# feiyeha/BS-YOLO

Hardware: AMD Instinct MI355X
Metric: images/sec YOLO11s 640x640 bs=64 (forward + NMS) (higher is better)
Workload: dtype f16

## Files before the change

bs_yolo_amd/csrc/c3k2_fused.hip:

```cpp
#include "common.h"

#define CK_TH 4
#define CK_TW 16
#define CK_XR (CK_TH + 4)
#define CK_XC (CK_TW + 4)
#define CK_NX (CK_XR * CK_XC)
#define CK_MR (CK_TH + 2)
#define CK_MC (CK_TW + 2)
#define CK_NM (CK_MR * CK_MC)
#define CK_NPX (CK_TH * CK_TW)

struct C3k2K {
    const half_t* src;
    half_t* dst;
    const half_t *w1, *wa, *wb, *w4;
    const float *b1, *ba, *bb, *b4;
    int B, H, W, lds, ldd, K1, Ka, Kb, K4;
    TileGrid grid;
};

template <int CIN, int C, int C2>
__global__ __launch_bounds__(256, 3) void c3k2_fused_kernel(const C3k2K p) {
    constexpr int CH = C / 2;
    constexpr int YS = C + 8, MS = CH + 8, OS = C2 + 8;
    constexpr int WAS = 9 * C + 8, WBS = 9 * CH + 8;
    constexpr int KS1 = CIN / 16, KSA = 9 * C / 16, KSB = 9 * CH / 16, KSEG = C / 16;
    static_assert(C == 32 && CH == 16 && CIN % 16 == 0 && C2 == 128 && CK_NX == 160 && CK_NPX == 64, "instantiated for the c = 32 C3k2 block");
    constexpr int SY1 = CK_NX * YS, SY0 = CK_NPX * YS, SM = CK_NM * MS, SY2 = CK_NPX * YS;
    constexpr int SOUT = CK_NPX * OS;
    static_assert(SOUT <= SY1 + SY0, "output tile must fit the y1 + y0 tiles it aliases");
    constexpr int SWA = CH * WAS, SWB = C * WBS;
    constexpr int W0S = CIN + 8, SW0 = C * W0S;
    __shared__ __attribute__((aligned(16))) half_t lds[SY1 + SY0 + SM + SY2 + SWA + SWB + SW0 + 2 * (2 * C + CH + C + C2)];
    half_t* sy1 = lds;
    half_t* sy0 = sy1 + SY1;
    half_t* sout = lds;
    half_t* smid = sy0 + SY0;
    half_t* sy2 = smid + SM;
    half_t* swa = sy2 + SY2;
    half_t* swb = swa + SWA;
    half_t* sw0 = swb + SWB;
    float* sb1 = reinterpret_cast<float*>(sw0 + SW0);
    float* sba = sb1 + 2 * C;
    float* sbb = sba + CH;
    float* sb4 = sbb + C;

    const int tid = threadIdx.x, lane = tid & 63;
    const int wave = __builtin_amdgcn_readfirstlane(tid >> 6);
    const int lrow = lane & 31, lh = lane >> 5;

    for (int i = tid; i < 2 * C; i += 256) sb1[i] = p.b1[i];
    if (tid < CH) sba[tid] = p.ba[tid];
    if (tid < C) sbb[tid] = p.bb[tid];
    for (int i = tid; i < C2; i += 256) sb4[i] = p.b4[i];
    half8 w1y1[KS1], a4[3 * KSEG];
#pragma unroll
    for (int ks = 0; ks < KS1; ++ks) w1y1[ks] = *reinterpret_cast<const half8*>(p.w1 + (size_t)(C + lrow) * p.K1 + 16 * ks + 8 * lh);
    for (int i = tid; i < C * (CIN / 8); i += 256) {
        const int row = i / (CIN / 8), ch = i - row * (CIN / 8);
        *reinterpret_cast<half8*>(sw0 + row * W0S + ch * 8) = *reinterpret_cast<const half8*>(p.w1 + (size_t)row * p.K1 + ch * 8);
    }
#pragma unroll
    for (int ks = 0; ks < 3 * KSEG; ++ks) a4[ks] = *reinterpret_cast<const half8*>(p.w4 + (size_t)(32 * wave + lrow) * p.K4 + 16 * ks + 8 * lh);
    for (int i = tid; i < CH * (9 * C / 8); i += 256) {
        const int row = i / (9 * C / 8), ch = i - row * (9 * C / 8);
        *reinterpret_cast<half8*>(swa + row * WAS + ch * 8) = *reinterpret_cast<const half8*>(p.wa + (size_t)row * p.Ka + ch * 8);
    }
    for (int i = tid; i < C * (9 * CH / 8); i += 256) {
        const int row = i / (9 * CH / 8), ch = i - row * (9 * CH / 8);
        *reinterpret_cast<half8*>(swb + row * WBS + ch * 8) = *reinterpret_cast<const half8*>(p.wb + (size_t)row * p.Kb + ch * 8);
    }

    auto tile_origin = [&](int tile, int& n, int& oy0, int& ox0) {
        const TileIdx t = tile_index(p.grid, tile);
        n = t.n; oy0 = t.ty * CK_TH; ox0 = t.tx * CK_TW;
    };
    const int lty = lrow >> 4, ltx = lrow & 15;
    const int eA = 32 * wave + lrow, rA = eA / CK_XC, cA = eA - rA * CK_XC;
    const bool b_y0 = wave == 1 || wave == 2;
    const int eB = b_y0 ? (2 * (wave - 1) + lty + 2) * CK_XC + ltx + 2 : 128 + lrow, rB = eB / CK_XC, cB = eB - rB * CK_XC;
    const unsigned relA = (unsigned)((rA * p.W + cA) * p.lds + 8 * lh), relB = (unsigned)((rB * p.W + cB) * p.lds + 8 * lh);
    half8 xa[KS1], xb[KS1];
    int nn = 0, noy0 = 0, nox0 = 0;
    auto fetch = [&](int tile) {
        tile_origin(tile, nn, noy0, nox0);
        const half_t* tb = p.src + ((long long)(nn * p.H + noy0 - 2) * p.W + (nox0 - 2)) * p.lds;
        const bool inA = (unsigned)(noy0 - 2 + rA) < (unsigned)p.H && (unsigned)(nox0 - 2 + cA) < (unsigned)p.W;
        const bool inB = wave < 3 && (unsigned)(noy0 - 2 + rB) < (unsigned)p.H && (unsigned)(nox0 - 2 + cB) < (unsigned)p.W;
#pragma unroll
        for (int ks = 0; ks < KS1; ++ks) {
            xa[ks] = half8{0, 0, 0, 0, 0, 0, 0, 0};
            xb[ks] = half8{0, 0, 0, 0, 0, 0, 0, 0};
            if (inA) xa[ks] = *reinterpret_cast<const half8*>(tb + relA + 16 * ks);
            if (inB) xb[ks] = *reinterpret_cast<const half8*>(tb + relB + 16 * ks);
        }
    };
    constexpr int CPRW = C2 / 8, NST = CK_NPX * CPRW / 256;
    const int mm2 = wave * 32 + lrow, mc2 = mm2 < CK_NM ? mm2 : CK_NM - 1, r2 = mc2 / CK_MC, c2 = mc2 - r2 * CK_MC;

    const half_t* a2base = swb + lrow * WBS + 8 * lh;
    const int a1off = (lrow & (CH - 1)) * WAS + 8 * lh;

    __builtin_amdgcn_s_waitcnt(0x0F70);
    const TileWalk tw = xcd_tile_walk(blockIdx.x, gridDim.x, p.grid.ntiles);
    int tile = tw.tile;
    if (tile < tw.end) fetch(tile);
    __syncthreads();
    for (; tile < tw.end; tile += tw.step) {
        const int n = nn, oy0 = noy0, ox0 = nox0;
        half_t* ob = p.dst + ((long long)(n * p.H + oy0) * p.W + ox0) * p.ldd;
        auto s1_job = [&](const bool is_y0, const half8 (&wf)[KS1], const half8 (&xf)[KS1], const int e, const int r, const int c, const int opix) {
            f32x16 acc;
            acc_bias(acc, sb1 + (is_y0 ? 0 : C), lh);
#pragma unroll
            for (int ks = 0; ks < KS1; ++ks)
                acc = __builtin_amdgcn_mfma_f32_32x32x16_f16(wf[ks], xf[ks], acc, 0, 0, 0);
            const unsigned keep = (is_y0 || ((unsigned)(oy0 - 2 + r) < (unsigned)p.H && (unsigned)(ox0 - 2 + c) < (unsigned)p.W)) ? 0xffffffffu : 0u;
            half_t* d = is_y0 ? sy0 + opix * YS : sy1 + e * YS;
#pragma unroll
            for (int g = 0; g < C / 8; ++g) {
                union { half4 h; unsigned u[2]; } o;
                const f32x4 tv = silu4_f(f32x4{acc[4 * g], acc[4 * g + 1], acc[4 * g + 2], acc[4 * g + 3]});
#pragma unroll
                for (int q = 0; q < 4; ++q) o.h[q] = (half_t)tv[q];
                o.u[0] &= keep;
                o.u[1] &= keep;
                *reinterpret_cast<half4*>(d + 8 * g + 4 * lh) = o.h;
            }
        };
        s1_job(false, w1y1, xa, eA, rA, cA, 0);
        if (wave == 0) s1_job(false, w1y1, xb, eB, rB, cB, 0);
        else if (wave < 3) {
            int wo = lrow * W0S + 8 * lh;
            asm volatile("" : "+v"(wo));
            half8 w1y0[KS1];
#pragma unroll
            for (int ks = 0; ks < KS1; ++ks) w1y0[ks] = *reinterpret_cast<const half8*>(sw0 + wo + 16 * ks);
            s1_job(true, w1y0, xb, eB, rB, cB, 32 * (wave - 1) + lrow);
        }
        if (tile + tw.step < tw.end) fetch(tile + tw.step);
        lds_barrier();

        {
            const int mm = mm2, r = r2, c = c2;
            const half_t* yb = sy1 + (r * CK_XC + c) * YS + 8 * lh;
            int ao = a1off;
            asm volatile("" : "+v"(ao));
            const half_t* a1base = swa + ao;
            f32x16 acc;
            acc_bias(acc, sba, lh);
#pragma unroll
            for (int ks = 0; ks < KSA; ++ks) {
                const int k0 = 16 * ks, tap = k0 / C, ch0 = (k0 % C) / 8;
                const half8 bf = *reinterpret_cast<const half8*>(yb + ((tap / 3) * CK_XC + tap % 3) * YS + ch0 * 8);
                acc = __builtin_amdgcn_mfma_f32_32x32x16_f16(*reinterpret_cast<const half8*>(a1base + 16 * ks), bf, acc, 0, 0, 0);
            }
            const unsigned keep = ((unsigned)(oy0 - 1 + r) < (unsigned)p.H && (unsigned)(ox0 - 1 + c) < (unsigned)p.W) ? 0xffffffffu : 0u;
            if (mm < CK_NM) {
#pragma unroll
                for (int g = 0; g < CH / 8; ++g) {
                    union { half4 h; unsigned u[2]; } o;
                    const f32x4 tv = silu4_f(f32x4{acc[4 * g], acc[4 * g + 1], acc[4 * g + 2], acc[4 * g + 3]});
#pragma unroll
                    for (int q = 0; q < 4; ++q) o.h[q] = (half_t)tv[q];
                    o.u[0] &= keep;
                    o.u[1] &= keep;
                    *reinterpret_cast<half4*>(smid + mm * MS + 8 * g + 4 * lh) = o.h;
                }
            }
        }
        lds_barrier();

        if (wave < 2) {
            const int ty2 = 2 * wave + lty;
            const half_t* b2base = smid + (ty2 * CK_MC + ltx) * MS + 8 * lh;
            const half_t* y1own = sy1 + ((ty2 + 2) * CK_XC + ltx + 2) * YS;
            f32x16 acc;
            acc_bias(acc, sbb, lh);
#pragma unroll
            for (int ks = 0; ks < KSB; ++ks) {
                const int k0 = 16 * ks, tap = k0 / CH, ch0 = (k0 % CH) / 8;
                const half8 bf = *reinterpret_cast<const half8*>(b2base + ((tap / 3) * CK_MC + tap % 3) * MS + ch0 * 8);
                acc = __builtin_amdgcn_mfma_f32_32x32x16_f16(*reinterpret_cast<const half8*>(a2base + 16 * ks), bf, acc, 0, 0, 0);
            }
#pragma unroll
            for (int g = 0; g < C / 8; ++g) {
                const half4 rv = *reinterpret_cast<const half4*>(y1own + 8 * g + 4 * lh);
                half4 o;
                const f32x4 tv = silu4_f(f32x4{acc[4 * g], acc[4 * g + 1], acc[4 * g + 2], acc[4 * g + 3]});
#pragma unroll
                for (int q = 0; q < 4; ++q) o[q] = (half_t)((float)(half_t)tv[q] + (float)rv[q]);
                *reinterpret_cast<half4*>(sy2 + (32 * wave + lrow) * YS + 8 * g + 4 * lh) = o;
            }
        }
        lds_barrier();

        {
            f32x16 acc[2];
#pragma unroll
            for (int q2 = 0; q2 < 2; ++q2) acc_bias(acc[q2], sb4 + 32 * wave, lh);
#pragma unroll
            for (int ks = 0; ks < 3 * KSEG; ++ks) {
                const int seg = ks / KSEG, kk = ks - seg * KSEG;
#pragma unroll
                for (int q2 = 0; q2 < 2; ++q2) {
                    const int prow = 32 * q2 + lrow;
                    const half_t* sp = seg == 0 ? sy0 + prow * YS : (seg == 1 ? sy1 + ((2 * q2 + lty + 2) * CK_XC + ltx + 2) * YS : sy2 + prow * YS);
                    acc[q2] = __builtin_amdgcn_mfma_f32_32x32x16_f16(a4[ks], *reinterpret_cast<const half8*>(sp + 16 * kk + 8 * lh), acc[q2], 0, 0, 0);
                }
            }
            lds_barrier();
#pragma unroll
            for (int q2 = 0; q2 < 2; ++q2)
#pragma unroll
                for (int g = 0; g < 4; ++g) {
                    const int cc = 32 * wave + 8 * g + 4 * lh;
                    half4 o;
                    const f32x4 tv = silu4_f(f32x4{acc[q2][4 * g], acc[q2][4 * g + 1], acc[q2][4 * g + 2], acc[q2][4 * g + 3]});
#pragma unroll
                    for (int q = 0; q < 4; ++q) o[q] = (half_t)tv[q];
                    *reinterpret_cast<half4*>(sout + (32 * q2 + lrow) * OS + cc) = o;
                }
        }
        lds_barrier();

#pragma unroll
        for (int j = 0; j < NST; ++j) {
            const int id = tid + 256 * j, pr = id / CPRW, cc = (id % CPRW) * 8, sy = pr / CK_TW, sx_ = pr % CK_TW;
            if (oy0 + sy < p.H && ox0 + sx_ < p.W)
                *reinterpret_cast<half8*>(ob + (size_t)(sy * p.W + sx_) * p.ldd + cc) = *reinterpret_cast<const half8*>(sout + pr * OS + cc);
        }
        lds_barrier();
    }
}

bool c3k2_fused_supported(int Cin, int C, int C2) { return Cin == 64 && C == 32 && C2 == 128; }

int launch_c3k2_fused(const C3k2Args& a, hipStream_t s) {
    if (!c3k2_fused_supported(a.Cin, a.C, a.C2)) BSY_FAIL(BSY_ERR_ARG, "c3k2: unsupported widths (Cin %d, c %d, C2 %d): need (64, 32, 128)", a.Cin, a.C, a.C2);
    if (a.B <= 0 || a.H <= 0 || a.W <= 0) BSY_FAIL(BSY_ERR_ARG, "c3k2: bad extent");
    const void* ptrs[10] = {a.src, a.dst, a.w1, a.wa, a.wb, a.w4, a.b1, a.ba, a.bb, a.b4};
    for (const void* q : ptrs)
        if (!q || ((uintptr_t)q & 15)) BSY_FAIL(BSY_ERR_ARG, "c3k2: null or misaligned pointer");
    if ((a.lds & 7) || (a.ldd & 7) || a.lds < a.Cin || a.ldd < a.C2) BSY_FAIL(BSY_ERR_ARG, "c3k2: bad leading dimension");
    C3k2K k;
    k.src = a.src; k.dst = a.dst; k.w1 = (const half_t*)a.w1; k.wa = (const half_t*)a.wa; k.wb = (const half_t*)a.wb; k.w4 = (const half_t*)a.w4;
    k.b1 = a.b1; k.ba = a.ba; k.bb = a.bb; k.b4 = a.b4;
    k.B = a.B; k.H = a.H; k.W = a.W; k.lds = a.lds; k.ldd = a.ldd;
    int cp = 0;
    bsy_conv_packed_dims(2 * a.C, a.Cin, 1, &cp, &k.K1);
    bsy_conv_packed_dims(a.C / 2, a.C, 3, &cp, &k.Ka);
    bsy_conv_packed_dims(a.C, a.C / 2, 3, &cp, &k.Kb);
    bsy_conv_packed_dims(a.C2, 3 * a.C, 1, &cp, &k.K4);
    const int rc = make_tile_grid(k.grid, a.B, a.H, a.W, CK_TH, CK_TW, "c3k2");
    if (rc != BSY_OK) return rc;
    const int grid = k.grid.ntiles < 768 ? k.grid.ntiles : 768;
    hipLaunchKernelGGL((c3k2_fused_kernel<64, 32, 128>), dim3(grid), dim3(256), 0, s, k);
    HIP_TRY(hipGetLastError());
    return BSY_OK;
}
```

bs_yolo_amd/csrc/common.h:

```cpp
#pragma once
#include <hip/hip_runtime.h>
#include <stdint.h>
#include <stdio.h>
#include <string>

#include "../../include/bsyolo.h"

typedef _Float16 half_t;
typedef _Float16 half8 __attribute__((ext_vector_type(8)));
typedef _Float16 half4 __attribute__((ext_vector_type(4)));
typedef _Float16 half2v __attribute__((ext_vector_type(2)));
typedef float f32x16 __attribute__((ext_vector_type(16)));
typedef float f32x4 __attribute__((ext_vector_type(4)));

void bsy_set_error(const char* fmt, ...);
#define BSY_FAIL(code, ...)        \
    do {                           \
        bsy_set_error(__VA_ARGS__); \
        return (code);             \
    } while (0)
#define HIP_TRY(expr)                                                                                     \
    do {                                                                                                  \
        hipError_t _e = (expr);                                                                           \
        if (_e != hipSuccess) BSY_FAIL(BSY_ERR_HIP, "%s failed: %s (%s:%d)", #expr, hipGetErrorString(_e), \
                                       __FILE__, __LINE__);                                               \
    } while (0)

static inline int ceil_div(int a, int b) { return (a + b - 1) / b; }
static inline int round_up(int a, int b) { return ceil_div(a, b) * b; }

struct ConvArgs {
    const half_t* src0;
    const half_t* src1;
    int ld0, ld1;
    int C0, C1;
    int up0, up1;
    int B, H, W, OH, OW;
    int ksize, stride, pad;
    const half_t* wgt;
    const float* bias;
    void* dst;
    int ldd, Cout, out_f32;
    const half_t* res;
    int ldr;
    int act;
    int dst_scale, dst_dy, dst_dx;
    int cfg;
    int epi;
    void* y;
    int y_f32, A, a0, nrows;
    float lvl_stride;
    void* raw;
    int raw_f32, rawC;
    const half_t* tail_wgt;
    const float* tail_bias;
    int nsl_c = 0, nsl_t = 0;
    float* split_ws = nullptr;
};
int launch_conv(const ConvArgs& a, hipStream_t s);
#define BSY_CONV_MAX_CFG 64
int conv_candidates(const ConvArgs& a, int* out, int max_out);
bool conv_cfg_valid(const ConvArgs& a, int cfg);
int conv_korder(const ConvArgs& a);

struct ConvFirstArgs {
    const void* img;
    int img_dtype;
    int B, H, W, OH, OW, ksize, stride, pad;
    const void* w;
    const float* b;
    half_t* dst;
    int ldd, Cout, act;
};
int launch_conv_first(const ConvFirstArgs& a, hipStream_t s);

struct StemArgs {
    const void* img;
    int img_dtype;
    int B, H, W, OH, OW;
    const void* w0;
    const float* b0;
    const void* w1;
    const float* b1;
    int C0, C1, Kpad1;
    half_t* dst;
    int ldd, act;
};
bool stem_fused_supported(int C0, int C1, int H, int W);
int launch_stem_fused(const StemArgs& a, hipStream_t s);

struct BneckArgs {
    const half_t* src;
    int lds;
    int B, H, W, C, CH;
    const void *w1, *w2;
    const float *b1, *b2;
    int Kpad1, Kpad2;
    half_t* dst;
    int ldd, act;
};
bool bneck_fused_supported(int C, int CH);
int launch_bneck_fused(const BneckArgs& a, hipStream_t s);

struct C3k2Args {
    const half_t* src;
    int lds;
    int B, H, W, Cin, C, C2;
    const void *w1, *wa, *wb, *w4;
    const float *b1, *ba, *bb, *b4;
    half_t* dst;
    int ldd;
};
bool c3k2_fused_supported(int Cin, int C, int C2);
int launch_c3k2_fused(const C3k2Args& a, hipStream_t s);

struct DwGenArgs {
    const half_t* src;
    int lds;
    int B, H, W, C, OH, OW, kh, kw, stride;
    const float* w;
    int wld;
    const float* b;
    half_t* dst;
    int ldd, act_c;
    int ident_c0 = 0;
};
int launch_dwconv_generic(const DwGenArgs& a, hipStream_t s);
struct PmsfaArgs {
    const half_t* P;
    int ldp;
    const half_t* x;
    int ldx;
    half_t* dst;
    int ldd;
    int B, H, W, C;
    const float* w2;
    const float* b2;
    int wld2;
    const float* w3;
    const float* b3;
    int wld3;
    const half_t* w4;
    const float* b4;
    int kpad4;
};
bool pmsfa_tail_supported(int C);
int launch_pmsfa_tail(const PmsfaArgs& a, hipStream_t s);
int launch_copy_view(const half_t* src, int lds_, int up, int B, int H, int W, int C, half_t* dst, int ldd, hipStream_t s);
int launch_gap(const half_t* src, int lds_, int B, int H, int W, int C, half_t* out, int ldo, hipStream_t s);
struct MscaSpArgs {
    const half_t* src;
    int lds, B, H, W, C;
    const float* w[9];
    const float* b[9];
    half_t* br[4];
    int ldb[4];
    half_t* gap[4];
    int ldg[4];
};
bool msca_spatial_supported(int H, int W);
int launch_msca_spatial(const MscaSpArgs& a, hipStream_t s);
struct MixArgs {
    const half_t* br[4];
    int ldb[4];
    const float* lg[4];
    int ldl[4];
    int B, HW, C;
    half_t* dst;
    int ldd;
};
int launch_msca_mix(const MixArgs& a, hipStream_t s);
int launch_mul(const half_t* a, int lda, const half_t* b, int ldb, long long npix, int C, half_t* dst, int ldd, hipStream_t s);
struct ElaArgs {
    const half_t* src;
    int lds;
    int B, H, W, C, k;
    const float *wsp, *wch, *gnw, *gnb;
    float ch_coef, sp_coef, res_coef;
    float* scratch;
    half_t* dst;
    int ldd;
};
size_t ela_scratch_floats(int H, int W, int C);
int launch_ela(const ElaArgs& a, hipStream_t s);
int launch_ela_gate(const ElaArgs& a, hipStream_t s);

struct Conv32Args {
    const void* src0;
    const void* src1;
    int src_dtype, first;
    int ld0, ld1, C0, C1, up0, up1;
    int B, H, W, OH, OW, ks, stride, pad;
    const float* w;
    const float* bias;
    float* dst;
    int ldd, Cout;
    const float* res;
    int ldr, act, dst_scale, dst_dy, dst_dx;
    const half_t* wx_hi;
    const half_t* wx_lo;
    int wx_kpad;
};
int launch_conv32(const Conv32Args& a, hipStream_t s);
bool conv32x_mfma_supported(const Conv32Args& a);
int launch_conv32x_mfma(const Conv32Args& a, hipStream_t s);
int launch_conv32_scalar(const Conv32Args& a, hipStream_t s);
bool conv32_mfma_supported(const Conv32Args& a);
int launch_conv32_mfma(const Conv32Args& a, hipStream_t s);
struct Dw32Args {
    const float* src;
    int lds, B, H, W, C, OH, OW, kh, kw, stride;
    const float* w;
    int wld;
    const float* b;
    float* dst;
    int ldd, act_c;
    const float* res;
    int ldr;
};
int launch_dw32(const Dw32Args& a, hipStream_t s);
struct Mix32Args {
    const float* br[4];
    int ldb[4];
    const float* lg[4];
    int ldl[4];
    int B, HW, C;
    float* dst;
    int ldd;
};
int launch_mix32(const Mix32Args& a, hipStream_t s);
int launch_sppf32(float* buf, int ld, int B, int H, int W, int C, hipStream_t s);
int launch_attn32(const float* qkv, int ld, int B, int N, int heads, int kd, int hd, float scale, float* out, int ldo, hipStream_t s,
                  int impl = 0);
bool attn32x_supported(int ld, int ldo, int kd, int hd, const void* qkv, const void* out);
int launch_attn32x(const float* qkv, int ld, int B, int N, int heads, int kd, int hd, float scale, float* out, int ldo, hipStream_t s);
int launch_nhwc2nchw32(const float* src, int ld, int B, int C, int hw, void* out, int out_dtype, hipStream_t s);
int launch_copy32(const float* src, int lds_, int up, int B, int H, int W, int C, float* dst, int ldd, hipStream_t s);
int launch_gap32(const float* src, int lds_, int B, int H, int W, int C, float* out, int ldo, hipStream_t s);
int launch_mul32(const float* x, int ldx, const float* y, int ldy, long long npix, int C, float* dst, int ldd, hipStream_t s);
int launch_ela32(const ElaArgs& a, const float* src, float* dst, hipStream_t s);

struct DwPwArgs {
    const half_t* src;
    int lds;
    int B, H, W, C;
    const float *dww, *dwb;
    const void* wgt;
    const float* bias;
    half_t* dst;
    int ldd, Cout, act;
};
bool dwpw_fused_supported(int C, int Cout);
int launch_dwpw_fused(const DwPwArgs& a, hipStream_t s);

struct DwArgs {
    const half_t* src;
    int lds;
    int B, H, W, C;
    const float* w;
    const float* b;
    half_t* dst;
    int ldd;
    int act;
    const half_t* res;
// ... 168 lines not shown
```

bs_yolo_amd/csrc/engine.hip:

```cpp
#include <stdlib.h>
#include <string.h>

#include <algorithm>
#include <vector>

#include "common.h"

struct bsy_engine {
    int device = 0;
    void* weights = nullptr;
    size_t weight_bytes = 0;
    char* arena = nullptr;
    size_t arena_bytes = 0;
    unsigned arena_gen = 0;
    unsigned weights_gen = 0;
};

struct bsy_plan {
    bsy_engine* eng = nullptr;
    std::vector<bsy_op> ops;
    std::vector<size_t> buf_off;
    std::vector<size_t> buf_size;
    char* workspace = nullptr;
    size_t workspace_bytes = 0;
// ... 200 lines not shown
    float* f(const bsy_view& v) { char* b = base(v); return b ? (float*)b + v.coff : nullptr; }
};

static inline size_t fp32x_align(size_t n) { return (n + 255) & ~(size_t)255; }

int run_op_f32(const bsy_plan* p, const bsy_op& op, Resolver& R, hipStream_t s, bool& handled) {
    const char* wb = (const char*)p->eng->weights;
    handled = true;
    switch (op.kind) {
        case BSY_OP_CONV_FIRST:
        case BSY_OP_CONV: {
            Conv32Args a;
            memset(&a, 0, sizeof(a));
            a.first = op.kind == BSY_OP_CONV_FIRST;
            a.src0 = a.first ? (const void*)R.base(op.src0) : (const void*)R.f(op.src0);
            a.src_dtype = op.in_dtype;
            a.src1 = R.f(op.src1);
            a.ld0 = op.src0.ld; a.ld1 = op.src1.buf >= 0 ? op.src1.ld : 0;
            a.C0 = op.src0.C; a.C1 = op.src1.buf >= 0 ? op.src1.C : 0;
            a.up0 = op.up0; a.up1 = op.up1;
            a.B = op.B; a.H = op.H; a.W = op.W; a.OH = op.OH; a.OW = op.OW; a.ks = op.ksize; a.stride = op.stride; a.pad = op.pad;
            a.w = (const float*)(wb + op.w_off); a.bias = (const float*)(wb + op.b_off);
            a.dst = R.f(op.dst); a.ldd = op.dst.ld; a.Cout = op.dst.C;
            a.res = R.f(op.res); a.ldr = op.res.buf >= 0 ? op.res.ld : 0;
            a.act = op.act; a.dst_scale = op.dst_scale > 0 ? op.dst_scale : 1; a.dst_dy = op.dst_dy; a.dst_dx = op.dst_dx;
            if (op.out_f32 >= 2) BSY_FAIL(BSY_ERR_ARG, "fp32 mode: fused Detect decoder ops are not part of fp32 plans");
            if (!R.ok) return BSY_ERR_ARG;
            if (op.prec == 2) {
                const size_t K = (size_t)a.ks * a.ks * (a.C0 + a.C1), kpad = (K + 31) & ~(size_t)31;
                const size_t hi_off = fp32x_align(K * a.Cout * 4), lo_off = hi_off + fp32x_align((size_t)a.Cout * kpad * 2);
                a.wx_hi = (const half_t*)(wb + op.w_off + hi_off);
                a.wx_lo = (const half_t*)(wb + op.w_off + lo_off);
                a.wx_kpad = (int)kpad;
                if (conv32x_mfma_supported(a)) return launch_conv32x_mfma(a, s);
            }
            return launch_conv32(a, s);
        }
        case BSY_OP_DWCONV:
        case BSY_OP_DWCONV_G: {
            Dw32Args a;
            memset(&a, 0, sizeof(a));
            const bool g = op.kind == BSY_OP_DWCONV_G;
            a.src = R.f(op.src0); a.lds = op.src0.ld; a.B = op.B; a.H = op.H; a.W = op.W; a.C = op.src0.C; a.OH = op.OH; a.OW = op.OW;
            a.kh = g ? op.ksize : 3; a.kw = g ? op.pad : 3; a.stride = g ? op.stride : 1;
            a.wld = g ? op.heads : op.src0.C;
            a.w = (const float*)(wb + op.w_off) + (g ? op.key_dim : 0); a.b = (const float*)(wb + op.b_off) + (g ? op.key_dim : 0);
            a.dst = R.f(op.dst); a.ldd = op.dst.ld; a.act_c = g ? op.act : (op.act ? op.src0.C : 0);
            a.res = g ? nullptr : R.f(op.res); a.ldr = (!g && op.res.buf >= 0) ? op.res.ld : 0;
            if (!R.ok) return BSY_ERR_ARG;
            return launch_dw32(a, s);
        }
        case BSY_OP_SPPF_POOL: {
            float* b = R.f(op.src0);
            if (!R.ok) return BSY_ERR_ARG;
            return launch_sppf32(b, op.src0.ld, op.B, op.H, op.W, op.src0.C, s);
        }
        case BSY_OP_ATTN: {
            const float* q = R.f(op.src0);
            float* o = R.f(op.dst);
            if (!R.ok) return BSY_ERR_ARG;
            if (op.prec == 2 && attn32x_supported(op.src0.ld, op.dst.ld, op.key_dim, op.head_dim, q, o))
                return launch_attn32x(q, op.src0.ld, op.B, op.H * op.W, op.heads, op.key_dim, op.head_dim, op.scale, o, op.dst.ld, s);
            return launch_attn32(q, op.src0.ld, op.B, op.H * op.W, op.heads, op.key_dim, op.head_dim, op.scale, o, op.dst.ld, s);
        }
        case BSY_OP_NHWC2NCHW: {
            if (op.dst.buf >= BSY_EXT_BASE && (op.dst.buf - BSY_EXT_BASE >= R.n_ext || !R.ext[op.dst.buf - BSY_EXT_BASE])) return BSY_OK;
            const float* src = R.f(op.src0);
            void* out = R.base(op.dst);
            if (!R.ok) return BSY_ERR_ARG;
            return launch_nhwc2nchw32(src, op.src0.ld, op.B, op.src0.C, op.H * op.W, out, op.out_dtype, s);
        }
        case BSY_OP_COPY: {
            const float* src = R.f(op.src0);
            float* dst = R.f(op.dst);
            if (!R.ok) return BSY_ERR_ARG;
            return launch_copy32(src, op.src0.ld, op.up0, op.B, op.H, op.W, op.src0.C, dst, op.dst.ld, s);
        }
        case BSY_OP_GAP: {
            const float* src = R.f(op.src0);
            float* dst = R.f(op.dst);
            if (!R.ok) return BSY_ERR_ARG;
            return launch_gap32(src, op.src0.ld, op.B, op.H, op.W, op.src0.C, dst, op.dst.ld, s);
        }
        case BSY_OP_MSCA_MIX: {
            Mix32Args a;
            for (int i = 0; i < 4; ++i) {
                const bsy_view& bv = i < 3 ? op.box[i] : op.res;
                const bsy_view& lv = i < 3 ? op.cls[i] : op.msk[0];
                a.br[i] = R.f(bv); a.ldb[i] = bv.ld; a.lg[i] = R.f(lv); a.ldl[i] = lv.ld;
            }
            a.B = op.B; a.HW = op.H * op.W; a.C = op.dst.C; a.dst = R.f(op.dst); a.ldd = op.dst.ld;
            if (!R.ok) return BSY_ERR_ARG;
            return launch_mix32(a, s);
        }
        case BSY_OP_MUL: {
            const float* x = R.f(op.src0);
            const float* y = R.f(op.src1);
            float* dst = R.f(op.dst);
            if (!R.ok) return BSY_ERR_ARG;
            return launch_mul32(x, op.src0.ld, y, op.src1.ld, (long long)op.B * op.H * op.W, op.dst.C, dst, op.dst.ld, s);
        }
        case BSY_OP_ELA: {
            ElaArgs a;
            memset(&a, 0, sizeof(a));
            a.lds = op.src0.ld; a.B = op.B; a.H = op.H; a.W = op.W; a.C = op.src0.C; a.k = op.ksize;
            const float* blob = (const float*)(wb + op.w_off);
            a.wsp = blob; a.wch = blob + (size_t)a.C * a.k; a.gnw = a.wch + (size_t)a.C * a.k; a.gnb = a.gnw + a.C;
            a.ch_coef = op.scale; a.sp_coef = op.lvl_stride[0]; a.res_coef = op.lvl_stride[1];
            a.scratch = R.f(op.res); a.ldd = op.dst.ld;
            const float* src = R.f(op.src0);
            float* dst = R.f(op.dst);
            if (!R.ok) return BSY_ERR_ARG;
            return launch_ela32(a, src, dst, s);
        }
        case BSY_OP_DECODE:
        case BSY_OP_RAW_NCHW:
            handled = false;
            return BSY_OK;
        default:
            BSY_FAIL(BSY_ERR_ARG, "fp32 mode: op kind %d has no fp32 implementation (fused kinds are fp16-only)", op.kind);
    }
}

int run_op(const bsy_plan* p, const bsy_op& op, Resolver& R, hipStream_t s, ConvArgs* cargs = nullptr) {
    const char* wb = (const char*)p->eng->weights;
    if (op.prec == 1 || op.prec == 2) {
        bool handled = false;
        const int rc = run_op_f32(p, op, R, s, handled);
        if (rc != BSY_OK || handled) return rc;
    } else if (op.prec != 0) {
        BSY_FAIL(BSY_ERR_ARG, "plan_run: unknown precision mode %d", op.prec);
    }
    switch (op.kind) {
        case BSY_OP_CONV_FIRST: {
            ConvFirstArgs a;
            a.img = R.base(op.src0); a.img_dtype = op.in_dtype;
            a.B = op.B; a.H = op.H; a.W = op.W; a.OH = op.OH; a.OW = op.OW;
            a.ksize = op.ksize; a.stride = op.stride; a.pad = op.pad;
            a.w = (const void*)(wb + op.w_off); a.b = (const float*)(wb + op.b_off);
            a.dst = R.h(op.dst); a.ldd = op.dst.ld; a.Cout = op.dst.C; a.act = op.act;
            if (!R.ok) return BSY_ERR_ARG;
            return launch_conv_first(a, s);
        }
        case BSY_OP_STEM: {
            StemArgs a;
            a.img = R.base(op.src0); a.img_dtype = op.in_dtype;
            a.B = op.B; a.H = op.H; a.W = op.W; a.OH = op.OH; a.OW = op.OW;
            a.w0 = (const void*)(wb + op.w_off); a.b0 = (const float*)(wb + op.b_off);
            a.w1 = (const void*)(wb + op.w2_off); a.b1 = (const float*)(wb + op.b2_off);
            a.C0 = op.mid_c; a.C1 = op.dst.C;
            int cp = 0;
            bsy_conv_packed_dims(a.C1, a.C0, 3, &cp, &a.Kpad1);
            a.dst = R.h(op.dst); a.ldd = op.dst.ld; a.act = op.act;
            if (!R.ok) return BSY_ERR_ARG;
            return launch_stem_fused(a, s);
        }
        case BSY_OP_BNECK: {
            BneckArgs a;
            a.src = R.h(op.src0); a.lds = op.src0.ld; a.B = op.B; a.H = op.H; a.W = op.W;
            a.C = op.dst.C; a.CH = op.mid_c;
            a.w1 = (const void*)(wb + op.w_off); a.b1 = (const float*)(wb + op.b_off);
            a.w2 = (const void*)(wb + op.w2_off); a.b2 = (const float*)(wb + op.b2_off);
            int cp = 0;
            bsy_conv_packed_dims(a.CH, a.C, 3, &cp, &a.Kpad1);
            bsy_conv_packed_dims(a.C, a.CH, 3, &cp, &a.Kpad2);
            a.dst = R.h(op.dst); a.ldd = op.dst.ld; a.act = op.act;
            if (!R.ok) return BSY_ERR_ARG;
            return launch_bneck_fused(a, s);
        }
        case BSY_OP_S2D: {
            const void* img = R.base(op.src0);
            half_t* dst = R.h(op.dst);
            if (!R.ok) return BSY_ERR_ARG;
            return launch_s2d(img, op.in_dtype, op.B, op.H, op.W, dst, op.dst.ld, s);
        }
        case BSY_OP_C3K2: {
            C3k2Args a;
            a.src = R.h(op.src0); a.lds = op.src0.ld; a.B = op.B; a.H = op.H; a.W = op.W;
            a.Cin = op.src0.C; a.C = op.mid_c; a.C2 = op.dst.C;
            a.w1 = wb + op.aux_off[0]; a.b1 = (const float*)(wb + op.aux_off[1]);
            a.wa = wb + op.aux_off[2]; a.ba = (const float*)(wb + op.aux_off[3]);
            a.wb = wb + op.aux_off[4]; a.bb = (const float*)(wb + op.aux_off[5]);
            a.w4 = wb + op.aux_off[6]; a.b4 = (const float*)(wb + op.aux_off[7]);
            a.dst = R.h(op.dst); a.ldd = op.dst.ld;
            if (!R.ok) return BSY_ERR_ARG;
            return launch_c3k2_fused(a, s);
        }
        case BSY_OP_DWPW: {
            DwPwArgs a;
            a.src = R.h(op.src0); a.lds = op.src0.ld; a.B = op.B; a.H = op.H; a.W = op.W; a.C = op.src0.C;
            a.dww = (const float*)(wb + op.w_off); a.dwb = (const float*)(wb + op.b_off);
            a.wgt = (const void*)(wb + op.w2_off); a.bias = (const float*)(wb + op.b2_off);
            a.dst = R.h(op.dst); a.ldd = op.dst.ld; a.Cout = op.dst.C; a.act = op.act;
            if (!R.ok) return BSY_ERR_ARG;
            return launch_dwpw_fused(a, s);
        }
        case BSY_OP_DWCONV_G: {
            DwGenArgs a;
            a.src = R.h(op.src0); a.lds = op.src0.ld; a.B = op.B; a.H = op.H; a.W = op.W; a.C = op.src0.C;
            a.OH = op.OH; a.OW = op.OW; a.kh = op.ksize; a.kw = op.pad; a.stride = op.stride;
            a.wld = op.heads; a.w = (const float*)(wb + op.w_off) + op.key_dim; a.b = (const float*)(wb + op.b_off) + op.key_dim;
            a.dst = R.h(op.dst); a.ldd = op.dst.ld; a.act_c = op.act;
            a.ident_c0 = op.mid_c;
            if (!R.ok) return BSY_ERR_ARG;
            return launch_dwconv_generic(a, s);
        }
        case BSY_OP_PMSFA_TAIL: {
            PmsfaArgs a;
            a.P = R.h(op.src0); a.ldp = op.src0.ld; a.x = R.h(op.res); a.ldx = op.res.ld; a.dst = R.h(op.dst); a.ldd = op.dst.ld;
            a.B = op.B; a.H = op.H; a.W = op.W; a.C = op.dst.C;
            a.w2 = (const float*)(wb + op.aux_off[0]); a.b2 = (const float*)(wb + op.aux_off[1]); a.wld2 = op.heads;
            a.w3 = (const float*)(wb + op.aux_off[2]); a.b3 = (const float*)(wb + op.aux_off[3]); a.wld3 = op.key_dim;
            a.w4 = (const half_t*)(wb + op.aux_off[4]); a.b4 = (const float*)(wb + op.aux_off[5]);
            int cp = 0;
            bsy_conv_packed_dims(a.C, a.C, 1, &cp, &a.kpad4);
            if (!R.ok || op.src0.C != a.C || op.res.C != a.C) return BSY_ERR_ARG;
            return launch_pmsfa_tail(a, s);
        }
        case BSY_OP_COPY: {
            const half_t* src = R.h(op.src0);
            half_t* dst = R.h(op.dst);
            if (!R.ok) return BSY_ERR_ARG;
            return launch_copy_view(src, op.src0.ld, op.up0, op.B, op.H, op.W, op.src0.C, dst, op.dst.ld, s);
        }
        case BSY_OP_GAP: {
            const half_t* src = R.h(op.src0);
            half_t* dst = R.h(op.dst);
            if (!R.ok) return BSY_ERR_ARG;
            return launch_gap(src, op.src0.ld, op.B, op.H, op.W, op.src0.C, dst, op.dst.ld, s);
        }
        case BSY_OP_MSCA_SPATIAL: {
            MscaSpArgs a;
            a.src = R.h(op.src0); a.lds = op.src0.ld; a.B = op.B; a.H = op.H; a.W = op.W; a.C = op.src0.C;
            for (int i = 0; i < 9; ++i) {
                a.w[i] = (const float*)(wb + op.aux_off[2 * i]);
                a.b[i] = (const float*)(wb + op.aux_off[2 * i + 1]);
            }
            for (int i = 0; i < 4; ++i) {
                const bsy_view& bv = i < 3 ? op.box[i] : op.res;
                const bsy_view& gv = i < 3 ? op.cls[i] : op.msk[0];
                a.br[i] = R.h(bv); a.ldb[i] = bv.ld; a.gap[i] = R.h(gv); a.ldg[i] = gv.ld;
            }
            if (!R.ok) return BSY_ERR_ARG;
            return launch_msca_spatial(a, s);
        }
        case BSY_OP_MSCA_MIX: {
            MixArgs a;
            for (int i = 0; i < 4; ++i) {
                const bsy_view& bv = i < 3 ? op.box[i] : op.res;
                const bsy_view& lv = i < 3 ? op.cls[i] : op.msk[0];
                a.br[i] = R.h(bv); a.ldb[i] = bv.ld; a.lg[i] = R.f(lv); a.ldl[i] = lv.ld;
            }
            a.B = op.B; a.HW = op.H * op.W; a.C = op.dst.C; a.dst = R.h(op.dst); a.ldd = op.dst.ld;
            if (!R.ok) return BSY_ERR_ARG;
            return launch_msca_mix(a, s);
        }
        case BSY_OP_MUL: {
            const half_t* x = R.h(op.src0);
            const half_t* y = R.h(op.src1);
            half_t* dst = R.h(op.dst);
            if (!R.ok) return BSY_ERR_ARG;
            return launch_mul(x, op.src0.ld, y, op.src1.ld, (long long)op.B * op.H * op.W, op.dst.C, dst, op.dst.ld, s);
        }
        case BSY_OP_ELA: {
            ElaArgs a;
            a.src = R.h(op.src0); a.lds = op.src0.ld; a.B = op.B; a.H = op.H; a.W = op.W; a.C = op.src0.C; a.k = op.ksize;
            const float* blob = (const float*)(wb + op.w_off);
            a.wsp = blob; a.wch = blob + (size_t)a.C * a.k; a.gnw = a.wch + (size_t)a.C * a.k; a.gnb = a.gnw + a.C;
            a.ch_coef = op.scale; a.sp_coef = op.lvl_stride[0]; a.res_coef = op.lvl_stride[1];
            a.scratch = R.f(op.res); a.dst = R.h(op.dst); a.ldd = op.dst.ld;
            if (!R.ok) return BSY_ERR_ARG;
            return launch_ela(a, s);
        }
        case BSY_OP_CONV: {
            ConvArgs a;
            a.src0 = R.h(op.src0); a.src1 = R.h(op.src1);
            a.ld0 = op.src0.ld; a.ld1 = op.src1.buf >= 0 ? op.src1.ld : 0;
            a.C0 = op.src0.C; a.C1 = op.src1.buf >= 0 ? op.src1.C : 0;
            a.up0 = op.up0; a.up1 = op.up1;
            a.B = op.B; a.H = op.H; a.W = op.W; a.OH = op.OH; a.OW = op.OW;
            a.ksize = op.ksize; a.stride = op.stride; a.pad = op.pad;
            a.wgt = (const half_t*)(wb + op.w_off); a.bias = (const float*)(wb + op.b_off);
            a.dst = op.out_f32 ? (void*)R.f(op.dst) : (void*)R.h(op.dst);
            a.ldd = op.dst.ld; a.Cout = op.dst.C; a.out_f32 = op.out_f32;
            a.res = R.h(op.res); a.ldr = op.res.buf >= 0 ? op.res.ld : 0;
            a.act = op.act; a.dst_scale = op.dst_scale; a.dst_dy = op.dst_dy; a.dst_dx = op.dst_dx;
            a.epi = 0; a.y = nullptr; a.raw = nullptr; a.y_f32 = a.raw_f32 = a.A = a.a0 = a.nrows = a.rawC = 0; a.lvl_stride = 0.f;
            a.tail_wgt = nullptr; a.tail_bias = nullptr;
            if (op.out_f32 >= 2) {
                a.epi = op.out_f32; a.out_f32 = 0; a.dst = nullptr; a.ldd = 8; a.Cout = op.nl;
                a.y = R.base(op.dst); a.y_f32 = op.out_dtype == BSY_F32; a.A = op.A; a.a0 = op.lvl_h[1]; a.nrows = op.dst.C;
                a.lvl_stride = op.lvl_stride[0];
                const bsy_view& rv = op.box[0];
                const bool bound = rv.buf >= BSY_EXT_BASE && rv.buf - BSY_EXT_BASE < R.n_ext && R.ext[rv.buf - BSY_EXT_BASE];
                a.raw = bound ? R.base(rv) : nullptr; a.raw_f32 = a.y_f32; a.rawC = rv.C;
                if (op.out_f32 == 3 && op.mid_c > 0) {
                    a.Cout = op.mid_c;
                    a.tail_wgt = (const half_t*)(wb + op.w2_off); a.tail_bias = (const float*)(wb + op.b2_off);
                }
            }
            if (op.ksplit > 0 && op.out_f32 == 0) {
                a.nsl_c = op.ksplit & 255; a.nsl_t = (op.ksplit >> 8) & 255;
                a.split_ws = R.f(op.box[0]);
            }
            a.cfg = op.tuned_cfg - 1;
            if (!R.ok) return BSY_ERR_ARG;
            if (cargs) { *cargs = a; return BSY_OK; }
            return launch_conv(a, s);
        }
        case BSY_OP_DWCONV: {
            DwArgs a;
            a.src = R.h(op.src0); a.lds = op.src0.ld; a.B = op.B; a.H = op.H; a.W = op.W; a.C = op.src0.C;
            a.w = (const float*)(wb + op.w_off); a.b = (const float*)(wb + op.b_off);
            a.dst = R.h(op.dst); a.ldd = op.dst.ld; a.act = op.act;
            a.res = R.h(op.res); a.ldr = op.res.buf >= 0 ? op.res.ld : 0;
            if (!R.ok) return BSY_ERR_ARG;
            return launch_dwconv(a, s);
        }
        case BSY_OP_SPPF_POOL: {
            half_t* b = R.h(op.src0);
            if (!R.ok) return BSY_ERR_ARG;
            return launch_sppf_pool(b, op.src0.ld, op.B, op.H, op.W, op.src0.C, s);
        }
        case BSY_OP_ATTN: {
            AttnArgs a;
            a.qkv = R.h(op.src0); a.ld = op.src0.ld; a.B = op.B; a.N = op.H * op.W; a.heads = op.heads;
            a.key_dim = op.key_dim; a.head_dim = op.head_dim; a.scale = op.scale;
            a.out = R.h(op.dst); a.ldo = op.dst.ld;
            if (!R.ok) return BSY_ERR_ARG;
            return launch_attention(a, s);
        }
        case BSY_OP_DECODE: {
            DecodeArgs a;
            memset(&a, 0, sizeof(a));
            a.nl = op.nl; a.B = op.B; a.nc = op.nc; a.nm = op.nm; a.A = op.A; a.ne = op.ne;
            const bool extra = op.nm || op.ne;
            for (int l = 0; l < op.nl && l < 3; ++l) {
// ... 236 lines not shown
}

extern "C" int bsy_plan_autotune_in_place(bsy_plan* p, void* const* ext, int n_ext, bsy_stream stream, int rounds) {
    if (!p || (n_ext && !ext) || rounds < 1 || rounds > 16) BSY_FAIL(BSY_ERR_ARG, "plan_autotune_in_place: bad argument");
    p->drop_graphs();
    hipStream_t s = (hipStream_t)stream;
    const size_t n = p->ops.size();
    Resolver R{p, ext, n_ext};
    std::vector<std::vector<int>> cand(n);
    size_t K = 0;
    for (size_t i = 0; i < n; ++i) {
        bsy_op& op = p->ops[i];
        if (op.kind == BSY_OP_CONV && op.tuned_cfg <= 0 && op.prec == 0) {
            ConvArgs a;
            int rc = run_op(p, op, R, s, &a);
            if (rc != BSY_OK) return rc;
            int list[BSY_CONV_MAX_CFG];
            const int nc = conv_candidates(a, list, BSY_CONV_MAX_CFG);
            cand[i].assign(list, list + (nc > 0 ? nc : 0));
            K = cand[i].size() > K ? cand[i].size() : K;
        }
        const int rc = run_op(p, op, R, s);
        if (rc != BSY_OK) return rc;
    }
    if (K == 0) return BSY_OK;
    std::vector<float> best(n, 1e30f), ms(n);
    std::vector<std::vector<float>> tk(n);
    for (size_t i = 0; i < n; ++i) tk[i].assign(cand[i].size(), 1e30f);
    std::vector<int> best_c(n, -1);
    for (size_t i = 0; i < n; ++i)
        if (!cand[i].empty()) best_c[i] = cand[i][0];
    for (size_t k = 0; k < K; ++k) {
        for (size_t i = 0; i < n; ++i)
            if (!cand[i].empty()) p->ops[i].tuned_cfg = (k < cand[i].size() ? cand[i][k] : best_c[i]) + 1;
        for (int r = 0; r < rounds; ++r) {
            const int rc = bsy_plan_profile(p, ext, n_ext, stream, ms.data());
            if (rc != BSY_OK) {
                for (size_t i = 0; i < n; ++i)
                    if (!cand[i].empty()) p->ops[i].tuned_cfg = 0;
                return rc;
            }
            for (size_t i = 0; i < n; ++i)
                if (k < cand[i].size()) {
                    if (ms[i] < tk[i][k]) tk[i][k] = ms[i];
                    if (ms[i] < best[i]) { best[i] = ms[i]; best_c[i] = cand[i][k]; }
                }
        }
    }
    for (size_t i = 0; i < n; ++i)
        if (!cand[i].empty()) p->ops[i].tuned_cfg = best_c[i] + 1;
    return BSY_OK;
}

extern "C" int bsy_conv2d(const void* x, int ldx, int B, int H, int W, int C1, const void* w, const float* b, void* y,
                          int ldy, int C2, int ksize, int stride, int act, const void* res, int ldr, int y_f32,
                          bsy_stream stream) {
    if (!x || !w || !b || !y) BSY_FAIL(BSY_ERR_ARG, "conv2d: null pointer");
    ConvArgs a;
    memset(&a, 0, sizeof(a));
    a.src0 = (const half_t*)x; a.ld0 = ldx; a.C0 = C1; a.B = B; a.H = H; a.W = W;
    a.ksize = ksize; a.stride = stride; a.pad = ksize / 2;
    a.OH = (H + 2 * a.pad - ksize) / stride + 1; a.OW = (W + 2 * a.pad - ksize) / stride + 1;
    a.wgt = (const half_t*)w; a.bias = b; a.dst = y; a.ldd = ldy; a.Cout = C2; a.out_f32 = y_f32;
    a.res = (const half_t*)res; a.ldr = ldr; a.act = act; a.dst_scale = 1;
    const char* forced = getenv("BSY_CONV_CFG");
    a.cfg = forced ? atoi(forced) : -1;
    if (a.cfg >= 0 && !conv_cfg_valid(a, a.cfg)) BSY_FAIL(BSY_ERR_ARG, "conv: BSY_CONV_CFG=%d is not valid for this shape", a.cfg);
    return launch_conv(a, (hipStream_t)stream);
}

extern "C" int bsy_conv2d_f32(const float* x, int ldx, int B, int H, int W, int C1, const float* w, const float* b, float* y, int ldy,
                              int C2, int ksize, int stride, int act, const float* res, int ldr, int impl, bsy_stream stream) {
    if (!x || !w || !b || !y) BSY_FAIL(BSY_ERR_ARG, "conv2d_f32: null pointer");
    if (B <= 0 || H <= 0 || W <= 0 || C1 <= 0 || C2 <= 0 || ksize < 1 || !(ksize & 1) || (stride != 1 && stride != 2) || ldx < C1 || ldy < C2 ||
        (res && ldr < C2) || impl < 0 || impl > 2)
        BSY_FAIL(BSY_ERR_ARG, "conv2d_f32: bad shape");
    Conv32Args a;
    memset(&a, 0, sizeof(a));
    a.src0 = x; a.src_dtype = BSY_F32; a.ld0 = ldx; a.C0 = C1; a.B = B; a.H = H; a.W = W;
    a.ks = ksize; a.stride = stride; a.pad = ksize / 2;
    a.OH = (H + 2 * a.pad - ksize) / stride + 1; a.OW = (W + 2 * a.pad - ksize) / stride + 1;
    a.w = w; a.bias = b; a.dst = y; a.ldd = ldy; a.Cout = C2; a.res = res; a.ldr = ldr; a.act = act; a.dst_scale = 1;
    if (impl == 1) return launch_conv32_scalar(a, (hipStream_t)stream);
    if (impl == 2) return launch_conv32_mfma(a, (hipStream_t)stream);
    return launch_conv32(a, (hipStream_t)stream);
}

extern "C" int bsy_conv2d_f32x(const float* x, int ldx, int B, int H, int W, int C1, const void* w_hi, const void* w_lo, int k_pad,
                               const float* b, float* y, int ldy, int C2, int ksize, int stride, int act, const float* res, int ldr,
                               bsy_stream stream) {
    if (!x || !w_hi || !w_lo || !b || !y) BSY_FAIL(BSY_ERR_ARG, "conv2d_f32x: null pointer");
    if (B <= 0 || H <= 0 || W <= 0 || C1 <= 0 || C2 <= 0 || ksize < 1 || !(ksize & 1) || (stride != 1 && stride != 2) || ldx < C1 || ldy < C2 ||
        (res && ldr < C2) || k_pad < ksize * ksize * C1 || (k_pad & 31))
        BSY_FAIL(BSY_ERR_ARG, "conv2d_f32x: bad shape");
    Conv32Args a;
    memset(&a, 0, sizeof(a));
    a.src0 = x; a.src_dtype = BSY_F32; a.ld0 = ldx; a.C0 = C1; a.B = B; a.H = H; a.W = W;
    a.ks = ksize; a.stride = stride; a.pad = ksize / 2;
    a.OH = (H + 2 * a.pad - ksize) / stride + 1; a.OW = (W + 2 * a.pad - ksize) / stride + 1;
    a.w = (const float*)w_hi;
    a.bias = b; a.dst = y; a.ldd = ldy; a.Cout = C2; a.res = res; a.ldr = ldr; a.act = act; a.dst_scale = 1;
    a.wx_hi = (const half_t*)w_hi; a.wx_lo = (const half_t*)w_lo; a.wx_kpad = k_pad;
    return launch_conv32x_mfma(a, (hipStream_t)stream);
}

extern "C" int bsy_conv_first_f32(const void* img, int img_dtype, int B, int H, int W, const float* w, const float* b, float* y, int ldy,
                                 int C2, int ksize, int stride, int act, int impl, bsy_stream stream) {
    if (!img || !w || !b || !y) BSY_FAIL(BSY_ERR_ARG, "conv_first_f32: null pointer");
    if (B <= 0 || H <= 0 || W <= 0 || C2 <= 0 || ksize < 1 || !(ksize & 1) || (stride != 1 && stride != 2) || ldy < C2 || impl < 0 || impl > 2 ||
        (img_dtype != BSY_F16 && img_dtype != BSY_F32))
        BSY_FAIL(BSY_ERR_ARG, "conv_first_f32: bad shape");
    Conv32Args a;
    memset(&a, 0, sizeof(a));
    a.first = 1; a.src0 = img; a.src_dtype = img_dtype; a.C0 = 3; a.B = B; a.H = H; a.W = W;
    a.ks = ksize; a.stride = stride; a.pad = ksize / 2;
    a.OH = (H + 2 * a.pad - ksize) / stride + 1; a.OW = (W + 2 * a.pad - ksize) / stride + 1;
    a.w = w; a.bias = b; a.dst = y; a.ldd = ldy; a.Cout = C2; a.act = act; a.dst_scale = 1;
    if (impl == 1) return launch_conv32_scalar(a, (hipStream_t)stream);
    if (impl == 2) return launch_conv32_mfma(a, (hipStream_t)stream);
    return launch_conv32(a, (hipStream_t)stream);
}

extern "C" int bsy_attention_f32(const float* qkv, int ld, int B, int N, int heads, int key_dim, int head_dim, float scale, float* out,
                                 int ldo, int impl, bsy_stream stream) {
    if (!qkv || !out || B <= 0 || N <= 0 || impl < 0 || impl > 3) BSY_FAIL(BSY_ERR_ARG, "attention_f32: bad argument");
    if (impl == 3) return launch_attn32x(qkv, ld, B, N, heads, key_dim, head_dim, scale, out, ldo, (hipStream_t)stream);
    return launch_attn32(qkv, ld, B, N, heads, key_dim, head_dim, scale, out, ldo, (hipStream_t)stream, impl);
}

extern "C" int bsy_conv_first(const void* img, int img_dtype, int B, int H, int W, const void* w, const float* b,
                              void* y, int ldy, int C2, int ksize, int stride, int act, bsy_stream stream) {
    if (!img || !w || !b || !y) BSY_FAIL(BSY_ERR_ARG, "conv_first: null pointer");
    ConvFirstArgs a;
    a.img = img; a.img_dtype = img_dtype; a.B = B; a.H = H; a.W = W; a.ksize = ksize; a.stride = stride; a.pad = ksize / 2;
    a.OH = (H + 2 * a.pad - ksize) / stride + 1; a.OW = (W + 2 * a.pad - ksize) / stride + 1;
    a.w = w; a.b = b; a.dst = (half_t*)y; a.ldd = ldy; a.Cout = C2; a.act = act;
    return launch_conv_first(a, (hipStream_t)stream);
}

extern "C" int bsy_stem_fused(const void* img, int img_dtype, int B, int H, int W, const void* w0, const float* b0, int C0,
                              const void* w1, const float* b1, int C1, void* y, int ldy, int act, bsy_stream stream) {
    if (!img || !w0 || !b0 || !w1 || !b1 || !y) BSY_FAIL(BSY_ERR_ARG, "stem: null pointer");
    StemArgs a;
    a.img = img; a.img_dtype = img_dtype; a.B = B; a.H = H; a.W = W;
    const int OH0 = (H - 1) / 2 + 1, OW0 = (W - 1) / 2 + 1;
    a.OH = (OH0 - 1) / 2 + 1; a.OW = (OW0 - 1) / 2 + 1;
    a.w0 = w0; a.b0 = b0; a.w1 = w1; a.b1 = b1; a.C0 = C0; a.C1 = C1;
    int cp = 0;
    bsy_conv_packed_dims(C1, C0, 3, &cp, &a.Kpad1);
    a.dst = (half_t*)y; a.ldd = ldy; a.act = act;
    return launch_stem_fused(a, (hipStream_t)stream);
}

extern "C" int bsy_stem_fused_supported(int C0, int C1, int H, int W) { return stem_fused_supported(C0, C1, H, W) ? 1 : 0; }

extern "C" int bsy_bottleneck_fused(const void* x, int ldx, int B, int H, int W, int C, int CH, const void* w1,
                                    const float* b1, const void* w2, const float* b2, void* y, int ldy, int act,
                                    bsy_stream stream) {
    if (!x || !w1 || !b1 || !w2 || !b2 || !y) BSY_FAIL(BSY_ERR_ARG, "bottleneck: null pointer");
    BneckArgs a;
    a.src = (const half_t*)x; a.lds = ldx; a.B = B; a.H = H; a.W = W; a.C = C; a.CH = CH;
    a.w1 = w1; a.b1 = b1; a.w2 = w2; a.b2 = b2;
    int cp = 0;
    if (C <= 0 || CH <= 0) BSY_FAIL(BSY_ERR_ARG, "bottleneck: bad widths");
    bsy_conv_packed_dims(CH, C, 3, &cp, &a.Kpad1);
    bsy_conv_packed_dims(C, CH, 3, &cp, &a.Kpad2);
    a.dst = (half_t*)y; a.ldd = ldy; a.act = act;
    return launch_bneck_fused(a, (hipStream_t)stream);
}

extern "C" int bsy_bottleneck_fused_supported(int C, int CH) { return bneck_fused_supported(C, CH) ? 1 : 0; }

extern "C" int bsy_c3k2_fused(const void* x, int ldx, int B, int H, int W, int Cin, int c, int C2, const void* w1, const float* b1,
                              const void* wa, const float* ba, const void* wb, const float* bb, const void* w4, const float* b4,
                              void* y, int ldy, bsy_stream stream) {
    C3k2Args a;
    a.src = (const half_t*)x; a.lds = ldx; a.B = B; a.H = H; a.W = W; a.Cin = Cin; a.C = c; a.C2 = C2;
    a.w1 = w1; a.b1 = b1; a.wa = wa; a.ba = ba; a.wb = wb; a.bb = bb; a.w4 = w4; a.b4 = b4;
    a.dst = (half_t*)y; a.ldd = ldy;
    return launch_c3k2_fused(a, (hipStream_t)stream);
}

extern "C" int bsy_c3k2_fused_supported(int Cin, int c, int C2) { return c3k2_fused_supported(Cin, c, C2) ? 1 : 0; }

extern "C" int bsy_dwconv(const void* x, int ldx, int B, int H, int W, int C, int kh, int kw, int stride, const float* w,
                          int wld, const float* b, void* y, int ldy, int act, bsy_stream stream) {
    DwGenArgs a;
    a.src = (const half_t*)x; a.lds = ldx; a.B = B; a.H = H; a.W = W; a.C = C; a.kh = kh; a.kw = kw; a.stride = stride;
    if (kh < 1 || kw < 1 || (stride != 1 && stride != 2)) BSY_FAIL(BSY_ERR_ARG, "dwconv: bad kernel / stride");
    a.OH = (H + 2 * (kh / 2) - kh) / stride + 1; a.OW = (W + 2 * (kw / 2) - kw) / stride + 1;
    a.w = w; a.wld = wld; a.b = b; a.dst = (half_t*)y; a.ldd = ldy; a.act_c = act ? C : 0;
    return launch_dwconv_generic(a, (hipStream_t)stream);
}

extern "C" size_t bsy_ela_scratch_bytes(int B, int H, int W, int C) {
    return (B > 0 && H > 0 && W > 0 && C > 0) ? ela_scratch_floats(H, W, C) * (size_t)B * sizeof(float) : 0;
}

extern "C" int bsy_ela(const void* x, int ldx, int B, int H, int W, int C, int k, const float* wsp, const float* wch,
                       const float* gnw, const float* gnb, const float* coef, void* scratch, void* y, int ldy,
                       bsy_stream stream) {
    if (!coef) BSY_FAIL(BSY_ERR_ARG, "ela: null coefficient pointer");
    ElaArgs a;
    a.src = (const half_t*)x; a.lds = ldx; a.B = B; a.H = H; a.W = W; a.C = C; a.k = k;
    a.wsp = wsp; a.wch = wch; a.gnw = gnw; a.gnb = gnb; a.ch_coef = coef[0]; a.sp_coef = coef[1]; a.res_coef = coef[2];
    a.scratch = (float*)scratch; a.dst = (half_t*)y; a.ldd = ldy;
    return launch_ela(a, (hipStream_t)stream);
}

extern "C" int bsy_dwpw_fused(const void* x, int ldx, int B, int H, int W, int C, const float* dww, const float* dwb,
                              const void* w, const float* b, void* y, int ldy, int C2, int act, bsy_stream stream) {
    DwPwArgs a;
    a.src = (const half_t*)x; a.lds = ldx; a.B = B; a.H = H; a.W = W; a.C = C; a.dww = dww; a.dwb = dwb; a.wgt = w; a.bias = b;
    a.dst = (half_t*)y; a.ldd = ldy; a.Cout = C2; a.act = act;
    return launch_dwpw_fused(a, (hipStream_t)stream);
}

extern "C" int bsy_dwpw_fused_supported(int C, int C2) { return dwpw_fused_supported(C, C2) ? 1 : 0; }

extern "C" int bsy_dwconv3x3(const void* x, int ldx, int B, int H, int W, int C, const float* w, const float* b, void* y,
                             int ldy, int act, const void* res, int ldr, bsy_stream stream) {
    if (!x || !w || !b || !y) BSY_FAIL(BSY_ERR_ARG, "dwconv3x3: null pointer");
    DwArgs a;
    a.src = (const half_t*)x; a.lds = ldx; a.B = B; a.H = H; a.W = W; a.C = C; a.w = w; a.b = b;
    a.dst = (half_t*)y; a.ldd = ldy; a.act = act; a.res = (const half_t*)res; a.ldr = ldr;
    return launch_dwconv(a, (hipStream_t)stream);
}

extern "C" int bsy_sppf_pool(void* buf, int ld, int B, int H, int W, int C, bsy_stream stream) {
    if (!buf) BSY_FAIL(BSY_ERR_ARG, "sppf_pool: null pointer");
    return launch_sppf_pool((half_t*)buf, ld, B, H, W, C, (hipStream_t)stream);
}

extern "C" int bsy_attention(const void* qkv, int ld, int B, int N, int heads, int key_dim, int head_dim, float scale,
                             void* out, int ldo, bsy_stream stream) {
    if (!qkv || !out) BSY_FAIL(BSY_ERR_ARG, "attention: null pointer");
    AttnArgs a;
    a.qkv = (const half_t*)qkv; a.ld = ld; a.B = B; a.N = N; a.heads = heads; a.key_dim = key_dim; a.head_dim = head_dim;
    a.scale = scale; a.out = (half_t*)out; a.ldo = ldo;
    return launch_attention(a, (hipStream_t)stream);
}

extern "C" int bsy_detect_decode(const float* const* box, const int* ldb, const float* const* cls, const int* ldc,
                                 const float* const* msk, const int* ldm, const int* lvl_h, const int* lvl_w,
                                 const float* lvl_stride, int nl, int B, int nc, int nm, void* y, int y_dtype,
                                 bsy_stream stream) {
    if (!box || !ldb || !cls || !ldc || !lvl_h || !lvl_w || !lvl_stride || !y || nl < 1 || nl > 3)
        BSY_FAIL(BSY_ERR_ARG, "detect_decode: bad argument");
    if (nm && (!msk || !ldm)) BSY_FAIL(BSY_ERR_ARG, "detect_decode: mask inputs missing");
    DecodeArgs a;
    memset(&a, 0, sizeof(a));
    a.nl = nl; a.B = B; a.nc = nc; a.nm = nm; a.A = 0;
    for (int l = 0; l < nl; ++l) {
        a.box[l] = box[l]; a.cls[l] = cls[l]; a.msk[l] = nm ? msk[l] : nullptr;
        a.ldb[l] = ldb[l]; a.ldc[l] = ldc[l]; a.ldm[l] = nm ? ldm[l] : 0;
        a.h[l] = lvl_h[l]; a.w[l] = lvl_w[l]; a.stride[l] = lvl_stride[l];
    }
    a.y = y; a.y_dtype = y_dtype;
    return launch_decode(a, (hipStream_t)stream);
}
```

bs_yolo_amd/csrc/stem_fused.hip:

```cpp
#include "image_conv.h"

#define ST_TH 4
#define ST_TW 16
#define ST_R0 (2 * ST_TH + 1)
#define ST_C0W (2 * ST_TW + 1)
#define ST_NE (ST_R0 * ST_C0W)
#define ST_NMT ((ST_NE + 31) / 32)
#define ST_EV (ST_TW + 1)
#define ST_IR (2 * ST_R0 + 1)
#define ST_NG 17
#define ST_ROWPX (4 * ST_NG)
#define ST_NITEM (ST_IR * ST_NG)
#define ST_NLOAD ((ST_NITEM + 255) / 256)

struct StemK {
    const void* img;
    const half_t* w0;
    const float* b0;
    const half_t* w1;
    const float* b1;
    half_t* dst;
    int B, H, W, OH0, OW0, OH1, OW1, ldd, Kpad1, act;
    TileGrid grid;
};

template <typename T, int C0, int C1>
__global__ __launch_bounds__(256, sizeof(T) == 4 ? 2 : 3) void stem_fused_kernel(const StemK p) {
    constexpr int NCH = C0 / 8;
    constexpr int KS1 = (9 * C0 + 15) / 16;
    constexpr int NH = C1 / 32;
    constexpr int LDO = C1 + 8;
    constexpr int IMG = ST_IR * ST_ROWPX * 4;
    constexpr int MID = ST_NE * C0;
    constexpr int OUT = ST_TH * ST_TW * LDO;
    static_assert(C0 == 16 || C0 == 32, "layer-0 width");
    static_assert(NH == 1 || NH == 2, "layer-1 width");
    __shared__ __attribute__((aligned(16))) half_t lds[IMG + MID + OUT + 2 * (C0 + C1)];
    half_t* simg = lds;
    half_t* smid = lds + IMG;
    half_t* sout = smid + MID;
    float* sb0 = reinterpret_cast<float*>(sout + OUT);
    float* sb1 = sb0 + C0;

    const int tid = threadIdx.x, lane = tid & 63;
    const int wave = __builtin_amdgcn_readfirstlane(tid >> 6);
    const int lrow = lane & 31, lh = lane >> 5;
    const T* img = reinterpret_cast<const T*>(p.img);

    if (tid < C0) sb0[tid] = p.b0[tid];
    if (tid < C1) sb1[tid] = p.b1[tid];
    half8 a0[IMGC_KSUB];
#pragma unroll
    for (int s = 0; s < IMGC_KSUB; ++s)
        a0[s] = *reinterpret_cast<const half8*>(p.w0 + (size_t)lrow * IMGC_KROW + 16 * s + 8 * lh);
    const int mt1 = wave & 1, nh1 = wave >> 1;
    const bool l1 = nh1 < NH;
    half8 a1[KS1];
#pragma unroll
    for (int ks = 0; ks < KS1; ++ks)
        a1[ks] = l1 ? *reinterpret_cast<const half8*>(p.w1 + (size_t)(nh1 * 32 + lrow) * p.Kpad1 + 16 * ks + 8 * lh)
                    : half8{0, 0, 0, 0, 0, 0, 0, 0};
    int it_r[ST_NLOAD], it_j[ST_NLOAD];
#pragma unroll
    for (int i = 0; i < ST_NLOAD; ++i) {
        const int idx = tid + 256 * i;
        it_r[i] = idx / ST_NG;
        it_j[i] = idx - it_r[i] * ST_NG;
    }
    const int e1base = (2 * (2 * mt1 + (lrow >> 4))) * ST_C0W + (lrow & 15);

    auto tile_origin = [&](int tile, int& n, int& oy0, int& ox0) {
        const TileIdx t = tile_index(p.grid, tile);
        n = t.n; oy0 = t.ty * ST_TH; ox0 = t.tx * ST_TW;
    };
    ImgItem<T> pre[ST_NLOAD];
    int nn = 0, noy0 = 0, nox0 = 0;
    auto fetch = [&](int tile) {
        tile_origin(tile, nn, noy0, nox0);
        const int n = nn, oy0 = noy0, ox0 = nox0;
        const T* ip = img + (size_t)n * 3 * p.H * p.W;
#pragma unroll
        for (int i = 0; i < ST_NLOAD; ++i)
            pre[i] = img_item_load<T>(ip, p.H, p.W, 4 * oy0 - 3 + it_r[i], 4 * ox0 - 4 + 4 * it_j[i], tid + 256 * i < ST_NITEM);
    };

    __builtin_amdgcn_s_waitcnt(0x0F70);
    const TileWalk tw = xcd_tile_walk(blockIdx.x, gridDim.x, p.grid.ntiles);
    int tile = tw.tile;
    if (tile < tw.end) fetch(tile);
    for (; tile < tw.end; tile += tw.step) {
        const int n = nn, oy0 = noy0, ox0 = nox0;
#pragma unroll
        for (int i = 0; i < ST_NLOAD; ++i)
            if (tid + 256 * i < ST_NITEM) img_item_park<T>(pre[i], simg + (it_r[i] * ST_ROWPX + 4 * it_j[i]) * 4);
        lds_barrier();
        if (tile + tw.step < tw.end) fetch(tile + tw.step);

        const int r00 = 2 * oy0 - 1, c00 = 2 * ox0 - 1;
        for (int mt = wave; mt < ST_NMT; mt += 4) {
            const int pp = mt * 32 + lrow;
            const int pc = pp < ST_NE ? pp : ST_NE - 1;
            const int r = pc / ST_C0W, c = pc - r * ST_C0W;
            const int win = (2 * r * ST_ROWPX + 2 * c + 1) * 4;
            f32x16 acc;
            acc_bias(acc, sb0, lh);
#pragma unroll
            for (int s = 0; s < IMGC_KSUB; ++s)
                acc = __builtin_amdgcn_mfma_f32_32x32x16_f16(a0[s], img_frag<ST_ROWPX>(simg, win, s, lh), acc, 0, 0, 0);
            const unsigned keep = ((unsigned)(r00 + r) < (unsigned)p.OH0 && (unsigned)(c00 + c) < (unsigned)p.OW0) ? 0xffffffffu : 0u;
            const int e = r * ST_C0W + (c & 1) * ST_EV + (c >> 1);
            if (pp < ST_NE) {
#pragma unroll
                for (int g = 0; g < NCH; ++g) {
                    union { half4 h; unsigned u[2]; } o;
                    f32x4 t = f32x4{acc[4 * g], acc[4 * g + 1], acc[4 * g + 2], acc[4 * g + 3]};
                    if (p.act) t = silu4_f(t);
#pragma unroll
                    for (int q = 0; q < 4; ++q) o.h[q] = (half_t)t[q];
                    o.u[0] &= keep;
                    o.u[1] &= keep;
                    *reinterpret_cast<half4*>(smid + (e * NCH + (g ^ ((e >> 2) & (NCH - 1)))) * 8 + 4 * lh) = o.h;
                }
            }
        }
        lds_barrier();

        if (l1) {
            f32x16 acc;
            acc_bias(acc, sb1 + nh1 * 32, lh);
#pragma unroll
            for (int ks = 0; ks < KS1; ++ks) {
                const int k0 = 16 * ks, k1 = k0 + 8;
                const int t0 = k0 / C0, t1 = k1 / C0;
                const int ch0 = (k0 % C0) / 8, ch1 = (k1 % C0) / 8;
                const int e0 = t0 < 9 ? (t0 / 3) * ST_C0W + ((t0 % 3) & 1) * ST_EV + ((t0 % 3) >> 1) : 0;
                const int e1 = t1 < 9 ? (t1 / 3) * ST_C0W + ((t1 % 3) & 1) * ST_EV + ((t1 % 3) >> 1) : 0;
                const int e = e1base + (e0 == e1 ? e0 : (lh ? e1 : e0));
                const int ch = lh ? ch1 : ch0;
                half8 bf = *reinterpret_cast<const half8*>(smid + (e * NCH + (ch ^ ((e >> 2) & (NCH - 1)))) * 8);
                if (t1 >= 9 && (t0 >= 9 || lh)) bf = half8{0, 0, 0, 0, 0, 0, 0, 0};
                acc = __builtin_amdgcn_mfma_f32_32x32x16_f16(a1[ks], bf, acc, 0, 0, 0);
            }
            const int prow = mt1 * 32 + lrow;
#pragma unroll
            for (int g = 0; g < 4; ++g) {
                const int c = nh1 * 32 + 8 * g + 4 * lh;
                half4 o;
                f32x4 t = f32x4{acc[4 * g], acc[4 * g + 1], acc[4 * g + 2], acc[4 * g + 3]};
                if (p.act) t = silu4_f(t);
#pragma unroll
                for (int q = 0; q < 4; ++q) o[q] = (half_t)t[q];
                *reinterpret_cast<half4*>(sout + prow * LDO + c) = o;
            }
        }
        lds_barrier();

        constexpr int CPRW = C1 / 8;
#pragma unroll
        for (int id = tid; id < ST_TH * ST_TW * CPRW; id += 256) {
            const int prow = id / CPRW, cc = (id % CPRW) * 8;
            const int oy = oy0 + prow / ST_TW, ox = ox0 + prow % ST_TW;
            if (oy < p.OH1 && ox < p.OW1)
                *reinterpret_cast<half8*>(p.dst + ((size_t)(n * p.OH1 + oy) * p.OW1 + ox) * p.ldd + cc) =
                    *reinterpret_cast<const half8*>(sout + prow * LDO + cc);
        }
    }
}

bool stem_fused_supported(int C0, int C1, int H, int W) {
    return ((C0 == 32 && C1 == 64) || (C0 == 16 && C1 == 32)) && !(W & 3) && H >= 4 && W >= 4;
}

template <typename T>
static int launch_t(const StemArgs& a, const StemK& k, hipStream_t s) {
    const int slots = sizeof(T) == 4 ? 512 : 768;
    const int grid = k.grid.ntiles < slots ? k.grid.ntiles : slots;
    if (a.C0 == 32) hipLaunchKernelGGL((stem_fused_kernel<T, 32, 64>), dim3(grid), dim3(256), 0, s, k);
    else hipLaunchKernelGGL((stem_fused_kernel<T, 16, 32>), dim3(grid), dim3(256), 0, s, k);
    HIP_TRY(hipGetLastError());
    return BSY_OK;
}

int launch_stem_fused(const StemArgs& a, hipStream_t s) {
    if (!stem_fused_supported(a.C0, a.C1, a.H, a.W))
        BSY_FAIL(BSY_ERR_ARG, "stem: unsupported shape (C0 %d, C1 %d, H %d, W %d): need (32,64) or (16,32) channels, W %% 4 == 0", a.C0, a.C1, a.H, a.W);
    const int OH0 = (a.H - 1) / 2 + 1, OW0 = (a.W - 1) / 2 + 1;
    const int OH1 = (OH0 - 1) / 2 + 1, OW1 = (OW0 - 1) / 2 + 1;
    if (a.OH != OH1 || a.OW != OW1) BSY_FAIL(BSY_ERR_ARG, "stem: output extent mismatch (%d x %d, expected %d x %d)", a.OH, a.OW, OH1, OW1);
    const int esz = a.img_dtype == BSY_F32 ? 4 : 2;
    if (((uintptr_t)a.img & (4 * esz - 1)) || ((uintptr_t)a.dst & 15) || (a.ldd & 7) || ((uintptr_t)a.w0 & 15) ||
        ((uintptr_t)a.w1 & 15) || ((uintptr_t)a.b0 & 15) || ((uintptr_t)a.b1 & 15) || (a.Kpad1 & 7) || a.Kpad1 < 9 * a.C0 || a.Kpad1 < 16 * ((9 * a.C0 + 15) / 16))
        BSY_FAIL(BSY_ERR_ARG, "stem: misaligned pointer / leading dimension");
    StemK k;
    k.img = a.img; k.w0 = (const half_t*)a.w0; k.b0 = a.b0; k.w1 = (const half_t*)a.w1; k.b1 = a.b1; k.dst = a.dst;
    k.B = a.B; k.H = a.H; k.W = a.W; k.OH0 = OH0; k.OW0 = OW0; k.OH1 = OH1; k.OW1 = OW1; k.ldd = a.ldd; k.Kpad1 = a.Kpad1;
    k.act = a.act;
    const int rc = make_tile_grid(k.grid, a.B, OH1, OW1, ST_TH, ST_TW, "stem");
    if (rc != BSY_OK) return rc;
    if (a.img_dtype == BSY_F16) return launch_t<half_t>(a, k, s);
    if (a.img_dtype == BSY_F32) return launch_t<float>(a, k, s);
    BSY_FAIL(BSY_ERR_ARG, "stem: image dtype %d unsupported", a.img_dtype);
}
```

bs_yolo_amd/engine.py:

```python
from __future__ import annotations

import ctypes as C
import json
import math
import os
from collections import OrderedDict
from typing import Dict, List, Mapping, Optional, Tuple

import torch

from . import lib as L
from . import ops as O
from . import tta as T
from .plan import Plan
from .weights import BN_EPS, adopt_offsets, pack_plan_weights


class YoloEngine:
    def __init__(self, cfg: dict, state_dict: Mapping[str, torch.Tensor], device: int = 0, bn_eps: float = BN_EPS,
                 autotune: Optional[bool] = None, fuse_stem: Optional[bool] = None,
                 fuse_bneck: Optional[bool] = None, fuse_head: Optional[bool] = None, fuse_dwpw: Optional[bool] = None,
                 merge_c3k: Optional[bool] = None, fuse_msca: Optional[bool] = None, fuse_tail: Optional[bool] = None,
                 max_plans: Optional[int] = None, precision: str = "fp16", graph: Optional[bool] = None, graph_ring: int = 3,
                 latency: Optional[bool] = None, fuse_pmsfa: Optional[bool] = None):
        if not torch.cuda.is_available():
            raise RuntimeError("bs_yolo_amd needs a ROCm GPU (there is no CPU fallback)")
        self.cfg = cfg
        self.precision = precision
        self.latency = (os.environ.get("BSY_LATENCY", "0") == "1") if latency is None else bool(latency)
        self.device = torch.device("cuda", device)
        self._h = C.c_void_p()
        L.check(L.lib.bsy_engine_create(device, C.byref(self._h)))
        self._plans: "OrderedDict[Tuple, Tuple]" = OrderedDict()
        self.max_plans = int(os.environ.get("BSY_MAX_PLANS", "8")) if max_plans is None else int(max_plans)
        self._tuned = set()
        self._elems: Dict[Tuple[int, int], int] = {}
        self._tune_cache: Dict[tuple, int] = {}
        self._tune_family: Dict[tuple, int] = {}
        self.tune_stats = {"timed_ops": 0, "cached_ops": 0, "family_ops": 0, "autotune_calls": 0}
        self.tune_mode = os.environ.get("BSY_TUNE_IN_PLACE", "1")
        self._tune_file = os.environ.get("BSY_TUNE_CACHE")
        if self._tune_file and os.path.exists(self._tune_file):
            try:
                self._tune_cache = {tuple(k): int(v) for k, v in json.load(open(self._tune_file))}
                for k, v in self._tune_cache.items():
                    self._tune_family.setdefault(self._family(k), v)
            except (OSError, ValueError):
                self._tune_cache = {}
        self.reuse = os.environ.get("BSY_ARENA_REUSE", "1") != "0" and not os.environ.get("BSY_PLAN_GUARD")
        self.graph = (os.environ.get("BSY_GRAPH", "0") == "1") if graph is None else bool(graph)
        self.graph_ring = max(1, int(graph_ring))
        self._rings: Dict[Tuple, dict] = {}
        self._gstream = None
        import threading
        self._lock = threading.RLock()
        self._last_done = None
        self._last_stream = None
        self.graph_stats = {"captures": 0, "replays": 0, "eager": 0}
        self._tta_geom: Dict[Tuple[int, int], list] = {}
        self._tta_bufs: "OrderedDict[Tuple, torch.Tensor]" = OrderedDict()
        self.autotune = ((os.environ.get("BSY_AUTOTUNE", "1") != "0") if autotune is None else bool(autotune)) and precision == "fp16"
        self.fuse_stem = fuse_stem
        self.fuse_bneck = fuse_bneck
        self.fuse_head = fuse_head
        self.fuse_dwpw = fuse_dwpw
        self.merge_c3k = merge_c3k
        self.fuse_msca = fuse_msca
        self.fuse_tail = fuse_tail
        self.fuse_pmsfa = fuse_pmsfa
        self._packed = Plan(cfg, 1, 64, 64, **self._fuse_kw())
        blob = pack_plan_weights(self._packed, state_dict, bn_eps)
        self.weight_bytes = len(blob)
        buf = (C.c_char * len(blob)).from_buffer_copy(blob)
        L.check(L.lib.bsy_engine_load_weights(self._h, buf, len(blob)))
        self.meta = dict(self._packed.meta)
        self.nc = self.meta["nc"]
        self.stride = torch.tensor(self.meta["strides"])
        self.names = {i: f"{i}" for i in range(self.nc)}

    def load_weights(self, state_dict: Mapping[str, torch.Tensor], bn_eps: float = BN_EPS) -> None:
        with self._lock:
            blob = pack_plan_weights(self._packed, state_dict, bn_eps)
            if len(blob) != self.weight_bytes:
                raise ValueError(f"state_dict packs to {len(blob)} bytes, the engine was built for {self.weight_bytes}")
            for plan, _ in self._plans.values():
                adopt_offsets(plan, self._packed)
            buf = (C.c_char * len(blob)).from_buffer_copy(blob)
            L.check(L.lib.bsy_engine_load_weights(self._h, buf, len(blob)))

    def _fuse_kw(self):
        return dict(fuse_stem=self.fuse_stem, fuse_bneck=self.fuse_bneck, fuse_head=self.fuse_head, fuse_dwpw=self.fuse_dwpw,
                    merge_c3k=self.merge_c3k, fuse_msca=self.fuse_msca, fuse_tail=self.fuse_tail, precision=self.precision,
                    lanes=True if getattr(self, "graph", False) else None, latency=getattr(self, "latency", False),
                    fuse_pmsfa=self.fuse_pmsfa)

    def plan_for(self, B: int, H: int, W: int, in_dtype: torch.dtype, out_dtype: torch.dtype):
        key = (B, H, W, in_dtype, out_dtype)
        hit = self._plans.get(key)
        if hit is not None:
            self._plans.move_to_end(key)
            return hit
        if H % 32 or W % 32:
            raise ValueError(f"input {H}x{W} must be a multiple of the max stride 32 (utils/checks.py:120-172)")
        plan = Plan(self.cfg, B, H, W, L.dtype_code(in_dtype), L.dtype_code(out_dtype), **self._fuse_kw())
        adopt_offsets(plan, self._packed)
        ops = plan.c_ops()
        sizes = (C.c_int64 * len(plan.buf_bytes))(*plan.buf_bytes)
        h = C.c_void_p()
        with torch.cuda.device(self.device):
            if os.environ.get("BSY_PLAN_GUARD"):
                L.check(L.lib.bsy_plan_create(self._h, ops, len(plan.ops), sizes, len(plan.buf_bytes), C.byref(h)))
                plan.arena_bytes = sum((b + 255) & ~255 for b in plan.buf_bytes)
            else:
                offs, arena = plan.assign_offsets(self.reuse)
                plan.arena_bytes = arena
                L.check(L.lib.bsy_plan_create_arena(self._h, ops, len(plan.ops), sizes, (C.c_int64 * len(offs))(*offs),
                                                    len(offs), arena, C.byref(h)))
        plan.conv_sigs = [plan.conv_signature(o) for o in plan.ops]
        for sg in plan.conv_sigs:
            if sg is not None and sg not in self._tune_cache and self._family(sg) in self._tune_family:
                self._tune_cache[sg] = self._tune_family[self._family(sg)]
                self.tune_stats["family_ops"] += 1
        preset = (C.c_int32 * len(plan.ops))(*[self._tune_cache.get(sg, -1) if sg is not None else -1 for sg in plan.conv_sigs])
        L.check(L.lib.bsy_plan_set_tuning(h, preset, len(plan.ops)))
        while len(self._plans) >= max(self.max_plans, 1):
            old_key, (_, old) = self._plans.popitem(last=False)
            L.lib.bsy_plan_destroy(old)
            for rk in [k for k in self._rings if k[0] == old_key]:
                del self._rings[rk]
        self._plans[key] = (plan, h)
        return plan, h

    @property
    def arena_bytes(self) -> int:
        return int(L.lib.bsy_engine_arena_bytes(self._h))

    @staticmethod
    def _family(sg: tuple) -> tuple:
        B, H, W = sg[:3]
        return sg[3:] + (int(round(math.log2(max(B * H * W, 1)))),)

    def _autotune(self, plan, h, ext, n, stream):
        nops = len(plan.ops)
        valid = (C.c_int32 * nops)()
        L.check(L.lib.bsy_plan_check_tuning(h, ext, n, valid, nops))
        bad = [i for i in range(nops) if valid[i] == 0]
        if bad:
            clear = (C.c_int32 * nops)(*([-1] * nops))
            for i in bad:
                sg = plan.conv_sigs[i]
                cfg = self._tune_cache.pop(sg, None)
                if cfg is not None and self._tune_family.get(self._family(sg)) == cfg:
                    del self._tune_family[self._family(sg)]
                clear[i] = -2
            L.check(L.lib.bsy_plan_set_tuning(h, clear, nops))
            self.tune_stats["invalid_presets"] = self.tune_stats.get("invalid_presets", 0) + len(bad)
        todo = sum(1 for sg in plan.conv_sigs if sg is not None and sg not in self._tune_cache)
        self.tune_stats["autotune_calls"] += 1
        self.tune_stats["timed_ops"] += todo
        self.tune_stats["cached_ops"] += sum(1 for sg in plan.conv_sigs if sg is not None) - todo
        if self.tune_mode == "1":
            L.check(L.lib.bsy_plan_autotune_in_place(h, ext, n, C.c_void_p(stream), 3))
        else:
            L.check(L.lib.bsy_plan_autotune(h, ext, n, C.c_void_p(stream)))
        if todo:
            out = (C.c_int32 * nops)()
            L.check(L.lib.bsy_plan_get_tuning(h, out, nops))
            for sg, c in zip(plan.conv_sigs, out):
                if sg is not None and c >= 0:
                    self._tune_cache.setdefault(sg, int(c))
                    self._tune_family.setdefault(self._family(sg), int(c))
            if self._tune_file:
                try:
                    tmp = self._tune_file + f".{os.getpid()}.tmp"
                    json.dump([[list(k), v] for k, v in self._tune_cache.items()], open(tmp, "w"))
                    os.replace(tmp, self._tune_file)
                except OSError:
                    pass

    def _max_view_elems(self, H: int, W: int) -> int:
        key = (H, W)
        hit = self._elems.get(key)
        if hit is None:
            p1 = Plan(self.cfg, 1, H, W, **self._fuse_kw())
            hit = 1
            for o in p1.ops:
                for k in ("src0", "src1", "dst", "res"):
                    t = o.get(k)
                    if t is not None and t.buf < L.BSY_EXT_BASE:
                        hs, ws = (t.H // 2, t.W // 2) if t.up else (t.H, t.W)
                        hit = max(hit, hs * ws * t.ld)
            self._elems[key] = hit
        return hit

    def _ext(self, im, y, raws, proto=None):
        ptrs = [im.data_ptr(), y.data_ptr()] + [r.data_ptr() if r is not None else None for r in raws]
        ptrs.append(proto.data_ptr() if proto is not None else None)
        return (C.c_void_p * len(ptrs))(*ptrs), len(ptrs)

    def forward(self, im: torch.Tensor, want_raw: bool = True):
        if im.device != self.device:
            raise ValueError(f"input on {im.device}, engine on {self.device}")
        if im.dtype not in (torch.float16, torch.float32):
            raise TypeError("input must be fp16 or fp32 (BCHW, 0..1)")
        im = im.contiguous()
        B, Cc, H, W = im.shape
        if Cc != 3:
            raise ValueError("expected 3 input channels")
        big = self._max_view_elems(H, W)
        if B > 1 and B * big >= (1 << 31) - (1 << 24):
            n_chunks = -(-B * big // ((1 << 31) - (1 << 24)))
            step = -(-B // n_chunks)
            outs = [self.forward(im[i:i + step], want_raw) for i in range(0, B, step)]
            y = torch.cat([o[0] for o in outs])
            if self.meta["nm"]:
                raws = [torch.cat([o[1][0][l] for o in outs]) for l in range(3)] if want_raw else [None] * 3
                return y, (raws, y[:, 4 + self.meta["nc"]:], torch.cat([o[1][2] for o in outs]))
            if self.meta["ne"]:
                raws = [torch.cat([o[1][0][l] for o in outs]) for l in range(3)] if want_raw else [None] * 3
                return y, (raws, y[:, 4 + self.meta["nc"]:])
            return y, ([torch.cat([o[1][l] for o in outs]) for l in range(3)] if want_raw else [None] * 3)
        with self._lock:
            return self._forward_one(im, want_raw, B, H, W)

    def _forward_one(self, im, want_raw, B, H, W):
        plan, h = self.plan_for(B, H, W, im.dtype, im.dtype)
        m = plan.meta

        def outputs():
            y = torch.empty((B, 4 + m["nc"] + m["nm"] + m["ne"], m["A"]), dtype=im.dtype, device=self.device)
            raws: List[Optional[torch.Tensor]] = [None, None, None]
            if want_raw:
                raws = [torch.empty((B, m["no"], lh, lw), dtype=im.dtype, device=self.device) for lh, lw in m["levels"]]
            proto = None
            if m["nm"]:
                ph, pw = m["proto_hw"]
                proto = torch.empty((B, m["nm"], ph, pw), dtype=im.dtype, device=self.device)
            return y, raws, proto

        if self.graph:
            ring = self._rings.setdefault(((B, H, W, im.dtype, im.dtype), bool(want_raw)), {"i": 0, "slots": []})
            if len(ring["slots"]) < self.graph_ring:
                ring["slots"].append(outputs())
            y, raws, proto = ring["slots"][ring["i"] % len(ring["slots"])]
            ring["i"] += 1
        else:
            y, raws, proto = outputs()
# ... 145 lines not shown
```

bs_yolo_amd/lib.py:

```python
from __future__ import annotations

import ctypes as C
import os
from pathlib import Path

import torch

PKG = Path(__file__).resolve().parent
LIB_PATH = Path(os.environ["BSY_LIB"]) if os.environ.get("BSY_LIB") else PKG / "libbsyolo_hip.so"

BSY_F16, BSY_F32, BSY_U8 = 0, 1, 2
BSY_EXT_BASE = 0x100000
(OP_CONV_FIRST, OP_CONV, OP_DWCONV, OP_SPPF_POOL, OP_ATTN, OP_DECODE, OP_RAW_NCHW, OP_NHWC2NCHW, OP_STEM, OP_BNECK, OP_DWCONV_G, OP_COPY, OP_GAP, OP_MSCA_MIX, OP_MUL, OP_ELA, OP_DWPW, OP_MSCA_SPATIAL, OP_C3K2, OP_S2D, OP_PMSFA_TAIL, OP_CHAIN) = range(22)

SYMBOLS = [
    "bsy_engine_create", "bsy_engine_destroy", "bsy_engine_load_weights", "bsy_plan_create", "bsy_plan_create_arena", "bsy_engine_arena_bytes", "bsy_plan_set_tuning", "bsy_plan_destroy",
    "bsy_plan_run", "bsy_plan_graph_launch", "bsy_plan_profile", "bsy_plan_copy_buffer", "bsy_plan_check_guards", "bsy_plan_autotune", "bsy_plan_get_tuning", "bsy_plan_check_tuning", "bsy_plan_autotune_in_place", "bsy_conv2d", "bsy_conv2d_f32", "bsy_conv2d_f32x", "bsy_conv_first_f32", "bsy_attention_f32", "bsy_conv_packed_dims", "bsy_conv_first", "bsy_stem_fused", "bsy_stem_fused_supported", "bsy_bottleneck_fused", "bsy_bottleneck_fused_supported", "bsy_c3k2_fused", "bsy_c3k2_fused_supported", "bsy_dwconv", "bsy_dwpw_fused", "bsy_dwpw_fused_supported", "bsy_ela", "bsy_ela_scratch_bytes", "bsy_dwconv3x3",
    "bsy_sppf_pool", "bsy_attention", "bsy_detect_decode", "bsy_nms_workspace_bytes", "bsy_nms", "bsy_scale_boxes",
    "bsy_letterbox", "bsy_process_mask", "bsy_process_mask_native", "bsy_scale_masks", "bsy_val_match", "bsy_pack_masks", "bsy_val_match_masks_workspace_bytes", "bsy_val_match_masks", "bsy_val_match_rotated", "bsy_slice_tiles", "bsy_sahi_merge_workspace_bytes",
    "bsy_sahi_merge", "bsy_scale_img", "bsy_tta_merge", "bsy_nms_rotated_workspace_bytes", "bsy_nms_rotated", "bsy_obb_scale", "bsy_end2end_topk_workspace_bytes", "bsy_end2end_topk", "bsy_ap_workspace_bytes", "bsy_ap_per_class", "bsy_last_error", "bsy_version", "bsy_sizeof_op",
]


class View(C.Structure):
    _fields_ = [("buf", C.c_int32), ("ld", C.c_int32), ("coff", C.c_int32), ("C", C.c_int32)]


NO_VIEW = (-1, 0, 0, 0)


class Op(C.Structure):
    _fields_ = [
        ("kind", C.c_int32),
        ("B", C.c_int32), ("H", C.c_int32), ("W", C.c_int32),
        ("OH", C.c_int32), ("OW", C.c_int32),
        ("src0", View), ("src1", View),
        ("up0", C.c_int32), ("up1", C.c_int32),
        ("dst", View), ("res", View),
        ("ksize", C.c_int32), ("stride", C.c_int32), ("pad", C.c_int32),
        ("act", C.c_int32), ("out_f32", C.c_int32),
        ("dst_scale", C.c_int32), ("dst_dy", C.c_int32), ("dst_dx", C.c_int32),
        ("w_off", C.c_int64), ("b_off", C.c_int64),
        ("heads", C.c_int32), ("key_dim", C.c_int32), ("head_dim", C.c_int32),
        ("scale", C.c_float),
        ("nl", C.c_int32), ("nc", C.c_int32), ("nm", C.c_int32), ("A", C.c_int32),
        ("box", View * 3), ("cls", View * 3), ("msk", View * 3),
        ("lvl_h", C.c_int32 * 3), ("lvl_w", C.c_int32 * 3),
        ("lvl_stride", C.c_float * 3),
        ("in_dtype", C.c_int32), ("out_dtype", C.c_int32),
        ("level", C.c_int32),
        ("lane", C.c_int32), ("tuned_cfg", C.c_int32), ("join", C.c_int32),
        ("mid_c", C.c_int32),
        ("w2_off", C.c_int64), ("b2_off", C.c_int64),
        ("aux_off", C.c_int64 * 18),
        ("prec", C.c_int32), ("ne", C.c_int32), ("ksplit", C.c_int32), ("reserved1", C.c_int32),
    ]


class BsyError(RuntimeError):
    pass


def _load() -> C.CDLL:
    if not LIB_PATH.exists():
        raise ImportError(
            f"{LIB_PATH} is missing: build it with `python -m bs_yolo_amd.build` (hipcc, gfx950). "
            "bs_yolo_amd has no CPU fallback.")
    if not os.environ.get("BSY_LIB") and os.environ.get("BSY_ALLOW_STALE_LIB") != "1":
        from .build import stale_sources
        stale = stale_sources()
        if stale:
            raise ImportError(f"{LIB_PATH} was not built from the current sources ({', '.join(stale)} changed or failed to compile): run "
                              "`python -m bs_yolo_amd.build` (BSY_ALLOW_STALE_LIB=1 loads it anyway)")
    lib = C.CDLL(str(LIB_PATH))
    missing = [s for s in SYMBOLS if not hasattr(lib, s)]
    if missing:
        raise ImportError(f"{LIB_PATH} does not export {missing}; rebuild it")
    if lib.bsy_sizeof_op() != C.sizeof(Op):
        raise ImportError(f"{LIB_PATH}: bsy_op is {lib.bsy_sizeof_op()} bytes in the library, {C.sizeof(Op)} in bs_yolo_amd/lib.py; rebuild it")
    vp, i32, i64, f32 = C.c_void_p, C.c_int, C.c_int64, C.c_float
    lib.bsy_last_error.restype = C.c_char_p
    lib.bsy_engine_create.argtypes = [i32, C.POINTER(vp)]
    lib.bsy_engine_destroy.argtypes = [vp]
    lib.bsy_engine_destroy.restype = None
    lib.bsy_engine_load_weights.argtypes = [vp, vp, C.c_size_t]
    lib.bsy_plan_create.argtypes = [vp, C.POINTER(Op), i32, C.POINTER(i64), i32, C.POINTER(vp)]
    lib.bsy_plan_create_arena.argtypes = [vp, C.POINTER(Op), i32, C.POINTER(i64), C.POINTER(i64), i32, i64, C.POINTER(vp)]
    lib.bsy_engine_arena_bytes.argtypes = [vp]
    lib.bsy_engine_arena_bytes.restype = C.c_size_t
    lib.bsy_plan_set_tuning.argtypes = [vp, C.POINTER(C.c_int32), i32]
    lib.bsy_plan_destroy.argtypes = [vp]
    lib.bsy_plan_destroy.restype = None
    lib.bsy_plan_run.argtypes = [vp, C.POINTER(vp), i32, vp]
    lib.bsy_plan_graph_launch.argtypes = [vp, C.POINTER(vp), i32, vp, C.POINTER(i32)]
    lib.bsy_plan_autotune.argtypes = [vp, C.POINTER(vp), i32, vp]
    lib.bsy_plan_get_tuning.argtypes = [vp, C.POINTER(C.c_int32), i32]
    lib.bsy_plan_check_tuning.argtypes = [vp, C.POINTER(vp), i32, C.POINTER(C.c_int32), i32]
    lib.bsy_plan_autotune_in_place.argtypes = [vp, C.POINTER(vp), i32, vp, i32]
    lib.bsy_plan_copy_buffer.argtypes = [vp, i32, vp, C.c_size_t]
    lib.bsy_plan_check_guards.argtypes = [vp, C.POINTER(C.c_int32), C.POINTER(C.c_int64)]
    lib.bsy_plan_profile.argtypes = [vp, C.POINTER(vp), i32, vp, C.POINTER(f32)]
    lib.bsy_conv2d.argtypes = [vp, i32, i32, i32, i32, i32, vp, vp, vp, i32, i32, i32, i32, i32, vp, i32, i32, vp]
    lib.bsy_conv2d_f32.argtypes = [vp, i32, i32, i32, i32, i32, vp, vp, vp, i32, i32, i32, i32, i32, vp, i32, i32, vp]
    lib.bsy_conv2d_f32x.argtypes = [vp, i32, i32, i32, i32, i32, vp, vp, i32, vp, vp, i32, i32, i32, i32, i32, vp, i32, vp]
    lib.bsy_conv_first_f32.argtypes = [vp, i32, i32, i32, i32, vp, vp, vp, i32, i32, i32, i32, i32, i32, vp]
    lib.bsy_attention_f32.argtypes = [vp, i32, i32, i32, i32, i32, i32, f32, vp, i32, i32, vp]
    lib.bsy_conv_packed_dims.argtypes = [i32, i32, i32, C.POINTER(i32), C.POINTER(i32)]
    lib.bsy_conv_first.argtypes = [vp, i32, i32, i32, i32, vp, vp, vp, i32, i32, i32, i32, i32, vp]
    lib.bsy_stem_fused.argtypes = [vp, i32, i32, i32, i32, vp, vp, i32, vp, vp, i32, vp, i32, i32, vp]
    lib.bsy_stem_fused_supported.argtypes = [i32, i32, i32, i32]
    lib.bsy_val_match.argtypes = [vp, i32, vp, i32, i32, vp, vp, vp, i32, C.POINTER(C.c_float), i32, vp, vp]
    lib.bsy_pack_masks.argtypes = [vp, i32, i32, i32, i32, vp, vp, vp]
    lib.bsy_val_match_masks_workspace_bytes.argtypes = [i32, i32, i32]
    lib.bsy_val_match_masks_workspace_bytes.restype = C.c_size_t
    lib.bsy_val_match_masks.argtypes = [vp, i32, vp, i32, i32, vp, vp, vp, vp, i32, vp, vp, i32, C.POINTER(C.c_float), i32, vp, vp, vp,
                                        C.c_size_t, vp]
    lib.bsy_val_match_rotated.argtypes = [vp, i32, vp, i32, i32, vp, vp, vp, i32, C.POINTER(C.c_float), i32, vp, vp, vp]
    lib.bsy_bottleneck_fused.argtypes = [vp, i32, i32, i32, i32, i32, i32, vp, vp, vp, vp, vp, i32, i32, vp]
    lib.bsy_bottleneck_fused_supported.argtypes = [i32, i32]
    lib.bsy_c3k2_fused.argtypes = [vp, i32, i32, i32, i32, i32, i32, i32, vp, vp, vp, vp, vp, vp, vp, vp, vp, i32, vp]
    lib.bsy_c3k2_fused_supported.argtypes = [i32, i32, i32]
    lib.bsy_dwconv.argtypes = [vp, i32, i32, i32, i32, i32, i32, i32, i32, vp, i32, vp, vp, i32, i32, vp]
    lib.bsy_ela_scratch_bytes.argtypes = [i32, i32, i32, i32]
    lib.bsy_dwpw_fused.argtypes = [vp, i32, i32, i32, i32, i32, vp, vp, vp, vp, vp, i32, i32, i32, vp]
    lib.bsy_dwpw_fused_supported.argtypes = [i32, i32]
    lib.bsy_ela_scratch_bytes.restype = C.c_size_t
    lib.bsy_ela.argtypes = [vp, i32, i32, i32, i32, i32, i32, vp, vp, vp, vp, C.POINTER(C.c_float), vp, vp, i32, vp]
    lib.bsy_dwconv3x3.argtypes = [vp, i32, i32, i32, i32, i32, vp, vp, vp, i32, i32, vp, i32, vp]
    lib.bsy_sppf_pool.argtypes = [vp, i32, i32, i32, i32, i32, vp]
    lib.bsy_attention.argtypes = [vp, i32, i32, i32, i32, i32, i32, f32, vp, i32, vp]
    lib.bsy_detect_decode.argtypes = [C.POINTER(vp), C.POINTER(i32), C.POINTER(vp), C.POINTER(i32), C.POINTER(vp),
                                      C.POINTER(i32), C.POINTER(i32), C.POINTER(i32), C.POINTER(f32), i32, i32, i32,
                                      i32, vp, i32, vp]
    lib.bsy_nms_workspace_bytes.argtypes = [i32, i32, i32, i32, i32]
    lib.bsy_nms_workspace_bytes.restype = C.c_size_t
    lib.bsy_nms.argtypes = [vp, i32, i32, i32, i32, i32, f32, f32, vp, i32, i32, i32, i32, i32, f32, i32, vp, vp, vp,
                            C.c_size_t, vp]
    lib.bsy_scale_boxes.argtypes = [vp, vp, i32, i32, i32, vp, vp, vp, vp, vp, vp]
    lib.bsy_nms_rotated_workspace_bytes.argtypes = [i32, i32, i32, i32, i32]
    lib.bsy_nms_rotated_workspace_bytes.restype = C.c_size_t
    lib.bsy_nms_rotated.argtypes = [vp, i32, i32, i32, i32, i32, f32, f32, vp, i32, i32, i32, i32, i32, f32, vp, vp, vp,
                                    C.c_size_t, vp]
    lib.bsy_obb_scale.argtypes = [vp, vp, i32, i32, i32, vp, vp, vp, vp, vp, vp]
    lib.bsy_end2end_topk_workspace_bytes.argtypes = [i32, i32, i32, i32]
    lib.bsy_end2end_topk_workspace_bytes.restype = C.c_size_t
    lib.bsy_end2end_topk.argtypes = [vp, i32, i32, i32, i32, i32, vp, vp, C.c_size_t, vp]
    lib.bsy_process_mask.argtypes = [vp, i32, i32, i32, i32, vp, i32, vp, i32, i32, i32, i32, i32, vp, vp, i32, vp]
    lib.bsy_process_mask_native.argtypes = [vp, i32, i32, i32, i32, vp, i32, vp, i32, i32, i32, i32, i32, i32, i32, i32, vp, vp, i32, vp]
    lib.bsy_scale_masks.argtypes = [vp, i32, i32, i32, i32, i32, i32, i32, i32, i32, i32, vp, vp]
    lib.bsy_letterbox.argtypes = [vp, vp, vp, i32, i32, i32, vp, i32, vp]
    lib.bsy_slice_tiles.argtypes = [vp, i32, i32, i32, vp, i32, i32, i32, i32, vp, i32, vp]
    lib.bsy_ap_workspace_bytes.argtypes = [i32, i32]
    lib.bsy_ap_workspace_bytes.restype = C.c_size_t
    lib.bsy_ap_per_class.argtypes = [vp, vp, vp, i32, i32, vp, vp, i32, vp, vp, C.c_double, vp, vp, vp, vp, vp, vp, C.c_size_t, vp]
    lib.bsy_sahi_merge_workspace_bytes.argtypes = [i32, i32]
    lib.bsy_sahi_merge_workspace_bytes.restype = C.c_size_t
    lib.bsy_sahi_merge.argtypes = [vp, vp, vp, i32, i32, i32, i32, f32, i32, i32, f32, f32, vp, vp, i32, vp, C.c_size_t, vp]
    lib.bsy_scale_img.argtypes = [vp, i32, i32, i32, i32, i32, i32, i32, i32, i32, i32, vp, vp]
    lib.bsy_tta_merge.argtypes = [C.POINTER(vp), C.POINTER(C.c_int32), C.POINTER(C.c_int32), C.POINTER(C.c_int32), C.POINTER(f32),
                                  C.POINTER(C.c_int32), i32, i32, i32, i32, i32, i32, vp, vp]
    return lib


lib = _load()


def check(rc: int) -> None:
    if rc != 0:
        raise BsyError(f"libbsyolo_hip: {lib.bsy_last_error().decode(errors='replace')} (status {rc})")


def dtype_code(t) -> int:
    import torch
    if t == torch.float16:
        return BSY_F16
    if t == torch.float32:
        return BSY_F32
    if t == torch.uint8:
        return BSY_U8
    raise TypeError(f"unsupported dtype {t}")
```

bs_yolo_amd/ops.py:

```python
from __future__ import annotations

import ctypes as C
from typing import List, Optional, Sequence

import torch

from . import lib as L


def _stream(t: torch.Tensor):
    return C.c_void_p(torch.cuda.current_stream(t.device).cuda_stream)


def _p(t: Optional[torch.Tensor]):
    return C.c_void_p(t.data_ptr()) if t is not None else None


def pack_conv_weight(w: torch.Tensor, b: Optional[torch.Tensor], device) -> tuple:
    cout, cin, k, _ = w.shape
    cp, kp = C.c_int(), C.c_int()
    L.check(L.lib.bsy_conv_packed_dims(cout, cin, k, C.byref(cp), C.byref(kp)))
    w = w.detach().float().cpu()
    if cin == 3:
        w = torch.cat([w, torch.zeros(cout, 1, k, k)], 1)
        cin = 4
    K = k * k * cin
    wp = torch.zeros(cp.value, kp.value, dtype=torch.float16)
    wp[:cout, :K] = w.permute(0, 2, 3, 1).reshape(cout, K).half()
    bp = torch.zeros(cp.value, dtype=torch.float32)
    if b is not None:
        bp[:cout] = b.detach().float().cpu()
    return wp.to(device), bp.to(device)


def conv2d_nhwc(x: torch.Tensor, wp: torch.Tensor, bp: torch.Tensor, cout: int, k: int, s: int = 1, act: bool = True,
                res: Optional[torch.Tensor] = None, out_f32: bool = False, cin: Optional[int] = None,
                out: Optional[torch.Tensor] = None) -> torch.Tensor:
    assert x.dtype == torch.float16 and x.is_contiguous() and x.dim() == 4
    B, H, W, ld = x.shape
    cin = ld if cin is None else cin
    p = k // 2
    OH, OW = (H + 2 * p - k) // s + 1, (W + 2 * p - k) // s + 1
    if out is None:
        ldy = (cout + 3) // 4 * 4 if out_f32 else (cout + 7) // 8 * 8
        out = torch.zeros((B, OH, OW, ldy), dtype=torch.float32 if out_f32 else torch.float16, device=x.device)
    L.check(L.lib.bsy_conv2d(_p(x), ld, B, H, W, cin, _p(wp), _p(bp), _p(out), out.shape[-1], cout, k, s, int(act),
                             _p(res), res.shape[-1] if res is not None else 0, int(out_f32), _stream(x)))
    return out


def conv2d_nhwc_f32(x: torch.Tensor, w: torch.Tensor, b: torch.Tensor, k: int, s: int = 1, act: bool = True,
                    res: Optional[torch.Tensor] = None, cin: Optional[int] = None, impl: int = 0) -> torch.Tensor:
    assert x.dtype == torch.float32 and x.is_contiguous() and x.dim() == 4
    B, H, W, ld = x.shape
    cin = ld if cin is None else cin
    cout = w.shape[0]
    assert tuple(w.shape) == (cout, cin, k, k)
    wk = w.detach().float().permute(2, 3, 1, 0).reshape(k * k * cin, cout).contiguous().to(x.device)
    bk = b.detach().float().contiguous().to(x.device)
    p = k // 2
    OH, OW = (H + 2 * p - k) // s + 1, (W + 2 * p - k) // s + 1
    ldy = (cout + 3) // 4 * 4
    out = torch.zeros((B, OH, OW, ldy), dtype=torch.float32, device=x.device)
    L.check(L.lib.bsy_conv2d_f32(_p(x), ld, B, H, W, cin, _p(wk), _p(bk), _p(out), ldy, cout, k, s, int(act), _p(res),
                                 res.shape[-1] if res is not None else 0, impl, _stream(x)))
    return out


def conv2d_nhwc_f32x(x: torch.Tensor, w: torch.Tensor, b: torch.Tensor, k: int, s: int = 1, act: bool = True,
                     res: Optional[torch.Tensor] = None, cin: Optional[int] = None) -> torch.Tensor:
    from .weights import split_f16_planes
    assert x.dtype == torch.float32 and x.is_contiguous() and x.dim() == 4
    B, H, W, ld = x.shape
    cin = ld if cin is None else cin
    cout = w.shape[0]
    assert tuple(w.shape) == (cout, cin, k, k)
    hi, lo = split_f16_planes(w.detach().float().cpu().permute(0, 2, 3, 1).reshape(cout, k * k * cin))
    hi, lo = hi.contiguous().to(x.device), lo.contiguous().to(x.device)
    bk = b.detach().float().contiguous().to(x.device)
    p = k // 2
    OH, OW = (H + 2 * p - k) // s + 1, (W + 2 * p - k) // s + 1
    ldy = (cout + 3) // 4 * 4
    out = torch.zeros((B, OH, OW, ldy), dtype=torch.float32, device=x.device)
    L.check(L.lib.bsy_conv2d_f32x(_p(x), ld, B, H, W, cin, _p(hi), _p(lo), hi.shape[1], _p(bk), _p(out), ldy, cout, k, s, int(act),
                                  _p(res), res.shape[-1] if res is not None else 0, _stream(x)))
    return out


def conv_first(img: torch.Tensor, w: torch.Tensor, b: torch.Tensor, k: int = 3, s: int = 2, act: bool = True):
    assert img.is_contiguous() and img.shape[1] == 3
    B, _, H, W = img.shape
    cout = w.shape[0]
    wp, bp = pack_conv_weight(w, b, img.device)
    p = k // 2
    OH, OW = (H + 2 * p - k) // s + 1, (W + 2 * p - k) // s + 1
    out = torch.empty((B, OH, OW, cout), dtype=torch.float16, device=img.device)
    L.check(L.lib.bsy_conv_first(_p(img), L.dtype_code(img.dtype), B, H, W, _p(wp), _p(bp), _p(out), cout, cout, k, s,
                                 int(act), _stream(img)))
    return out


def stem_fused(img: torch.Tensor, w0: torch.Tensor, b0: torch.Tensor, w1: torch.Tensor, b1: torch.Tensor,
               act: bool = True) -> torch.Tensor:
    assert img.is_contiguous() and img.shape[1] == 3
    B, _, H, W = img.shape
    c0, c1 = w0.shape[0], w1.shape[0]
    w0p, b0p = pack_conv_weight(w0, b0, img.device)
    w1p, b1p = pack_conv_weight(w1, b1, img.device)
    oh0, ow0 = (H - 1) // 2 + 1, (W - 1) // 2 + 1
    out = torch.empty((B, (oh0 - 1) // 2 + 1, (ow0 - 1) // 2 + 1, c1), dtype=torch.float16, device=img.device)
    L.check(L.lib.bsy_stem_fused(_p(img), L.dtype_code(img.dtype), B, H, W, _p(w0p), _p(b0p), c0, _p(w1p), _p(b1p), c1,
                                 _p(out), c1, int(act), _stream(img)))
    return out


def bottleneck_fused(x: torch.Tensor, w1: torch.Tensor, b1: torch.Tensor, w2: torch.Tensor, b2: torch.Tensor,
                     out: Optional[torch.Tensor] = None) -> torch.Tensor:
    B, H, W, c = x.shape
    assert x.stride(3) == 1 and x.stride(1) == W * x.stride(2) and x.stride(0) == H * W * x.stride(2)
    ch = w1.shape[0]
    w1p, b1p = pack_conv_weight(w1, b1, x.device)
    w2p, b2p = pack_conv_weight(w2, b2, x.device)
    if out is None:
        out = torch.empty((B, H, W, c), dtype=torch.float16, device=x.device)
    assert out.shape == x.shape and out.stride(3) == 1 and out.stride(1) == W * out.stride(2)
    L.check(L.lib.bsy_bottleneck_fused(_p(x), x.stride(2), B, H, W, c, ch, _p(w1p), _p(b1p), _p(w2p), _p(b2p), _p(out),
                                       out.stride(2), 1, _stream(x)))
    return out


def c3k2_fused(x: torch.Tensor, w1, b1, wa, ba, wb, bb, w4, b4, out: Optional[torch.Tensor] = None) -> torch.Tensor:
    B, H, W, cin = x.shape
    assert x.stride(3) == 1 and x.stride(1) == W * x.stride(2) and x.stride(0) == H * W * x.stride(2)
    c, c2 = wb.shape[0], w4.shape[0]
    packs = [pack_conv_weight(w, b, x.device) for w, b in ((w1, b1), (wa, ba), (wb, bb), (w4, b4))]
    if out is None:
        out = torch.empty((B, H, W, c2), dtype=torch.float16, device=x.device)
    assert out.shape == (B, H, W, c2) and out.stride(3) == 1 and out.stride(1) == W * out.stride(2)
    L.check(L.lib.bsy_c3k2_fused(_p(x), x.stride(2), B, H, W, cin, c, c2, _p(packs[0][0]), _p(packs[0][1]), _p(packs[1][0]),
                                 _p(packs[1][1]), _p(packs[2][0]), _p(packs[2][1]), _p(packs[3][0]), _p(packs[3][1]), _p(out),
                                 out.stride(2), _stream(x)))
    return out


def dwpw_fused(x: torch.Tensor, wd: torch.Tensor, bd: torch.Tensor, w: torch.Tensor, b: torch.Tensor, act: bool = True) -> torch.Tensor:
    B, H, W, Cc = x.shape
    c2 = w.shape[0]
    wdp = wd.detach().float().cpu().view(Cc, 9).t().contiguous().to(x.device)
    bdp = bd.detach().float().contiguous().to(x.device)
    wp, bp = pack_conv_weight(w, b, x.device)
    out = torch.empty((B, H, W, c2), dtype=torch.float16, device=x.device)
    L.check(L.lib.bsy_dwpw_fused(_p(x), Cc, B, H, W, Cc, _p(wdp), _p(bdp), _p(wp), _p(bp), _p(out), c2, c2, int(act), _stream(x)))
    return out


def dwconv_nhwc(x: torch.Tensor, w: torch.Tensor, b: torch.Tensor, stride: int = 1, act: bool = False) -> torch.Tensor:
    B, H, W, Cc = x.shape
    kh, kw = int(w.shape[2]), int(w.shape[3])
    wp = w.detach().float().cpu().view(Cc, kh * kw).t().contiguous().to(x.device)
    bp = b.detach().float().contiguous().to(x.device)
    OH, OW = (H + 2 * (kh // 2) - kh) // stride + 1, (W + 2 * (kw // 2) - kw) // stride + 1
    out = torch.empty((B, OH, OW, Cc), dtype=torch.float16, device=x.device)
    L.check(L.lib.bsy_dwconv(_p(x), Cc, B, H, W, Cc, kh, kw, stride, _p(wp), Cc, _p(bp), _p(out), Cc, int(act), _stream(x)))
    return out


def ela_nhwc(x: torch.Tensor, wsp: torch.Tensor, wch: torch.Tensor, gnw: torch.Tensor, gnb: torch.Tensor, coef) -> torch.Tensor:
    B, H, W, Cc = x.shape
    k = int(wsp.shape[-1])
    dev = x.device
    f = lambda t: t.detach().float().reshape(-1).contiguous().to(dev)
    a, b_, c, d = f(wsp), f(wch), f(gnw), f(gnb)
    scratch = torch.empty(int(L.lib.bsy_ela_scratch_bytes(B, H, W, Cc)) // 4, dtype=torch.float32, device=dev)
    out = torch.empty_like(x)
    cf = (C.c_float * 3)(*[float(v) for v in coef])
    L.check(L.lib.bsy_ela(_p(x), Cc, B, H, W, Cc, k, _p(a), _p(b_), _p(c), _p(d), cf, _p(scratch), _p(out), Cc, _stream(x)))
    return out


def dwconv3x3_nhwc(x: torch.Tensor, w: torch.Tensor, b: torch.Tensor, act: bool = True,
                   res: Optional[torch.Tensor] = None) -> torch.Tensor:
    B, H, W, Cc = x.shape
    wp = w.detach().float().cpu().view(Cc, 9).t().contiguous().to(x.device)
    bp = b.detach().float().contiguous().to(x.device)
    out = torch.empty_like(x)
    L.check(L.lib.bsy_dwconv3x3(_p(x), Cc, B, H, W, Cc, _p(wp), _p(bp), _p(out), Cc, int(act), _p(res),
                                res.shape[-1] if res is not None else 0, _stream(x)))
    return out


def sppf_pool_nhwc(x1: torch.Tensor) -> torch.Tensor:
    B, H, W, Cc = x1.shape
    buf = torch.zeros((B, H, W, 4 * Cc), dtype=torch.float16, device=x1.device)
    buf[..., :Cc] = x1
    L.check(L.lib.bsy_sppf_pool(_p(buf), 4 * Cc, B, H, W, Cc, _stream(x1)))
    return buf


def attention_nhwc(qkv: torch.Tensor, heads: int, key_dim: int, head_dim: int, scale: float) -> torch.Tensor:
    B, N, ld = qkv.shape
    out = torch.empty((B, N, heads * head_dim), dtype=torch.float16, device=qkv.device)
    L.check(L.lib.bsy_attention(_p(qkv), ld, B, N, heads, key_dim, head_dim, float(scale), _p(out), heads * head_dim,
                                _stream(qkv)))
    return out


def detect_decode(box: Sequence[torch.Tensor], cls: Sequence[torch.Tensor], hw: Sequence[tuple],
                  strides: Sequence[float], nc: int, out_dtype=torch.float32,
                  msk: Optional[Sequence[torch.Tensor]] = None) -> torch.Tensor:
    nl = len(box)
    B = box[0].shape[0] // (hw[0][0] * hw[0][1])
    nm = msk[0].shape[-1] if msk else 0
    A = sum(h * w for h, w in hw)
    y = torch.empty((B, 4 + nc + nm, A), dtype=out_dtype, device=box[0].device)
    vp, i32, f32 = C.c_void_p, C.c_int, C.c_float
    bp = (vp * nl)(*[t.data_ptr() for t in box])
    cp = (vp * nl)(*[t.data_ptr() for t in cls])
    mp = (vp * nl)(*[t.data_ptr() for t in msk]) if msk else None
    ldb = (i32 * nl)(*[t.shape[-1] for t in box])
    ldc = (i32 * nl)(*[t.shape[-1] for t in cls])
    ldm = (i32 * nl)(*[t.shape[-1] for t in msk]) if msk else None
    hh = (i32 * nl)(*[h for h, _ in hw])
    ww = (i32 * nl)(*[w for _, w in hw])
    st = (f32 * nl)(*[float(s) for s in strides])
    L.check(L.lib.bsy_detect_decode(bp, ldb, cp, ldc, mp, ldm, hh, ww, st, nl, B, nc, nm, _p(y), L.dtype_code(out_dtype),
                                    _stream(y)))
    return y


def scale_img(x: torch.Tensor, ratio: float, flip: Optional[int] = None, gs: int = 32,
              out: Optional[torch.Tensor] = None) -> torch.Tensor:
    from .tta import scaled_size
    assert x.is_contiguous() and x.dim() == 4 and x.dtype in (torch.float16, torch.float32)
    B, Cc, H, W = x.shape
    (oh, ow), (ph, pw) = scaled_size(H, W, ratio, gs)
    if out is None:
        out = torch.empty((B, Cc, ph, pw), dtype=x.dtype, device=x.device)
    assert out.is_contiguous() and tuple(out.shape) == (B, Cc, ph, pw) and out.dtype == x.dtype
    L.check(L.lib.bsy_scale_img(_p(x), L.dtype_code(x.dtype), B, Cc, H, W, oh, ow, ph, pw, int(flip or 0), _p(out), _stream(x)))
    return out


def tta_merge(ys: Sequence[torch.Tensor], windows: Sequence[tuple], scales: Sequence[float], flips: Sequence[Optional[int]],
              img_hw: tuple, out: Optional[torch.Tensor] = None) -> torch.Tensor:
    n = len(ys)
    y0 = ys[0]
    B, no = y0.shape[:2]
    for y in ys:
        assert y.is_contiguous() and y.dim() == 3 and tuple(y.shape[:2]) == (B, no) and y.dtype == y0.dtype and y.device == y0.device
    total = sum(e - b for b, e in windows)
    if out is None:
        out = torch.empty((B, no, total), dtype=y0.dtype, device=y0.device)
    assert out.is_contiguous() and tuple(out.shape) == (B, no, total) and out.dtype == y0.dtype
    i32 = C.c_int32
    L.check(L.lib.bsy_tta_merge((C.c_void_p * n)(*[y.data_ptr() for y in ys]), (i32 * n)(*[y.shape[2] for y in ys]),
                                (i32 * n)(*[b for b, _ in windows]), (i32 * n)(*[e for _, e in windows]),
                                (C.c_float * n)(*[float(s) for s in scales]), (i32 * n)(*[int(f or 0) for f in flips]), n, B, no,
                                int(img_hw[0]), int(img_hw[1]), L.dtype_code(y0.dtype), _p(out), _stream(out)))
    return out


def end2end_topk(pred: torch.Tensor, max_det: int = 300, out: Optional[torch.Tensor] = None,
                 workspace: Optional[torch.Tensor] = None) -> torch.Tensor:
    if not pred.is_cuda:
        raise RuntimeError("bs_yolo_amd.ops.end2end_topk needs a GPU tensor (no CPU fallback)")
    if pred.dim() != 3 or pred.shape[1] < 5:
        raise ValueError("pred must be (B, 4+nc, A)")
    pred = pred.contiguous()
    B, Cc, A = pred.shape
    nc = Cc - 4
    K = min(int(max_det), A)
    nbytes = L.lib.bsy_end2end_topk_workspace_bytes(B, A, nc, int(max_det))
    if workspace is None:
        workspace = torch.empty(max(nbytes, 1), dtype=torch.uint8, device=pred.device)
    if out is None:
        out = torch.empty((B, K, 6), dtype=torch.float32, device=pred.device)
    assert out.is_contiguous() and tuple(out.shape) == (B, K, 6) and out.dtype == torch.float32
    L.check(L.lib.bsy_end2end_topk(_p(pred), L.dtype_code(pred.dtype), B, nc, A, int(max_det), _p(out), _p(workspace),
                                   workspace.numel() * workspace.element_size(), _stream(pred)))
    return out
```

bs_yolo_amd/plan.py:

```python
from __future__ import annotations

import math
import os
from collections import OrderedDict
from dataclasses import dataclass, field
from typing import Dict, List, Optional, Sequence, Tuple, Union

from . import lib as L


def make_divisible(x, d):
    return math.ceil(x / d) * d


@dataclass
class T:
    buf: int
    ld: int
    coff: int
    C: int
    H: int
    W: int
    up: bool = False
    f32: bool = False
    cmap: Optional[Tuple[int, ...]] = None

    def slice(self, c0: int, c: int) -> "T":
        assert 0 <= c0 and c0 + c <= self.C
        cm = None
        if self.cmap is not None:
            before = sum(1 for v in self.cmap[:c0] if v >= 0)
            cm = tuple(v - before if v >= 0 else -1 for v in self.cmap[c0:c0 + c])
            if all(v >= 0 for v in cm):
                cm = None
        return T(self.buf, self.ld, self.coff + c0, c, self.H, self.W, self.up, self.f32, cm)

    @property
    def real(self) -> int:
        return self.C if self.cmap is None else sum(1 for v in self.cmap if v >= 0)

    def padded(self, pieces: Sequence[Tuple[int, int]]) -> "T":
        cm, base = [], 0
        for width, real in pieces:
            cm += [base + i if i < real else -1 for i in range(width)]
            base += real
        assert len(cm) == self.C
        return T(self.buf, self.ld, self.coff, self.C, self.H, self.W, self.up, self.f32, tuple(cm))

    def view(self):
        return (self.buf, self.ld, self.coff, self.C)


@dataclass
class WRec:
    name: str
    kind: str
    cout: int
    cin: int
    k: int
    perm: Optional[List[int]] = None
    tap: Optional[Tuple[int, int]] = None
    kw: Optional[int] = None
    post: Optional[str] = None
    coef: Tuple[float, float, float] = (0.0, 0.0, 0.0)
    real_cout: int = 0
    real_cin: int = 0
    rows: Optional[List[int]] = None
    cols: Optional[List[int]] = None
    w_off: int = -1
    b_off: int = -1


def stem_supported(c0: int, c1: int, H: int, W: int) -> bool:
    return (c0, c1) in ((32, 64), (16, 32)) and W % 4 == 0 and H >= 4 and W >= 4


def msca_spatial_supported(H: int, W: int) -> bool:
    return H > 0 and W > 0 and H * W <= 1890


def attention_supported(kd: int, hd: int) -> bool:
    return 0 < kd <= 64 and kd % 16 == 0 and 0 < hd <= 128 and hd % 32 == 0


def pmsfa_tail_supported(c: int) -> bool:
    return c in (32, 64)


def dwpw_supported(c: int, cout: int) -> bool:
    return c > 0 and c % 32 == 0 and c <= 256 and cout % 8 == 0


def c3k2_supported(cin: int, c: int, c2: int) -> bool:
    return (cin, c, c2) == (64, 32, 128)


def bneck_supported(c: int, ch: int) -> bool:
    return (c, ch) in ((32, 16), (64, 32))


class Plan:

    EXT_IMG, EXT_Y, EXT_RAW0 = 0, 1, 2
    EXT_PROTO = 5

    def __init__(self, cfg: dict, B: int, H: int, W: int, in_dtype: int = L.BSY_F16, out_dtype: int = L.BSY_F16,
                 fuse_stem: Optional[bool] = None, fuse_bneck: Optional[bool] = None, fuse_head: Optional[bool] = None,
                 fuse_dwpw: Optional[bool] = None, merge_c3k: Optional[bool] = None, fuse_msca: Optional[bool] = None,
                 fuse_tail: Optional[bool] = None, precision: str = "fp16", lanes: Optional[bool] = None, latency: bool = False,
                 fuse_pmsfa: Optional[bool] = None):
        self.cfg, self.B, self.H, self.W = cfg, B, H, W
        self.latency = bool(latency) and precision == "fp16"
        if precision not in ("fp16", "fp32", "fp32x"):
            raise ValueError(f"precision must be 'fp16', 'fp32' or 'fp32x', not {precision!r}")
        self.f32_mode = precision in ("fp32", "fp32x")
        self.split_f16 = precision == "fp32x"
        if self.f32_mode:
            fuse_stem = fuse_bneck = fuse_head = fuse_dwpw = merge_c3k = fuse_msca = fuse_tail = fuse_pmsfa = False
        self.in_dtype, self.out_dtype = in_dtype, out_dtype
        self.fuse_stem = (os.environ.get("BSY_FUSE_STEM", "1") != "0") if fuse_stem is None else bool(fuse_stem)
        self.fuse_bneck = (os.environ.get("BSY_FUSE_BNECK", "1") != "0") if fuse_bneck is None else bool(fuse_bneck)
        self.fuse_head = (os.environ.get("BSY_FUSE_HEAD", "1") != "0") if fuse_head is None else bool(fuse_head)
        self.fuse_boxtail = self.fuse_head and os.environ.get("BSY_FUSE_BOXTAIL", "1") != "0"
        self.fuse_dwpw = (os.environ.get("BSY_FUSE_DWPW", "1") != "0") if fuse_dwpw is None else bool(fuse_dwpw)
        self.merge_c3k = (os.environ.get("BSY_MERGE_C3K", "1") != "0") if merge_c3k is None else bool(merge_c3k)
        self.fuse_msca = (os.environ.get("BSY_FUSE_MSCA", "1") != "0") if fuse_msca is None else bool(fuse_msca)
        self.fuse_tail = (os.environ.get("BSY_FUSE_TAIL", "1") != "0") if fuse_tail is None else bool(fuse_tail)
        self.fuse_pmsfa = (os.environ.get("BSY_FUSE_PMSFA", "1") != "0") if fuse_pmsfa is None else bool(fuse_pmsfa)
        self.buf_bytes: List[int] = []
        self.ops: List[dict] = []
        self.wrecs: "OrderedDict[str, WRec]" = OrderedDict()
        self.flops = 0
        self.meta: Dict = {}
        self._lane = 0
        self._build()
        if self.latency:
            self._apply_split_k()
        env = os.environ.get("BSY_LANES")
        if env == "0" or (env is None and not lanes and (lanes is not None or B * H * W < 12 * 640 * 640)):
            for o in self.ops:
                if "lane" in o:
                    o["lane"] = 0
        assert all(o.get("lane", 0) == 0 or o["kind"] in (L.OP_CONV, L.OP_DWCONV, L.OP_BNECK, L.OP_DWCONV_G, L.OP_DWPW, L.OP_C3K2) for o in self.ops)

    @staticmethod
    def split_factors(k: int, stride: int, cin: int, c0: int, cout: int, OH: int, OW: int) -> Tuple[int, int]:
        if cin % 64 or c0 % 64 or cout % 8:
            return 1, 1
        steps = k * k * cin // 64
        tiles = -(-OH * OW // 128) * -(-cout // 128)
        want = min(32 // max(tiles, 1), 8, steps // 4)
        if steps < 32 or want < 3:
            return 1, 1
        nt = 3 if k == 3 else 1
        n64 = cin // 64
        nc = max((d for d in range(1, n64 + 1) if n64 % d == 0 and d * nt <= want), default=1)
        return (nc, nt) if nc * nt >= 3 else (1, 1)

    def _apply_split_k(self) -> None:
        for o in self.ops:
            if o["kind"] != L.OP_CONV or o.get("out_f32", 0) or o.get("dst_scale", 1) != 1 or o["ksize"] not in (1, 3):
                continue
            s0, s1 = o["src0"], o.get("src1")
            cin = s0.C + (s1.C if s1 else 0)
            cout = o.get("cout", o["dst"].C)
            if o["dst"].ld % 8 or (o.get("res") is not None and o["res"].ld % 8):
                continue
            nc, nt = self.split_factors(o["ksize"], o["stride"], cin, s0.C if s1 else cin, cout, o["OH"], o["OW"])
            if nc * nt < 2:
                continue
            ldw = (cout + 31) // 32 * 32
            self.buf_bytes.append(nc * nt * self.B * o["OH"] * o["OW"] * ldw * 4)
            o["box"] = [T(len(self.buf_bytes) - 1, ldw, 0, ldw, o["OH"], o["OW"], False, True)]
            o["ksplit"] = nc | (nt << 8)

    def alloc(self, C: int, H: int, W: int, f32: bool = False) -> T:
        if self.f32_mode:
            self.buf_bytes.append(self.B * H * W * make_divisible(C, 8) * 4)
            return T(len(self.buf_bytes) - 1, make_divisible(C, 8), 0, C, H, W, False, True)
        ld = make_divisible(C, 4) if f32 else make_divisible(C, 8)
        self.buf_bytes.append(self.B * H * W * ld * (4 if f32 else 2))
        return T(len(self.buf_bytes) - 1, ld, 0, C, H, W, False, f32)

    def _wrec(self, key: str, **kw) -> str:
        if key not in self.wrecs:
            self.wrecs[key] = WRec(**kw)
        return key

    def conv(self, name: str, src: Union[T, Sequence[T]], cout: int, k: int = 1, s: int = 1, act: bool = True,
             dst: Optional[T] = None, res: Optional[T] = None, plain: bool = False, out_f32: bool = False,
             perm: Optional[List[int]] = None, name2: Optional[str] = None, wkind: Optional[str] = None,
             wshape: Optional[Tuple[int, int, int]] = None, real: Tuple[int, int] = (0, 0),
             rows: Optional[List[int]] = None, cols: Optional[List[int]] = None) -> T:
        srcs = [src] if isinstance(src, T) else list(src)
        assert 1 <= len(srcs) <= 2, "at most two concat operands per conv"
        H, W = srcs[0].H, srcs[0].W
        assert all(t.H == H and t.W == W and (t.f32 == self.f32_mode) for t in srcs)
        cin = sum(t.C for t in srcs)
        if not self.f32_mode and any(t.C % 8 or t.coff % 8 for t in srcs):
            raise NotImplementedError(f"{name}: source channels / offsets {[(t.C, t.coff) for t in srcs]} are not multiples of 8 (fp16 path)")
        p = k // 2
        OH, OW = (H + 2 * p - k) // s + 1, (W + 2 * p - k) // s + 1
        if dst is None:
            dst = self.alloc(cout, OH, OW, out_f32)
        assert dst.C == cout and dst.H == OH and dst.W == OW and dst.f32 == (out_f32 or self.f32_mode) and not dst.up
        if res is not None:
            assert res.C == cout and res.H == OH and res.W == OW and not res.up
        if rows is None and cols is None and (any(t.cmap is not None for t in srcs) or dst.cmap is not None):
            assert perm is None and wshape is None and not real[1]
            out_real = real[0] or dst.real
            rows = list(dst.cmap) if dst.cmap is not None else [i if i < out_real else -1 for i in range(cout)]
            cols, base = [], 0
            for t in srcs:
                cols += [base + v if v >= 0 else -1 for v in (t.cmap if t.cmap is not None else range(t.C))]
                base += t.real
            real = (out_real, base)
            if real[0] < cout and dst.cmap is None:
                dst = dst.padded([(cout, real[0])])
        if name2 is not None:
            assert not plain and perm is None and cout % 2 == 0
            key = self._wrec(name + "+" + name2, name=name, kind="conv2", cout=cout, cin=cin, k=k, post=name2, rows=rows, cols=cols,
                             real_cout=real[0], real_cin=real[1])
        else:
            wc, wi, wk = wshape or (cout, cin, k)
            key = self._wrec(name, name=name, kind=wkind or ("plain" if plain else "conv"), cout=wc, cin=wi, k=wk, perm=perm,
                             real_cout=real[0], real_cin=real[1], rows=rows, cols=cols)
        self.ops.append(dict(kind=L.OP_CONV, H=H, W=W, OH=OH, OW=OW, src0=srcs[0],
                             src1=srcs[1] if len(srcs) > 1 else None, dst=dst, res=res, ksize=k, stride=s, pad=p,
                             act=int(act), out_f32=int(out_f32), wkey=key, dst_scale=1, name=name, lane=self._lane, cout=cout,
                             mfma_flops=2 * self.B * OH * OW * cout * cin * k * k))
        self.flops += 2 * self.B * OH * OW * cout * cin * k * k
        return dst

    def conv_first(self, name: str, cout: int, k: int, s: int, p: Optional[int] = None) -> T:
        p = k // 2 if p is None else p
        if (k, s, p) == (6, 2, 2) and not self.f32_mode:
            assert self.H % 2 == 0 and self.W % 2 == 0
            sd = self.alloc(16, self.H // 2, self.W // 2)
            self.ops.append(dict(kind=L.OP_S2D, H=self.H, W=self.W, OH=self.H // 2, OW=self.W // 2,
                                 src0=T(L.BSY_EXT_BASE + self.EXT_IMG, 0, 0, 3, self.H, self.W), dst=sd, in_dtype=self.in_dtype,
                                 name=name + ".s2d"))
            return self.conv(name, sd, cout, 3, 1, wkind="first_s2d", wshape=(cout, 3, 6))
        OH, OW = (self.H + 2 * p - k) // s + 1, (self.W + 2 * p - k) // s + 1
        dst = self.alloc(cout, OH, OW)
        key = self._wrec(name, name=name, kind="first", cout=cout, cin=3, k=k)
        self.ops.append(dict(kind=L.OP_CONV_FIRST, H=self.H, W=self.W, OH=OH, OW=OW,
                             src0=T(L.BSY_EXT_BASE + self.EXT_IMG, 0, 0, 3, self.H, self.W), dst=dst, ksize=k, stride=s,
                             pad=p, act=1, wkey=key, in_dtype=self.in_dtype, name=name,
                             mfma_flops=2 * self.B * OH * OW * cout * 3 * k * k))
        self.flops += 2 * self.B * OH * OW * cout * 3 * k * k
        return dst

    def dwconv(self, name: str, src: T, act: bool, dst: Optional[T] = None, res: Optional[T] = None, real_c: int = 0) -> T:
        assert not src.up
        if dst is None:
            dst = self.alloc(src.C, src.H, src.W)
        key = self._wrec(name, name=name, kind="dw", cout=src.C, cin=1, k=3, real_cout=real_c)
        self.ops.append(dict(kind=L.OP_DWCONV, H=src.H, W=src.W, OH=src.H, OW=src.W, src0=src, dst=dst, res=res,
                             ksize=3, stride=1, pad=1, act=int(act), wkey=key, name=name, lane=self._lane))
        self.flops += 2 * self.B * src.H * src.W * src.C * 9
        return dst

    def dwconv_g(self, name: str, src: T, kh: int, kw: int, s: int, act_c: int, dst: Optional[T] = None, kind: str = "dwg",
                 post: Optional[str] = None, rows: Optional[List[int]] = None, real_c: int = 0) -> T:
        assert not src.up and src.f32 == self.f32_mode
        OH, OW = (src.H + 2 * (kh // 2) - kh) // s + 1, (src.W + 2 * (kw // 2) - kw) // s + 1
        if dst is None:
            dst = self.alloc(src.C, OH, OW)
        assert dst.C == src.C and dst.H == OH and dst.W == OW
        key = self._wrec(name, name=name, kind=kind, cout=src.C, cin=1, k=kh, kw=kw, post=post, rows=rows, real_cout=real_c)
        self.ops.append(dict(kind=L.OP_DWCONV_G, H=src.H, W=src.W, OH=OH, OW=OW, src0=src, dst=dst, ksize=kh, pad=kw, stride=s,
                             act=int(act_c), wkey=key, heads=src.C, key_dim=0, name=name, lane=self._lane,
                             mid_c=src.C // 2 if kind == "dwg_ext" else 0))
        self.flops += 2 * self.B * OH * OW * src.C * kh * kw
        return dst

    def dwpw(self, name: str, src: T, cout: int, real: Tuple[int, int] = (0, 0)) -> T:
        if not (self.fuse_dwpw and dwpw_supported(src.C, cout) and not src.up):
            t = self.dwconv(name + ".0", src, act=True, real_c=real[1])
            return self.conv(name + ".1", t, cout, 1, 1, real=real)
        kd = self._wrec(name + ".0", name=name + ".0", kind="dw", cout=src.C, cin=1, k=3, real_cout=real[1])
# ... 307 lines not shown
                self._lane = 2 * len(xs) + i
                c4 = max(ch[0] // 4, nm)
                t = self.conv(f"{name}.cv4.{i}.0", x, c4, 3, 1)
                t = self.conv(f"{name}.cv4.{i}.1", t, c4, 3, 1)
                msks.append(self.conv(f"{name}.cv4.{i}.2", t, nm, 1, 1, act=False, plain=True, out_f32=True))
            if ne:
                self._lane = 2 * len(xs) + i
                c4 = max(ch[0] // 4, ne)
                t = self.conv(f"{name}.cv4.{i}.0", x, c4, 3, 1)
                t = self.conv(f"{name}.cv4.{i}.1", t, c4, 3, 1)
                msks.append(self.conv(f"{name}.cv4.{i}.2", t, make_divisible(ne, 8), 1, 1, act=False, plain=True, out_f32=True,
                                      real=(ne, 0)))
        self._lane = 0
        self.meta.update(A=A, nc=nc, nm=nm, ne=ne, no=64 + nc, strides=strides, levels=[(t.H, t.W) for t in xs])
        if fused:
            return
        self.ops.append(dict(kind=L.OP_DECODE, join=1, H=self.H, W=self.W, OH=0, OW=0, nl=len(xs), nc=nc, nm=nm, ne=ne, A=A, box=boxes,
                             cls=clss, msk=msks, lvl_h=[t.H for t in xs], lvl_w=[t.W for t in xs], lvl_stride=strides,
                             dst=T(L.BSY_EXT_BASE + self.EXT_Y, 0, 0, 4 + nc + nm + ne, 0, 0), out_dtype=self.out_dtype,
                             name=name + ".decode"))
        for i in range(len(xs)):
            self.ops.append(dict(kind=L.OP_RAW_NCHW, H=self.H, W=self.W, OH=0, OW=0, nl=len(xs), nc=nc, nm=0, A=A,
                                 box=boxes, cls=clss, msk=[], lvl_h=[t.H for t in xs], lvl_w=[t.W for t in xs],
                                 lvl_stride=strides, level=i,
                                 dst=T(L.BSY_EXT_BASE + self.EXT_RAW0 + i, 0, 0, 64 + nc, 0, 0),
                                 out_dtype=self.out_dtype, name=f"{name}.raw{i}"))
        self.meta.update(A=A, nc=nc, nm=nm, ne=ne, no=64 + nc, strides=strides, levels=[(t.H, t.W) for t in xs])

    def _build(self):
        d = self.cfg
        scales = d.get("scales")
        depth, width, max_ch = d.get("depth_multiple", 1.0), d.get("width_multiple", 1.0), float("inf")
        scale = d.get("scale")
        if scales:
            if not scale:
                scale = next(iter(scales))
            depth, width, max_ch = scales[scale]
        nc = d["nc"]
        if d.get("activation"):
            raise NotImplementedError("custom activation (tasks.py:956-957) is not accelerated")
        legacy = True
        outs: List = []
        chans: List[int] = []
        x = None
        layers = list(d["backbone"]) + list(d["head"])
        for i, (f, n, m, args) in enumerate(layers):
            name = f"model.{i}"
            args = [nc if a == "nc" else a for a in args]
            n = max(round(n * depth), 1) if n > 1 else n
            if f != -1:
                x = outs[f] if isinstance(f, int) else [x if j == -1 else outs[j] for j in f]
            if m in ("Conv", "C3k2", "C2f", "SPPF", "C2PSA", "C3k2_gai", "SCDown", "C3", "DWConv"):
                c2 = make_divisible(min(args[0], max_ch) * width, 8)
                if m == "Conv":
                    k = args[1] if len(args) > 1 else 1
                    s = args[2] if len(args) > 2 else 1
                    pad = args[3] if len(args) > 3 and args[3] is not None else k // 2
                    if i == 0:
                        if (k, s, pad) not in ((3, 2, 1), (6, 2, 2)):
                            raise NotImplementedError(f"image conv k={k} s={s} p={pad}: 3x3 s2 p1 or 6x6 s2 p2 only")
                        y = self.conv_first(name, c2, k, s, pad)
                    else:
                        assert isinstance(x, T)
                        if pad != k // 2:
                            raise NotImplementedError(f"Conv with padding {pad} != k // 2 is not accelerated")
                        y = self.conv(name, x, c2, k, s)
                elif m == "C3":
                    xs = x if isinstance(x, list) else x
                    shortcut = bool(args[1]) if len(args) > 1 else True
                    x0 = xs[0] if isinstance(xs, list) else xs
                    y = self.alloc(c2, x0.H, x0.W)
                    self.c3k(name, xs, y, n, shortcut, k=(1, 3))
                elif m == "DWConv":
                    assert isinstance(x, T)
                    k = args[1] if len(args) > 1 else 1
                    s = args[2] if len(args) > 2 else 1
                    if c2 != x.C:
                        raise NotImplementedError(f"DWConv {x.C} -> {c2}: only the depthwise case c1 == c2 is accelerated")
                    y = self.dwconv_g(name, x, k, k, s, x.C)
                elif m == "C3k2":
                    legacy = False
                    c3k = bool(args[1]) if len(args) > 1 else False
                    e = args[2] if len(args) > 2 else 0.5
                    if scale and scale in "mlx":
                        c3k = True
                    y = self.c2f(name, x, c2, n, True, e, "c3k" if c3k else "bottleneck")
                elif m == "C3k2_gai":
                    c3k = bool(args[1]) if len(args) > 1 else False
                    e = args[2] if len(args) > 2 else 0.5
                    y = self.c2f(name, x, c2, n, True, e, "c3k_gai" if c3k else "pmsfa")
                elif m == "SCDown":
                    assert isinstance(x, T)
                    y = self.scdown(name, x, c2, args[1], args[2])
                elif m == "C2f":
                    shortcut = bool(args[1]) if len(args) > 1 else False
                    y = self.c2f(name, x, c2, n, shortcut, 0.5, "c2f")
                elif m == "SPPF":
                    assert isinstance(x, T) and (len(args) < 2 or args[1] == 5)
                    y = self.sppf(name, x, c2)
                else:
                    assert isinstance(x, T)
                    y = self.c2psa(name, x, c2, n)
                cout = c2
            elif m == "MSCAAttention":
                assert isinstance(x, T)
                y = self.msca(name, x)
                cout = x.C
            elif m == "ELA":
                assert isinstance(x, T)
                y = self.ela(name, x)
                cout = x.C
            elif m == "nn.Upsample":
                assert isinstance(x, T) and not x.up and args[1] == 2 and args[2] == "nearest"
                y = T(x.buf, x.ld, x.coff, x.C, x.H * 2, x.W * 2, True, x.f32)
                cout = x.C
            elif m == "Concat":
                assert isinstance(x, list) and len(x) == 2, "only two-operand Concat feeding a conv is accelerated"
                for j, t in enumerate(x):
                    if isinstance(t, list):
                        assert all(isinstance(u, T) for u in t)
                        real = self.alloc(sum(u.C for u in t), t[0].H, t[0].W)
                        c0 = 0
                        for u in t:
                            self.copy(f"{name}.cat{j}", u, real.slice(c0, u.C))
                            c0 += u.C
                        x[j] = real
                assert all(isinstance(t, T) for t in x)
                y = list(x)
                cout = sum(t.C for t in x)
            elif m in ("Detect", "Segment", "OBB"):
                xs = x if isinstance(x, list) else [x]
                assert all(isinstance(t, T) for t in xs)
                if m == "Segment":
                    nm = args[1]
                    npr = make_divisible(min(args[2], max_ch) * width, 8)
                    self.proto(name + ".proto", xs[0], npr, nm)
                    self.detect(name, xs, args[0], legacy, nm=nm)
                elif m == "OBB":
                    ne = args[1] if len(args) > 1 and not isinstance(args[1], (list, tuple)) else 1
                    if ne != 1:
                        raise NotImplementedError(f"OBB with ne = {ne}: dist2rbox (utils/tal.py:404-423) decodes one angle")
                    self.detect(name, xs, args[0], legacy, ne=ne)
                else:
                    self.detect(name, xs, args[0], legacy)
                y, cout = None, 0
            else:
                raise NotImplementedError(f"module {m} is not on the accelerated path")
            outs.append(y)
            chans.append(cout)
            x = y
        self.layer_out = outs
        self.meta.update(scale=scale, n_layers=len(layers), legacy=legacy)
        self._fuse_stem()

    def _fuse_stem(self):
        if not self.fuse_stem or len(self.ops) < 2:
            return
        a, b = self.ops[0], self.ops[1]
        if a["kind"] != L.OP_CONV_FIRST or b["kind"] != L.OP_CONV:
            return
        mid = a["dst"]
        if (b["src0"] is not mid or b.get("src1") is not None or b.get("res") is not None or b["ksize"] != 3
                or b["stride"] != 2 or b["out_f32"] or not b["act"] or a["ksize"] != 3 or a["stride"] != 2):
            return
        if not stem_supported(mid.C, b["dst"].C, self.H, self.W):
            return
        for o in self.ops[2:]:
            for key in ("src0", "src1", "res"):
                t = o.get(key)
                if t is not None and t.buf == mid.buf:
                    return
        self.buf_bytes[mid.buf] = 16
        self.ops[0:2] = [dict(kind=L.OP_STEM, H=self.H, W=self.W, OH=b["OH"], OW=b["OW"], src0=a["src0"], dst=b["dst"],
                              ksize=3, stride=2, pad=1, act=1, wkey=a["wkey"], wkey2=b["wkey"], mid_c=mid.C,
                              in_dtype=self.in_dtype, name=a["name"] + "+" + b["name"].split(".")[-1], lane=0,
                              mfma_flops=a["mfma_flops"] + b["mfma_flops"])]
        self.layer_out[0] = None

    _VIEW_KEYS = ("src0", "src1", "dst", "res")
    _LIST_KEYS = ("box", "cls", "msk")

    def op_buffers(self, o: dict) -> List[int]:
        out = []
        for k in self._VIEW_KEYS:
            t = o.get(k)
            if t is not None and t.buf < L.BSY_EXT_BASE:
                out.append(t.buf)
        for k in self._LIST_KEYS:
            for t in o.get(k, []) or []:
                if t is not None and t.buf < L.BSY_EXT_BASE:
                    out.append(t.buf)
        return out

    def buffer_lifetimes(self) -> List[Optional[Tuple[int, int]]]:
        n = len(self.ops)
        life: List[Optional[List[int]]] = [None] * len(self.buf_bytes)
        for i, o in enumerate(self.ops):
            for b in self.op_buffers(o):
                if life[b] is None:
                    life[b] = [i, i]
                else:
                    life[b][1] = i
        i = 0
        while i < n:
            if self.ops[i].get("lane", 0) > 0:
                start = i
                end = n - 1
                for j in range(i + 1, n):
                    if self.ops[j].get("join", 0):
                        end = j
                        break
                for j in range(start, end + 1):
                    if self.ops[j].get("lane", 0) > 0:
                        for b in self.op_buffers(self.ops[j]):
                            life[b][0] = min(life[b][0], start)
                            life[b][1] = max(life[b][1], end)
                i = end + 1
            else:
                i += 1
        return [tuple(x) if x is not None else None for x in life]

    def assign_offsets(self, reuse: bool = True) -> Tuple[List[int], int]:
        sizes = [(b + 255) & ~255 for b in self.buf_bytes]
        offs = [0] * len(sizes)
        if not reuse:
            off = 0
            for i, sz in enumerate(sizes):
                offs[i] = off
                off += sz
            return offs, off
        life = self.buffer_lifetimes()
        placed: List[int] = []
        top = 0
        for i in sorted(range(len(sizes)), key=lambda k: (-sizes[k], k)):
            if life[i] is None or sizes[i] == 0:
                continue
            busy = sorted((offs[j], offs[j] + sizes[j]) for j in placed
                          if not (life[j][1] < life[i][0] or life[i][1] < life[j][0]))
            at = 0
            for lo, hi in busy:
                if at + sizes[i] <= lo:
                    break
                at = max(at, hi)
            offs[i] = at
            placed.append(i)
            top = max(top, at + sizes[i])
        return offs, top

    def conv_signature(self, o: dict) -> Optional[tuple]:
        if o["kind"] != L.OP_CONV or self.f32_mode:
            return None
        s0, s1, d, r = o["src0"], o.get("src1"), o["dst"], o.get("res")
        return (self.B, o["H"], o["W"], s0.C, s0.ld, int(s0.up), s1.C if s1 else 0, s1.ld if s1 else 0, int(s1.up) if s1 else 0,
                o.get("cout", d.C), d.ld, o["ksize"], o["stride"], int(r is not None), r.ld if r is not None else 0,
                o.get("out_f32", 0), o.get("dst_scale", 1), o.get("act", 0), o.get("ksplit", 0))

    def c_ops(self):
        arr = (L.Op * len(self.ops))()
        for o, d in zip(arr, self.ops):
            def v(t):
                return L.View(*(t.view() if t is not None else L.NO_VIEW))
            o.kind = d["kind"]
            o.B, o.H, o.W, o.OH, o.OW = self.B, d["H"], d["W"], d["OH"], d["OW"]
            o.src0, o.src1 = v(d.get("src0")), v(d.get("src1"))
            o.up0 = int(bool(d.get("src0") and d["src0"].up))
            o.up1 = int(bool(d.get("src1") and d["src1"].up))
            o.dst, o.res = v(d.get("dst")), v(d.get("res"))
            o.ksize, o.stride, o.pad = d.get("ksize", 0), d.get("stride", 0), d.get("pad", 0)
            o.act, o.out_f32 = d.get("act", 0), d.get("out_f32", 0)
            o.dst_scale, o.dst_dy, o.dst_dx = d.get("dst_scale", 1), d.get("dst_dy", 0), d.get("dst_dx", 0)
            if "wkey" in d:
                w = self.wrecs[d["wkey"]]
                assert w.w_off >= 0, "pack weights before serialising"
                o.w_off, o.b_off = w.w_off, w.b_off
            if "wkey2" in d:
                w = self.wrecs[d["wkey2"]]
                assert w.w_off >= 0, "pack weights before serialising"
                o.w2_off, o.b2_off = w.w_off, w.b_off
            o.mid_c = d.get("mid_c", 0)
            for j, k in enumerate(d.get("wkeys", [])):
                w = self.wrecs[k]
                assert w.w_off >= 0, "pack weights before serialising"
                o.aux_off[2 * j], o.aux_off[2 * j + 1] = w.w_off, w.b_off
            if d["kind"] == L.OP_ELA:
                cf = self.wrecs[d["wkey"]].coef
                d = dict(d, scale=cf[0], lvl_stride=[cf[1], cf[2]])
            o.heads, o.key_dim, o.head_dim, o.scale = d.get("heads", 0), d.get("key_dim", 0), d.get("head_dim", 0), \
                d.get("scale", 0.0)
            o.nl, o.nc, o.nm, o.A = d.get("nl", 0), d.get("nc", 0), d.get("nm", 0), d.get("A", 0)
            o.ne = d.get("ne", 0)
            for j in range(3):
                o.box[j] = v(d["box"][j] if j < len(d.get("box", [])) else None)
                o.cls[j] = v(d["cls"][j] if j < len(d.get("cls", [])) else None)
                o.msk[j] = v(d["msk"][j] if j < len(d.get("msk", [])) else None)
                o.lvl_h[j] = d["lvl_h"][j] if j < len(d.get("lvl_h", [])) else 0
                o.lvl_w[j] = d["lvl_w"][j] if j < len(d.get("lvl_w", [])) else 0
                o.lvl_stride[j] = d["lvl_stride"][j] if j < len(d.get("lvl_stride", [])) else 0.0
            o.in_dtype, o.out_dtype, o.level = d.get("in_dtype", 0), d.get("out_dtype", 0), d.get("level", 0)
            o.lane, o.join, o.tuned_cfg = d.get("lane", 0), d.get("join", 0), 0
            o.prec = (2 if self.split_f16 else 1) if self.f32_mode else 0
            o.ksplit = d.get("ksplit", 0)
        return arr
```

include/bsyolo.h:

```cpp
#ifndef BSYOLO_H
#define BSYOLO_H

#include <stddef.h>
#include <stdint.h>

#ifdef __cplusplus
extern "C" {
#endif

typedef void* bsy_stream;

enum bsy_status {
    BSY_OK = 0,
    BSY_ERR_ARG = -1,
    BSY_ERR_HIP = -2,
    BSY_ERR_ALLOC = -3,
    BSY_ERR_STATE = -4
};

enum bsy_dtype { BSY_F16 = 0, BSY_F32 = 1, BSY_U8 = 2 };

typedef struct bsy_engine bsy_engine;
typedef struct bsy_plan bsy_plan;

#define BSY_EXT_BASE 0x100000
typedef struct bsy_view {
    int32_t buf, ld, coff, C;
} bsy_view;

enum bsy_op_kind {
    BSY_OP_CONV_FIRST = 0,
    BSY_OP_CONV = 1,
    BSY_OP_DWCONV = 2,
    BSY_OP_SPPF_POOL = 3,
    BSY_OP_ATTN = 4,
    BSY_OP_DECODE = 5,
    BSY_OP_RAW_NCHW = 6,
    BSY_OP_NHWC2NCHW = 7,
    BSY_OP_STEM = 8,
    BSY_OP_BNECK = 9,
    BSY_OP_DWCONV_G = 10,
    BSY_OP_COPY = 11,
    BSY_OP_GAP = 12,
    BSY_OP_MSCA_MIX = 13,
    BSY_OP_MUL = 14,
    BSY_OP_DWPW = 16,
    BSY_OP_MSCA_SPATIAL = 17,
    BSY_OP_C3K2 = 18,
    BSY_OP_S2D = 19,
    BSY_OP_PMSFA_TAIL = 20,
    BSY_OP_ELA = 15
};

typedef struct bsy_op {
    int32_t kind;
    int32_t B, H, W;
    int32_t OH, OW;
    bsy_view src0, src1;
    int32_t up0, up1;
    bsy_view dst;
    bsy_view res;
    int32_t ksize, stride, pad;
    int32_t act;
    int32_t out_f32;
    int32_t dst_scale, dst_dy, dst_dx;
    int64_t w_off, b_off;
    int32_t heads, key_dim, head_dim;
    float scale;
    int32_t nl, nc, nm, A;
    bsy_view box[3], cls[3], msk[3];
    int32_t lvl_h[3], lvl_w[3];
    float lvl_stride[3];
    int32_t in_dtype, out_dtype;
    int32_t level;
    int32_t lane;
    int32_t tuned_cfg;
    int32_t join;
    int32_t mid_c;
    int64_t w2_off, b2_off;
    int64_t aux_off[18];
    int32_t prec;
    int32_t ne;
    int32_t ksplit;
    int32_t reserved1;
} bsy_op;

int bsy_sizeof_op(void);
int bsy_engine_create(int device, bsy_engine** out);
void bsy_engine_destroy(bsy_engine* e);
int bsy_engine_load_weights(bsy_engine* e, const void* host_blob, size_t bytes);

int bsy_plan_create(bsy_engine* e, const bsy_op* ops, int n_ops, const int64_t* buf_bytes, int n_bufs, bsy_plan** out);
int bsy_plan_create_arena(bsy_engine* e, const bsy_op* ops, int n_ops, const int64_t* buf_bytes, const int64_t* buf_off, int n_bufs,
                          int64_t arena_bytes, bsy_plan** out);
size_t bsy_engine_arena_bytes(const bsy_engine* e);
void bsy_plan_destroy(bsy_plan* p);
int bsy_plan_run(bsy_plan* p, void* const* ext, int n_ext, bsy_stream stream);
int bsy_plan_graph_launch(bsy_plan* p, void* const* ext, int n_ext, bsy_stream stream, int* captured);
int bsy_plan_autotune(bsy_plan* p, void* const* ext, int n_ext, bsy_stream stream);
int bsy_plan_set_tuning(bsy_plan* p, const int32_t* cfg, int n_ops);
int bsy_plan_get_tuning(bsy_plan* p, int32_t* out, int n_ops);
int bsy_plan_check_tuning(bsy_plan* p, void* const* ext, int n_ext, int32_t* valid, int n_ops);
int bsy_plan_autotune_in_place(bsy_plan* p, void* const* ext, int n_ext, bsy_stream stream, int rounds);
int bsy_plan_check_guards(bsy_plan* p, int32_t* bad_buf, int64_t* bad_off);
int bsy_plan_copy_buffer(bsy_plan* p, int buf, void* host_dst, size_t bytes);
int bsy_plan_profile(bsy_plan* p, void* const* ext, int n_ext, bsy_stream stream, float* ms_per_op );


int bsy_conv2d(const void* x, int ldx, int B, int H, int W, int C1, const void* w, const float* b, void* y, int ldy,
               int C2, int ksize, int stride, int act, const void* res, int ldr, int y_f32, bsy_stream stream);
int bsy_conv2d_f32(const float* x, int ldx, int B, int H, int W, int C1, const float* w, const float* b, float* y, int ldy,
                   int C2, int ksize, int stride, int act, const float* res, int ldr, int impl, bsy_stream stream);
int bsy_conv2d_f32x(const float* x, int ldx, int B, int H, int W, int C1, const void* w_hi, const void* w_lo, int k_pad,
                    const float* b, float* y, int ldy, int C2, int ksize, int stride, int act, const float* res, int ldr,
                    bsy_stream stream);
int bsy_conv_first_f32(const void* img, int img_dtype, int B, int H, int W, const float* w, const float* b, float* y, int ldy,
                       int C2, int ksize, int stride, int act, int impl, bsy_stream stream);
int bsy_attention_f32(const float* qkv, int ld, int B, int N, int heads, int key_dim, int head_dim, float scale, float* out,
                      int ldo, int impl, bsy_stream stream);
int bsy_conv_packed_dims(int C2, int C1, int ksize, int* cout_pad, int* k_pad);

int bsy_conv_first(const void* img, int img_dtype, int B, int H, int W, const void* w, const float* b, void* y,
                   int ldy, int C2, int ksize, int stride, int act, bsy_stream stream);

int bsy_stem_fused(const void* img, int img_dtype, int B, int H, int W, const void* w0, const float* b0, int C0,
                   const void* w1, const float* b1, int C1, void* y, int ldy, int act, bsy_stream stream);
int bsy_stem_fused_supported(int C0, int C1, int H, int W);

int bsy_bottleneck_fused(const void* x, int ldx, int B, int H, int W, int C, int CH, const void* w1, const float* b1,
                         const void* w2, const float* b2, void* y, int ldy, int act, bsy_stream stream);
int bsy_bottleneck_fused_supported(int C, int CH);
int bsy_c3k2_fused(const void* x, int ldx, int B, int H, int W, int Cin, int c, int C2, const void* w1, const float* b1, const void* wa,
                   const float* ba, const void* wb, const float* bb, const void* w4, const float* b4, void* y, int ldy, bsy_stream stream);
int bsy_c3k2_fused_supported(int Cin, int c, int C2);

int bsy_dwconv(const void* x, int ldx, int B, int H, int W, int C, int kh, int kw, int stride, const float* w, int wld,
               const float* b, void* y, int ldy, int act, bsy_stream stream);
size_t bsy_ela_scratch_bytes(int B, int H, int W, int C);
int bsy_ela(const void* x, int ldx, int B, int H, int W, int C, int k, const float* wsp, const float* wch,
            const float* gnw, const float* gnb, const float* coef, void* scratch, void* y, int ldy, bsy_stream stream);

int bsy_dwpw_fused(const void* x, int ldx, int B, int H, int W, int C, const float* dww, const float* dwb, const void* w,
                   const float* b, void* y, int ldy, int C2, int act, bsy_stream stream);
int bsy_dwpw_fused_supported(int C, int C2);

int bsy_dwconv3x3(const void* x, int ldx, int B, int H, int W, int C, const float* w, const float* b, void* y, int ldy,
                  int act, const void* res, int ldr, bsy_stream stream);

int bsy_sppf_pool(void* buf, int ld, int B, int H, int W, int C, bsy_stream stream);

int bsy_attention(const void* qkv, int ld, int B, int N, int heads, int key_dim, int head_dim, float scale, void* out,
                  int ldo, bsy_stream stream);

int bsy_detect_decode(const float* const* box, const int* ldb, const float* const* cls, const int* ldc,
                      const float* const* msk, const int* ldm, const int* lvl_h, const int* lvl_w,
                      const float* lvl_stride, int nl, int B, int nc, int nm, void* y, int y_dtype, bsy_stream stream);

size_t bsy_nms_workspace_bytes(int B, int A, int nc, int multi_label, int max_nms);
int bsy_nms(void* pred, int pred_dtype, int B, int nc, int nm, int A, float conf_thres, float iou_thres,
            const int32_t* classes, int n_classes, int agnostic, int multi_label, int max_det, int max_nms,
            float max_wh, int in_place, float* out, int32_t* counts, void* workspace, size_t workspace_bytes,
            bsy_stream stream);

size_t bsy_nms_rotated_workspace_bytes(int B, int A, int nc, int multi_label, int max_nms);
int bsy_nms_rotated(void* pred, int pred_dtype, int B, int nc, int ne, int A, float conf_thres, float iou_thres,
                    const int32_t* classes, int n_classes, int agnostic, int multi_label, int max_det, int max_nms,
                    float max_wh, float* out, int32_t* counts, void* workspace, size_t workspace_bytes, bsy_stream stream);
int bsy_obb_scale(float* det, const int32_t* counts, int B, int max_det, int row, const float* gain, const float* pad_x,
                  const float* pad_y, const float* h0, const float* w0, bsy_stream stream);

size_t bsy_end2end_topk_workspace_bytes(int B, int A, int nc, int max_det);
int bsy_end2end_topk(const void* pred, int pred_dtype, int B, int nc, int A, int max_det, float* out, void* workspace,
                     size_t workspace_bytes, bsy_stream stream);

int bsy_scale_boxes(float* det, const int32_t* counts, int B, int max_det, int row, const float* gain,
                    const float* pad_x, const float* pad_y, const float* h0, const float* w0, bsy_stream stream);

int bsy_letterbox(const uint8_t* const* imgs, const int32_t* hw, const int32_t* geom, int B, int H2, int W2, void* out,
                  int out_dtype, bsy_stream stream);

int bsy_process_mask(const void* protos, int proto_dtype, int nm, int mh, int mw, const float* coef, int ldc,
                     const float* boxes, int ldb, int n, int ih, int iw, int upsample, float* lowres, void* out,
                     int out_dtype, bsy_stream stream);

int bsy_process_mask_native(const void* protos, int proto_dtype, int nm, int mh, int mw, const float* coef, int ldc,
                            const float* boxes, int ldb, int n, int top, int left, int bottom, int right, int oh, int ow,
                            float* lowres, void* out, int out_dtype, bsy_stream stream);
int bsy_scale_masks(const void* masks, int dtype, int n, int mh, int mw, int top, int left, int bottom, int right, int oh, int ow,
                    void* out, bsy_stream stream);

int bsy_val_match(const float* det, int row, const int32_t* counts, int B, int max_det, const float* gt_boxes,
                  const float* gt_cls, const int32_t* gt_counts, int Lmax, const float* iouv, int n_iou,
                  unsigned char* out, bsy_stream stream);

int bsy_pack_masks(const void* masks, int dtype, int n, int hw, int label_map, uint64_t* planes, int32_t* areas, bsy_stream stream);
size_t bsy_val_match_masks_workspace_bytes(int B, int max_det, int Lmax);
int bsy_val_match_masks(const float* det, int row, const int32_t* counts, int B, int max_det, const uint64_t* pred_planes,
                        const int32_t* pred_areas, const uint64_t* gt_planes, const int32_t* gt_areas, int words,
                        const float* gt_cls, const int32_t* gt_counts, int Lmax, const float* iouv, int n_iou, unsigned char* out,
                        float* iou_out, void* workspace, size_t workspace_bytes, bsy_stream stream);
int bsy_val_match_rotated(const float* det, int row, const int32_t* counts, int B, int max_det, const float* gt_rboxes,
                          const float* gt_cls, const int32_t* gt_counts, int Lmax, const float* iouv, int n_iou, unsigned char* out,
                          float* iou_out, bsy_stream stream);

size_t bsy_ap_workspace_bytes(int N, int T);
int bsy_ap_per_class(const uint8_t* tp, const float* conf, const float* pred_cls, int N, int T, const int32_t* classes,
                     const int32_t* nt, int nc, const double* x101, const double* x1000, double eps, double* ap, double* p_curve,
                     double* r_curve, double* prec_values, int32_t* n_pred, void* workspace, size_t workspace_bytes,
                     bsy_stream stream);

int bsy_slice_tiles(const uint8_t* img, int H, int W, int pitch, const int32_t* boxes, int T, int th, int tw,
                    int swap_rb, void* out, int out_dtype, bsy_stream stream);
size_t bsy_sahi_merge_workspace_bytes(int T, int max_det);
int bsy_sahi_merge(const float* det, const int32_t* counts, const float* shift, int T, int max_det, int row,
                   int match_metric, float match_threshold, int class_agnostic, int do_merge, float full_w,
                   float full_h, float* out, int32_t* out_count, int max_out, void* workspace, size_t workspace_bytes,
                   bsy_stream stream);

#define BSY_TTA_MAX_PASSES 8
int bsy_scale_img(const void* in, int dtype, int B, int C, int H, int W, int OH, int OW, int PH, int PW, int flip, void* out,
                  bsy_stream stream);
int bsy_tta_merge(const void* const* src, const int32_t* A, const int32_t* a_begin, const int32_t* a_end, const float* scale,
                  const int32_t* flip, int n, int B, int no, int img_h, int img_w, int dtype, void* out, bsy_stream stream);

const char* bsy_last_error(void);
int bsy_version(void);

#ifdef __cplusplus
}
#endif
#endif
```

Measured before the change: 20820.

## Fold C3k2 cv1 1x1 conv into stem epilogue, add pre-activated C3k2 path

Moves the first C3k2 block's cv1 pointwise conv (64->64) into the fused stem kernel as an extra MFMA epilogue on the output tile held in LDS. The C3k2 kernel gains a PRE variant that loads already-activated y0|y1 straight into LDS, skipping its stage-1 GEMM and its weight staging. The goal is to cut the cv1 work and halo recompute in the C3k2 kernel and to shrink its LDS footprint. The trade is more LDS and compute in the stem kernel, plus an extra barrier there.

New measurement: 20670. No clear change (-0.7%).

```diff
diff --git a/bs_yolo_amd/csrc/c3k2_fused.hip b/bs_yolo_amd/csrc/c3k2_fused.hip
--- a/bs_yolo_amd/csrc/c3k2_fused.hip
+++ b/bs_yolo_amd/csrc/c3k2_fused.hip
@@ -19,7 +19,7 @@
     TileGrid grid;
 };
 
-template <int CIN, int C, int C2>
+template <int CIN, int C, int C2, bool PRE>
 __global__ __launch_bounds__(256, 3) void c3k2_fused_kernel(const C3k2K p) {
     constexpr int CH = C / 2;
     constexpr int YS = C + 8, MS = CH + 8, OS = C2 + 8;
@@ -30,8 +30,10 @@
     constexpr int SOUT = CK_NPX * OS;
     static_assert(SOUT <= SY1 + SY0, "output tile must fit the y1 + y0 tiles it aliases");
     constexpr int SWA = CH * WAS, SWB = C * WBS;
-    constexpr int W0S = CIN + 8, SW0 = C * W0S;
-    __shared__ __attribute__((aligned(16))) half_t lds[SY1 + SY0 + SM + SY2 + SWA + SWB + SW0 + 2 * (2 * C + CH + C + C2)];
+    constexpr int W0S = CIN + 8, SW0 = PRE ? 0 : C * W0S;
+    constexpr int NB1 = PRE ? 0 : 2 * C;
+    static_assert(!PRE || CIN == 2 * C, "pre-activated input = [y0 | y1]");
+    __shared__ __attribute__((aligned(16))) half_t lds[SY1 + SY0 + SM + SY2 + SWA + SWB + SW0 + 2 * (NB1 + CH + C + C2)];
     half_t* sy1 = lds;
     half_t* sy0 = sy1 + SY1;
     half_t* sout = lds;
@@ -41,7 +43,7 @@
     half_t* swb = swa + SWA;
     half_t* sw0 = swb + SWB;
     float* sb1 = reinterpret_cast<float*>(sw0 + SW0);
-    float* sba = sb1 + 2 * C;
+    float* sba = sb1 + NB1;
     float* sbb = sba + CH;
     float* sb4 = sbb + C;
 
@@ -49,16 +51,19 @@
     const int wave = __builtin_amdgcn_readfirstlane(tid >> 6);
     const int lrow = lane & 31, lh = lane >> 5;
 
-    for (int i = tid; i < 2 * C; i += 256) sb1[i] = p.b1[i];
+    if constexpr (!PRE)
+        for (int i = tid; i < 2 * C; i += 256) sb1[i] = p.b1[i];
     if (tid < CH) sba[tid] = p.ba[tid];
     if (tid < C) sbb[tid] = p.bb[tid];
     for (int i = tid; i < C2; i += 256) sb4[i] = p.b4[i];
     half8 w1y1[KS1], a4[3 * KSEG];
-#pragma unroll
-    for (int ks = 0; ks < KS1; ++ks) w1y1[ks] = *reinterpret_cast<const half8*>(p.w1 + (size_t)(C + lrow) * p.K1 + 16 * ks + 8 * lh);
-    for (int i = tid; i < C * (CIN / 8); i += 256) {
-        const int row = i / (CIN / 8), ch = i - row * (CIN / 8);
-        *reinterpret_cast<half8*>(sw0 + row * W0S + ch * 8) = *reinterpret_cast<const half8*>(p.w1 + (size_t)row * p.K1 + ch * 8);
+    if constexpr (!PRE) {
+#pragma unroll
+        for (int ks = 0; ks < KS1; ++ks) w1y1[ks] = *reinterpret_cast<const half8*>(p.w1 + (size_t)(C + lrow) * p.K1 + 16 * ks + 8 * lh);
+        for (int i = tid; i < C * (CIN / 8); i += 256) {
+            const int row = i / (CIN / 8), ch = i - row * (CIN / 8);
+            *reinterpret_cast<half8*>(sw0 + row * W0S + ch * 8) = *reinterpret_cast<const half8*>(p.w1 + (size_t)row * p.K1 + ch * 8);
+        }
     }
 #pragma unroll
     for (int ks = 0; ks < 3 * KSEG; ++ks) a4[ks] = *reinterpret_cast<const half8*>(p.w4 + (size_t)(32 * wave + lrow) * p.K4 + 16 * ks + 8 * lh);
@@ -81,10 +86,33 @@
     const int eB = b_y0 ? (2 * (wave - 1) + lty + 2) * CK_XC + ltx + 2 : 128 + lrow, rB = eB / CK_XC, cB = eB - rB * CK_XC;
     const unsigned relA = (unsigned)((rA * p.W + cA) * p.lds + 8 * lh), relB = (unsigned)((rB * p.W + cB) * p.lds + 8 * lh);
     half8 xa[KS1], xb[KS1];
+    constexpr int NPY = (CK_NX * (C / 8) + 255) / 256;
+    static_assert(CK_NPX * (C / 8) == 256, "one y0 piece per thread");
+    half8 pre[NPY + 1];
+    int pr_r[NPY + 1], pr_c[NPY + 1];
+    unsigned pr_rel[NPY + 1];
+#pragma unroll
+    for (int i = 0; i < NPY; ++i) {
+        const int idx = tid + 256 * i, e = (idx >> 2) < CK_NX ? idx >> 2 : CK_NX - 1;
+        pr_r[i] = e / CK_XC; pr_c[i] = e - pr_r[i] * CK_XC;
+        pr_rel[i] = (unsigned)((pr_r[i] * p.W + pr_c[i]) * p.lds + C + 8 * (idx & 3));
+    }
+    pr_r[NPY] = 2 + (tid >> 2) / CK_TW; pr_c[NPY] = 2 + (tid >> 2) % CK_TW;
+    pr_rel[NPY] = (unsigned)((pr_r[NPY] * p.W + pr_c[NPY]) * p.lds + 8 * (tid & 3));
     int nn = 0, noy0 = 0, nox0 = 0;
     auto fetch = [&](int tile) {
         tile_origin(tile, nn, noy0, nox0);
         const half_t* tb = p.src + ((long long)(nn * p.H + noy0 - 2) * p.W + (nox0 - 2)) * p.lds;
+        if constexpr (PRE) {
+#pragma unroll
+            for (int i = 0; i <= NPY; ++i) {
+                const bool in = (i == NPY || tid + 256 * i < CK_NX * (C / 8)) && (unsigned)(noy0 - 2 + pr_r[i]) < (unsigned)p.H &&
+                                (unsigned)(nox0 - 2 + pr_c[i]) < (unsigned)p.W;
+                pre[i] = half8{0, 0, 0, 0, 0, 0, 0, 0};
+                if (in) pre[i] = *reinterpret_cast<const half8*>(tb + pr_rel[i]);
+            }
+            return;
+        }
         const bool inA = (unsigned)(noy0 - 2 + rA) < (unsigned)p.H && (unsigned)(nox0 - 2 + cA) < (unsigned)p.W;
         const bool inB = wave < 3 && (unsigned)(noy0 - 2 + rB) < (unsigned)p.H && (unsigned)(nox0 - 2 + cB) < (unsigned)p.W;
 #pragma unroll
@@ -109,6 +137,13 @@
     for (; tile < tw.end; tile += tw.step) {
         const int n = nn, oy0 = noy0, ox0 = nox0;
         half_t* ob = p.dst + ((long long)(n * p.H + oy0) * p.W + ox0) * p.ldd;
+        if constexpr (PRE) {
+#pragma unroll
+            for (int i = 0; i < NPY; ++i)
+                if (tid + 256 * i < CK_NX * (C / 8))
+                    *reinterpret_cast<half8*>(sy1 + ((tid + 256 * i) >> 2) * YS + 8 * (tid & 3)) = pre[i];
+            *reinterpret_cast<half8*>(sy0 + (tid >> 2) * YS + 8 * (tid & 3)) = pre[NPY];
+        } else {
         auto s1_job = [&](const bool is_y0, const half8 (&wf)[KS1], const half8 (&xf)[KS1], const int e, const int r, const int c, const int opix) {
             f32x16 acc;
             acc_bias(acc, sb1 + (is_y0 ? 0 : C), lh);
@@ -137,6 +172,7 @@
 #pragma unroll
             for (int ks = 0; ks < KS1; ++ks) w1y0[ks] = *reinterpret_cast<const half8*>(sw0 + wo + 16 * ks);
             s1_job(true, w1y0, xb, eB, rB, cB, 32 * (wave - 1) + lrow);
+        }
         }
         if (tile + tw.step < tw.end) fetch(tile + tw.step);
         lds_barrier();
@@ -239,9 +275,9 @@
 int launch_c3k2_fused(const C3k2Args& a, hipStream_t s) {
     if (!c3k2_fused_supported(a.Cin, a.C, a.C2)) BSY_FAIL(BSY_ERR_ARG, "c3k2: unsupported widths (Cin %d, c %d, C2 %d): need (64, 32, 128)", a.Cin, a.C, a.C2);
     if (a.B <= 0 || a.H <= 0 || a.W <= 0) BSY_FAIL(BSY_ERR_ARG, "c3k2: bad extent");
-    const void* ptrs[10] = {a.src, a.dst, a.w1, a.wa, a.wb, a.w4, a.b1, a.ba, a.bb, a.b4};
-    for (const void* q : ptrs)
-        if (!q || ((uintptr_t)q & 15)) BSY_FAIL(BSY_ERR_ARG, "c3k2: null or misaligned pointer");
+    const void* ptrs[10] = {a.src, a.dst, a.wa, a.wb, a.w4, a.ba, a.bb, a.b4, a.w1, a.b1};
+    for (int i = 0; i < (a.pre ? 8 : 10); ++i)
+        if (const void* q = ptrs[i]; !q || ((uintptr_t)q & 15)) BSY_FAIL(BSY_ERR_ARG, "c3k2: null or misaligned pointer");
     if ((a.lds & 7) || (a.ldd & 7) || a.lds < a.Cin || a.ldd < a.C2) BSY_FAIL(BSY_ERR_ARG, "c3k2: bad leading dimension");
     C3k2K k;
     k.src = a.src; k.dst = a.dst; k.w1 = (const half_t*)a.w1; k.wa = (const half_t*)a.wa; k.wb = (const half_t*)a.wb; k.w4 = (const half_t*)a.w4;
@@ -255,7 +291,8 @@
     const int rc = make_tile_grid(k.grid, a.B, a.H, a.W, CK_TH, CK_TW, "c3k2");
     if (rc != BSY_OK) return rc;
     const int grid = k.grid.ntiles < 768 ? k.grid.ntiles : 768;
-    hipLaunchKernelGGL((c3k2_fused_kernel<64, 32, 128>), dim3(grid), dim3(256), 0, s, k);
+    if (a.pre) hipLaunchKernelGGL((c3k2_fused_kernel<64, 32, 128, true>), dim3(grid), dim3(256), 0, s, k);
+    else hipLaunchKernelGGL((c3k2_fused_kernel<64, 32, 128, false>), dim3(grid), dim3(256), 0, s, k);
     HIP_TRY(hipGetLastError());
     return BSY_OK;
 }
diff --git a/bs_yolo_amd/csrc/common.h b/bs_yolo_amd/csrc/common.h
--- a/bs_yolo_amd/csrc/common.h
+++ b/bs_yolo_amd/csrc/common.h
@@ -85,8 +85,12 @@
     int C0, C1, Kpad1;
     half_t* dst;
     int ldd, act;
+    const void* wc = nullptr;
+    const float* bc = nullptr;
+    int Cc = 0;
 };
 bool stem_fused_supported(int C0, int C1, int H, int W);
+bool stem_cv1_supported(int C0, int C1, int Cc);
 int launch_stem_fused(const StemArgs& a, hipStream_t s);
 
 struct BneckArgs {
@@ -110,6 +114,7 @@
     const float *b1, *ba, *bb, *b4;
     half_t* dst;
     int ldd;
+    int pre = 0;
 };
 bool c3k2_fused_supported(int Cin, int C, int C2);
 int launch_c3k2_fused(const C3k2Args& a, hipStream_t s);
diff --git a/bs_yolo_amd/csrc/engine.hip b/bs_yolo_amd/csrc/engine.hip
--- a/bs_yolo_amd/csrc/engine.hip
+++ b/bs_yolo_amd/csrc/engine.hip
@@ -376,6 +376,9 @@
             int cp = 0;
             bsy_conv_packed_dims(a.C1, a.C0, 3, &cp, &a.Kpad1);
             a.dst = R.h(op.dst); a.ldd = op.dst.ld; a.act = op.act;
+            if (op.fold_cv1) {
+                a.wc = (const void*)(wb + op.aux_off[0]); a.bc = (const float*)(wb + op.aux_off[1]); a.Cc = op.dst.C;
+            }
             if (!R.ok) return BSY_ERR_ARG;
             return launch_stem_fused(a, s);
         }
@@ -407,6 +410,8 @@
             a.wb = wb + op.aux_off[4]; a.bb = (const float*)(wb + op.aux_off[5]);
             a.w4 = wb + op.aux_off[6]; a.b4 = (const float*)(wb + op.aux_off[7]);
             a.dst = R.h(op.dst); a.ldd = op.dst.ld;
+            a.pre = op.fold_cv1 ? 1 : 0;
+            if (a.pre && op.src0.C != 2 * op.mid_c) BSY_FAIL(BSY_ERR_ARG, "c3k2: pre-activated input must be 2c = %d channels wide, not %d", 2 * op.mid_c, op.src0.C);
             if (!R.ok) return BSY_ERR_ARG;
             return launch_c3k2_fused(a, s);
         }
@@ -949,6 +954,24 @@
     return launch_stem_fused(a, (hipStream_t)stream);
 }
 
+extern "C" int bsy_stem_cv1_fused(const void* img, int img_dtype, int B, int H, int W, const void* w0, const float* b0, int C0,
+                                  const void* w1, const float* b1, int C1, const void* wc, const float* bc, int Cc, void* y, int ldy,
+                                  bsy_stream stream) {
+    if (!img || !w0 || !b0 || !w1 || !b1 || !wc || !bc || !y) BSY_FAIL(BSY_ERR_ARG, "stem: null pointer");
+    StemArgs a;
+    a.img = img; a.img_dtype = img_dtype; a.B = B; a.H = H; a.W = W;
+    const int OH0 = (H - 1) / 2 + 1, OW0 = (W - 1) / 2 + 1;
+    a.OH = (OH0 - 1) / 2 + 1; a.OW = (OW0 - 1) / 2 + 1;
+    a.w0 = w0; a.b0 = b0; a.w1 = w1; a.b1 = b1; a.C0 = C0; a.C1 = C1;
+    int cp = 0;
+    bsy_conv_packed_dims(C1, C0, 3, &cp, &a.Kpad1);
+    a.dst = (half_t*)y; a.ldd = ldy; a.act = 1;
+    a.wc = wc; a.bc = bc; a.Cc = Cc;
+    return launch_stem_fused(a, (hipStream_t)stream);
+}
+
+extern "C" int bsy_stem_cv1_supported(int C0, int C1, int Cc) { return stem_cv1_supported(C0, C1, Cc) ? 1 : 0; }
+
 extern "C" int bsy_stem_fused_supported(int C0, int C1, int H, int W) { return stem_fused_supported(C0, C1, H, W) ? 1 : 0; }
 
 extern "C" int bsy_bottleneck_fused(const void* x, int ldx, int B, int H, int W, int C, int CH, const void* w1,
@@ -975,6 +998,15 @@
     a.src = (const half_t*)x; a.lds = ldx; a.B = B; a.H = H; a.W = W; a.Cin = Cin; a.C = c; a.C2 = C2;
     a.w1 = w1; a.b1 = b1; a.wa = wa; a.ba = ba; a.wb = wb; a.bb = bb; a.w4 = w4; a.b4 = b4;
     a.dst = (half_t*)y; a.ldd = ldy;
+    return launch_c3k2_fused(a, (hipStream_t)stream);
+}
+
+extern "C" int bsy_c3k2_preact(const void* y01, int ldx, int B, int H, int W, int c, int C2, const void* wa, const float* ba,
+                               const void* wb, const float* bb, const void* w4, const float* b4, void* y, int ldy, bsy_stream stream) {
+    C3k2Args a;
+    a.src = (const half_t*)y01; a.lds = ldx; a.B = B; a.H = H; a.W = W; a.Cin = 2 * c; a.C = c; a.C2 = C2;
+    a.w1 = nullptr; a.b1 = nullptr; a.wa = wa; a.ba = ba; a.wb = wb; a.bb = bb; a.w4 = w4; a.b4 = b4;
+    a.dst = (half_t*)y; a.ldd = ldy; a.pre = 1;
     return launch_c3k2_fused(a, (hipStream_t)stream);
 }
 
diff --git a/bs_yolo_amd/csrc/stem_fused.hip b/bs_yolo_amd/csrc/stem_fused.hip
--- a/bs_yolo_amd/csrc/stem_fused.hip
+++ b/bs_yolo_amd/csrc/stem_fused.hip
@@ -22,9 +22,12 @@
     half_t* dst;
     int B, H, W, OH0, OW0, OH1, OW1, ldd, Kpad1, act;
     TileGrid grid;
+    const half_t* wc;
+    const float* bc;
+    int Kc;
 };
 
-template <typename T, int C0, int C1>
+template <typename T, int C0, int C1, bool CV1>
 __global__ __launch_bounds__(256, sizeof(T) == 4 ? 2 : 3) void stem_fused_kernel(const StemK p) {
     constexpr int NCH = C0 / 8;
     constexpr int KS1 = (9 * C0 + 15) / 16;
@@ -35,12 +38,18 @@
     constexpr int OUT = ST_TH * ST_TW * LDO;
     static_assert(C0 == 16 || C0 == 32, "layer-0 width");
     static_assert(NH == 1 || NH == 2, "layer-1 width");
-    __shared__ __attribute__((aligned(16))) half_t lds[IMG + MID + OUT + 2 * (C0 + C1)];
+    constexpr int WCS = C1 + 8;
+    constexpr int SWC = CV1 ? C1 * WCS + 2 * C1 : 0;
+    static_assert(!CV1 || (C1 == 64 && OUT <= MID), "cv1 epilogue: 64 -> 64, result tile aliases the layer-0 patch");
+    __shared__ __attribute__((aligned(16))) half_t lds[IMG + MID + OUT + 2 * (C0 + C1) + SWC];
     half_t* simg = lds;
     half_t* smid = lds + IMG;
     half_t* sout = smid + MID;
     float* sb0 = reinterpret_cast<float*>(sout + OUT);
     float* sb1 = sb0 + C0;
+    float* sbc = sb1 + C1;
+    half_t* swc = reinterpret_cast<half_t*>(sbc + C1);
+    half_t* sres = smid;
 
     const int tid = threadIdx.x, lane = tid & 63;
     const int wave = __builtin_amdgcn_readfirstlane(tid >> 6);
@@ -49,6 +58,13 @@
 
     if (tid < C0) sb0[tid] = p.b0[tid];
     if (tid < C1) sb1[tid] = p.b1[tid];
+    if constexpr (CV1) {
+        if (tid < C1) sbc[tid] = p.bc[tid];
+        for (int i = tid; i < C1 * (C1 / 8); i += 256) {
+            const int row = i / (C1 / 8), ch = i - row * (C1 / 8);
+            *reinterpret_cast<half8*>(swc + row * WCS + ch * 8) = *reinterpret_cast<const half8*>(p.wc + (size_t)row * p.Kc + ch * 8);
+        }
+    }
     half8 a0[IMGC_KSUB];
 #pragma unroll
     for (int s = 0; s < IMGC_KSUB; ++s)
@@ -155,6 +171,30 @@
         }
         lds_barrier();
 
+        if constexpr (CV1) {
+            int wo = (nh1 * 32 + lrow) * WCS + 8 * lh;
+            asm volatile("" : "+v"(wo));
+            const half_t* xb = sout + (mt1 * 32 + lrow) * LDO + 8 * lh;
+            f32x16 acc;
+            acc_bias(acc, sbc + nh1 * 32, lh);
+#pragma unroll
+            for (int ks = 0; ks < C1 / 16; ++ks)
+                acc = __builtin_amdgcn_mfma_f32_32x32x16_f16(*reinterpret_cast<const half8*>(swc + wo + 16 * ks),
+                                                             *reinterpret_cast<const half8*>(xb + 16 * ks), acc, 0, 0, 0);
+            const int prow = mt1 * 32 + lrow;
+#pragma unroll
+            for (int g = 0; g < 4; ++g) {
+                const int c = nh1 * 32 + 8 * g + 4 * lh;
+                half4 o;
+                const f32x4 t = silu4_f(f32x4{acc[4 * g], acc[4 * g + 1], acc[4 * g + 2], acc[4 * g + 3]});
+#pragma unroll
+                for (int q = 0; q < 4; ++q) o[q] = (half_t)t[q];
+                *reinterpret_cast<half4*>(sres + prow * LDO + c) = o;
+            }
+            lds_barrier();
+        }
+        const half_t* stile = CV1 ? sres : sout;
+
         constexpr int CPRW = C1 / 8;
 #pragma unroll
         for (int id = tid; id < ST_TH * ST_TW * CPRW; id += 256) {
@@ -162,7 +202,7 @@
             const int oy = oy0 + prow / ST_TW, ox = ox0 + prow % ST_TW;
             if (oy < p.OH1 && ox < p.OW1)
                 *reinterpret_cast<half8*>(p.dst + ((size_t)(n * p.OH1 + oy) * p.OW1 + ox) * p.ldd + cc) =
-                    *reinterpret_cast<const half8*>(sout + prow * LDO + cc);
+                    *reinterpret_cast<const half8*>(stile + prow * LDO + cc);
         }
     }
 }
@@ -170,13 +210,16 @@
 bool stem_fused_supported(int C0, int C1, int H, int W) {
     return ((C0 == 32 && C1 == 64) || (C0 == 16 && C1 == 32)) && !(W & 3) && H >= 4 && W >= 4;
 }
+
+bool stem_cv1_supported(int C0, int C1, int Cc) { return C0 == 32 && C1 == 64 && Cc == 64; }
 
 template <typename T>
 static int launch_t(const StemArgs& a, const StemK& k, hipStream_t s) {
     const int slots = sizeof(T) == 4 ? 512 : 768;
     const int grid = k.grid.ntiles < slots ? k.grid.ntiles : slots;
-    if (a.C0 == 32) hipLaunchKernelGGL((stem_fused_kernel<T, 32, 64>), dim3(grid), dim3(256), 0, s, k);
-    else hipLaunchKernelGGL((stem_fused_kernel<T, 16, 32>), dim3(grid), dim3(256), 0, s, k);
+    if (k.wc) hipLaunchKernelGGL((stem_fused_kernel<T, 32, 64, true>), dim3(grid), dim3(256), 0, s, k);
+    else if (a.C0 == 32) hipLaunchKernelGGL((stem_fused_kernel<T, 32, 64, false>), dim3(grid), dim3(256), 0, s, k);
+    else hipLaunchKernelGGL((stem_fused_kernel<T, 16, 32, false>), dim3(grid), dim3(256), 0, s, k);
     HIP_TRY(hipGetLastError());
     return BSY_OK;
 }
@@ -195,6 +238,14 @@
     k.img = a.img; k.w0 = (const half_t*)a.w0; k.b0 = a.b0; k.w1 = (const half_t*)a.w1; k.b1 = a.b1; k.dst = a.dst;
     k.B = a.B; k.H = a.H; k.W = a.W; k.OH0 = OH0; k.OW0 = OW0; k.OH1 = OH1; k.OW1 = OW1; k.ldd = a.ldd; k.Kpad1 = a.Kpad1;
     k.act = a.act;
+    k.wc = nullptr; k.bc = nullptr; k.Kc = 0;
+    if (a.wc || a.bc) {
+        if (!stem_cv1_supported(a.C0, a.C1, a.Cc)) BSY_FAIL(BSY_ERR_ARG, "stem: cv1 epilogue needs (C0, C1, Cc) = (32, 64, 64), got (%d, %d, %d)", a.C0, a.C1, a.Cc);
+        if (!a.wc || !a.bc || ((uintptr_t)a.wc & 15) || ((uintptr_t)a.bc & 15) || !a.act) BSY_FAIL(BSY_ERR_ARG, "stem: cv1 epilogue: null / misaligned weights, or act = 0");
+        int cp = 0;
+        bsy_conv_packed_dims(a.Cc, a.C1, 1, &cp, &k.Kc);
+        k.wc = (const half_t*)a.wc; k.bc = a.bc;
+    }
     const int rc = make_tile_grid(k.grid, a.B, OH1, OW1, ST_TH, ST_TW, "stem");
     if (rc != BSY_OK) return rc;
     if (a.img_dtype == BSY_F16) return launch_t<half_t>(a, k, s);
diff --git a/bs_yolo_amd/engine.py b/bs_yolo_amd/engine.py
--- a/bs_yolo_amd/engine.py
+++ b/bs_yolo_amd/engine.py
@@ -22,7 +22,7 @@
                  fuse_bneck: Optional[bool] = None, fuse_head: Optional[bool] = None, fuse_dwpw: Optional[bool] = None,
                  merge_c3k: Optional[bool] = None, fuse_msca: Optional[bool] = None, fuse_tail: Optional[bool] = None,
                  max_plans: Optional[int] = None, precision: str = "fp16", graph: Optional[bool] = None, graph_ring: int = 3,
-                 latency: Optional[bool] = None, fuse_pmsfa: Optional[bool] = None):
+                 latency: Optional[bool] = None, fuse_pmsfa: Optional[bool] = None, fuse_stem_cv1: Optional[bool] = None):
         if not torch.cuda.is_available():
             raise RuntimeError("bs_yolo_amd needs a ROCm GPU (there is no CPU fallback)")
         self.cfg = cfg
@@ -68,6 +68,7 @@
         self.fuse_msca = fuse_msca
         self.fuse_tail = fuse_tail
         self.fuse_pmsfa = fuse_pmsfa
+        self.fuse_stem_cv1 = fuse_stem_cv1
         self._packed = Plan(cfg, 1, 64, 64, **self._fuse_kw())
         blob = pack_plan_weights(self._packed, state_dict, bn_eps)
         self.weight_bytes = len(blob)
@@ -92,7 +93,7 @@
         return dict(fuse_stem=self.fuse_stem, fuse_bneck=self.fuse_bneck, fuse_head=self.fuse_head, fuse_dwpw=self.fuse_dwpw,
                     merge_c3k=self.merge_c3k, fuse_msca=self.fuse_msca, fuse_tail=self.fuse_tail, precision=self.precision,
                     lanes=True if getattr(self, "graph", False) else None, latency=getattr(self, "latency", False),
-                    fuse_pmsfa=self.fuse_pmsfa)
+                    fuse_pmsfa=self.fuse_pmsfa, fuse_stem_cv1=self.fuse_stem_cv1)
 
     def plan_for(self, B: int, H: int, W: int, in_dtype: torch.dtype, out_dtype: torch.dtype):
         key = (B, H, W, in_dtype, out_dtype)
diff --git a/bs_yolo_amd/lib.py b/bs_yolo_amd/lib.py
--- a/bs_yolo_amd/lib.py
+++ b/bs_yolo_amd/lib.py
@@ -15,7 +15,7 @@
 
 SYMBOLS = [
     "bsy_engine_create", "bsy_engine_destroy", "bsy_engine_load_weights", "bsy_plan_create", "bsy_plan_create_arena", "bsy_engine_arena_bytes", "bsy_plan_set_tuning", "bsy_plan_destroy",
-    "bsy_plan_run", "bsy_plan_graph_launch", "bsy_plan_profile", "bsy_plan_copy_buffer", "bsy_plan_check_guards", "bsy_plan_autotune", "bsy_plan_get_tuning", "bsy_plan_check_tuning", "bsy_plan_autotune_in_place", "bsy_conv2d", "bsy_conv2d_f32", "bsy_conv2d_f32x", "bsy_conv_first_f32", "bsy_attention_f32", "bsy_conv_packed_dims", "bsy_conv_first", "bsy_stem_fused", "bsy_stem_fused_supported", "bsy_bottleneck_fused", "bsy_bottleneck_fused_supported", "bsy_c3k2_fused", "bsy_c3k2_fused_supported", "bsy_dwconv", "bsy_dwpw_fused", "bsy_dwpw_fused_supported", "bsy_ela", "bsy_ela_scratch_bytes", "bsy_dwconv3x3",
+    "bsy_plan_run", "bsy_plan_graph_launch", "bsy_plan_profile", "bsy_plan_copy_buffer", "bsy_plan_check_guards", "bsy_plan_autotune", "bsy_plan_get_tuning", "bsy_plan_check_tuning", "bsy_plan_autotune_in_place", "bsy_conv2d", "bsy_conv2d_f32", "bsy_conv2d_f32x", "bsy_conv_first_f32", "bsy_attention_f32", "bsy_conv_packed_dims", "bsy_conv_first", "bsy_stem_fused", "bsy_stem_fused_supported", "bsy_stem_cv1_fused", "bsy_stem_cv1_supported", "bsy_c3k2_preact", "bsy_bottleneck_fused", "bsy_bottleneck_fused_supported", "bsy_c3k2_fused", "bsy_c3k2_fused_supported", "bsy_dwconv", "bsy_dwpw_fused", "bsy_dwpw_fused_supported", "bsy_ela", "bsy_ela_scratch_bytes", "bsy_dwconv3x3",
     "bsy_sppf_pool", "bsy_attention", "bsy_detect_decode", "bsy_nms_workspace_bytes", "bsy_nms", "bsy_scale_boxes",
     "bsy_letterbox", "bsy_process_mask", "bsy_process_mask_native", "bsy_scale_masks", "bsy_val_match", "bsy_pack_masks", "bsy_val_match_masks_workspace_bytes", "bsy_val_match_masks", "bsy_val_match_rotated", "bsy_slice_tiles", "bsy_sahi_merge_workspace_bytes",
     "bsy_sahi_merge", "bsy_scale_img", "bsy_tta_merge", "bsy_nms_rotated_workspace_bytes", "bsy_nms_rotated", "bsy_obb_scale", "bsy_end2end_topk_workspace_bytes", "bsy_end2end_topk", "bsy_ap_workspace_bytes", "bsy_ap_per_class", "bsy_last_error", "bsy_version", "bsy_sizeof_op",
@@ -54,6 +54,7 @@
         ("w2_off", C.c_int64), ("b2_off", C.c_int64),
         ("aux_off", C.c_int64 * 18),
         ("prec", C.c_int32), ("ne", C.c_int32), ("ksplit", C.c_int32), ("reserved1", C.c_int32),
+        ("fold_cv1", C.c_int32), ("reserved2", C.c_int32),
     ]
 
 
@@ -109,6 +110,9 @@
     lib.bsy_conv_first.argtypes = [vp, i32, i32, i32, i32, vp, vp, vp, i32, i32, i32, i32, i32, vp]
     lib.bsy_stem_fused.argtypes = [vp, i32, i32, i32, i32, vp, vp, i32, vp, vp, i32, vp, i32, i32, vp]
     lib.bsy_stem_fused_supported.argtypes = [i32, i32, i32, i32]
+    lib.bsy_stem_cv1_fused.argtypes = [vp, i32, i32, i32, i32, vp, vp, i32, vp, vp, i32, vp, vp, i32, vp, i32, vp]
+    lib.bsy_stem_cv1_supported.argtypes = [i32, i32, i32]
+    lib.bsy_c3k2_preact.argtypes = [vp, i32, i32, i32, i32, i32, i32, vp, vp, vp, vp, vp, vp, vp, i32, vp]
     lib.bsy_val_match.argtypes = [vp, i32, vp, i32, i32, vp, vp, vp, i32, C.POINTER(C.c_float), i32, vp, vp]
     lib.bsy_pack_masks.argtypes = [vp, i32, i32, i32, i32, vp, vp, vp]
     lib.bsy_val_match_masks_workspace_bytes.argtypes = [i32, i32, i32]
diff --git a/bs_yolo_amd/ops.py b/bs_yolo_amd/ops.py
--- a/bs_yolo_amd/ops.py
+++ b/bs_yolo_amd/ops.py
@@ -114,6 +114,21 @@
     return out
 
 
+def stem_cv1_fused(img: torch.Tensor, w0: torch.Tensor, b0: torch.Tensor, w1: torch.Tensor, b1: torch.Tensor, wc: torch.Tensor,
+                   bc: torch.Tensor) -> torch.Tensor:
+    assert img.is_contiguous() and img.shape[1] == 3
+    B, _, H, W = img.shape
+    c0, c1, cc = w0.shape[0], w1.shape[0], wc.shape[0]
+    w0p, b0p = pack_conv_weight(w0, b0, img.device)
+    w1p, b1p = pack_conv_weight(w1, b1, img.device)
+    wcp, bcp = pack_conv_weight(wc, bc, img.device)
+    oh0, ow0 = (H - 1) // 2 + 1, (W - 1) // 2 + 1
+    out = torch.empty((B, (oh0 - 1) // 2 + 1, (ow0 - 1) // 2 + 1, cc), dtype=torch.float16, device=img.device)
+    L.check(L.lib.bsy_stem_cv1_fused(_p(img), L.dtype_code(img.dtype), B, H, W, _p(w0p), _p(b0p), c0, _p(w1p), _p(b1p), c1, _p(wcp), _p(bcp),
+                                     cc, _p(out), cc, _stream(img)))
+    return out
+
+
 def bottleneck_fused(x: torch.Tensor, w1: torch.Tensor, b1: torch.Tensor, w2: torch.Tensor, b2: torch.Tensor,
                      out: Optional[torch.Tensor] = None) -> torch.Tensor:
     B, H, W, c = x.shape
@@ -140,6 +155,20 @@
     L.check(L.lib.bsy_c3k2_fused(_p(x), x.stride(2), B, H, W, cin, c, c2, _p(packs[0][0]), _p(packs[0][1]), _p(packs[1][0]),
                                  _p(packs[1][1]), _p(packs[2][0]), _p(packs[2][1]), _p(packs[3][0]), _p(packs[3][1]), _p(out),
                                  out.stride(2), _stream(x)))
+    return out
+
+
+def c3k2_preact(y01: torch.Tensor, wa, ba, wb, bb, w4, b4, out: Optional[torch.Tensor] = None) -> torch.Tensor:
+    B, H, W, cin = y01.shape
+    assert y01.stride(3) == 1 and y01.stride(1) == W * y01.stride(2) and y01.stride(0) == H * W * y01.stride(2)
+    c, c2 = wb.shape[0], w4.shape[0]
+    assert cin == 2 * c
+    packs = [pack_conv_weight(w, b, y01.device) for w, b in ((wa, ba), (wb, bb), (w4, b4))]
+    if out is None:
+        out = torch.empty((B, H, W, c2), dtype=torch.float16, device=y01.device)
+    assert out.shape == (B, H, W, c2) and out.stride(3) == 1 and out.stride(1) == W * out.stride(2)
+    L.check(L.lib.bsy_c3k2_preact(_p(y01), y01.stride(2), B, H, W, c, c2, _p(packs[0][0]), _p(packs[0][1]), _p(packs[1][0]), _p(packs[1][1]),
+                                  _p(packs[2][0]), _p(packs[2][1]), _p(out), out.stride(2), _stream(y01)))
     return out
 
 
diff --git a/bs_yolo_amd/plan.py b/bs_yolo_amd/plan.py
--- a/bs_yolo_amd/plan.py
+++ b/bs_yolo_amd/plan.py
@@ -75,6 +75,10 @@
     return (c0, c1) in ((32, 64), (16, 32)) and W % 4 == 0 and H >= 4 and W >= 4
 
 
+def stem_cv1_supported(c0: int, c1: int, cc: int) -> bool:
+    return (c0, c1, cc) == (32, 64, 64)
+
+
 def msca_spatial_supported(H: int, W: int) -> bool:
     return H > 0 and W > 0 and H * W <= 1890
 
@@ -108,7 +112,7 @@
                  fuse_stem: Optional[bool] = None, fuse_bneck: Optional[bool] = None, fuse_head: Optional[bool] = None,
                  fuse_dwpw: Optional[bool] = None, merge_c3k: Optional[bool] = None, fuse_msca: Optional[bool] = None,
                  fuse_tail: Optional[bool] = None, precision: str = "fp16", lanes: Optional[bool] = None, latency: bool = False,
-                 fuse_pmsfa: Optional[bool] = None):
+                 fuse_pmsfa: Optional[bool] = None, fuse_stem_cv1: Optional[bool] = None):
         self.cfg, self.B, self.H, self.W = cfg, B, H, W
         self.latency = bool(latency) and precision == "fp16"
         if precision not in ("fp16", "fp32", "fp32x"):
@@ -127,6 +131,8 @@
         self.fuse_msca = (os.environ.get("BSY_FUSE_MSCA", "1") != "0") if fuse_msca is None else bool(fuse_msca)
         self.fuse_tail = (os.environ.get("BSY_FUSE_TAIL", "1") != "0") if fuse_tail is None else bool(fuse_tail)
         self.fuse_pmsfa = (os.environ.get("BSY_FUSE_PMSFA", "1") != "0") if fuse_pmsfa is None else bool(fuse_pmsfa)
+        self.fuse_stem_cv1 = ((os.environ.get("BSY_FUSE_STEM_CV1", "1") != "0") if fuse_stem_cv1 is None else bool(fuse_stem_cv1)) \
+            and self.fuse_stem and self.fuse_tail and not self.f32_mode
         self.buf_bytes: List[int] = []
         self.ops: List[dict] = []
         self.wrecs: "OrderedDict[str, WRec]" = OrderedDict()
@@ -740,6 +746,7 @@
         self.layer_out = outs
         self.meta.update(scale=scale, n_layers=len(layers), legacy=legacy)
         self._fuse_stem()
+        self._fuse_stem_cv1()
 
     def _fuse_stem(self):
         if not self.fuse_stem or len(self.ops) < 2:
@@ -764,6 +771,25 @@
                               in_dtype=self.in_dtype, name=a["name"] + "+" + b["name"].split(".")[-1], lane=0,
                               mfma_flops=a["mfma_flops"] + b["mfma_flops"])]
         self.layer_out[0] = None
+
+    def _fuse_stem_cv1(self):
+        if not self.fuse_stem_cv1 or len(self.ops) < 2:
+            return
+        a, b = self.ops[0], self.ops[1]
+        if a["kind"] != L.OP_STEM or b["kind"] != L.OP_C3K2:
+            return
+        x = a["dst"]
+        if b["src0"] is not x or b.get("lane", 0) != 0 or not stem_cv1_supported(a["mid_c"], x.C, 2 * b["mid_c"]):
+            return
+        for o in self.ops[2:]:
+            if x.buf in self.op_buffers(o):
+                return
+        if not isinstance(self.layer_out[1], T) or self.layer_out[1].buf != x.buf:
+            return
+        fl = 2 * self.B * x.H * x.W * 2 * b["mid_c"] * x.C
+        a.update(fold_cv1=1, wkeys=[b["wkeys"][0]], mfma_flops=a["mfma_flops"] + fl)
+        b.update(fold_cv1=1, mfma_flops=b["mfma_flops"] - fl)
+        self.layer_out[1] = None
 
     _VIEW_KEYS = ("src0", "src1", "dst", "res")
     _LIST_KEYS = ("box", "cls", "msk")
@@ -888,4 +914,5 @@
             o.lane, o.join, o.tuned_cfg = d.get("lane", 0), d.get("join", 0), 0
             o.prec = (2 if self.split_f16 else 1) if self.f32_mode else 0
             o.ksplit = d.get("ksplit", 0)
+            o.fold_cv1 = d.get("fold_cv1", 0)
         return arr
diff --git a/include/bsyolo.h b/include/bsyolo.h
--- a/include/bsyolo.h
+++ b/include/bsyolo.h
@@ -83,6 +83,8 @@
     int32_t ne;
     int32_t ksplit;
     int32_t reserved1;
+    int32_t fold_cv1;
+    int32_t reserved2;
 } bsy_op;
 
 int bsy_sizeof_op(void);
@@ -126,6 +128,10 @@
 int bsy_stem_fused(const void* img, int img_dtype, int B, int H, int W, const void* w0, const float* b0, int C0,
                    const void* w1, const float* b1, int C1, void* y, int ldy, int act, bsy_stream stream);
 int bsy_stem_fused_supported(int C0, int C1, int H, int W);
+int bsy_stem_cv1_fused(const void* img, int img_dtype, int B, int H, int W, const void* w0, const float* b0, int C0,
+                       const void* w1, const float* b1, int C1, const void* wc, const float* bc, int Cc, void* y, int ldy,
+                       bsy_stream stream);
+int bsy_stem_cv1_supported(int C0, int C1, int Cc);
 
 int bsy_bottleneck_fused(const void* x, int ldx, int B, int H, int W, int C, int CH, const void* w1, const float* b1,
                          const void* w2, const float* b2, void* y, int ldy, int act, bsy_stream stream);
@@ -133,6 +139,8 @@
 int bsy_c3k2_fused(const void* x, int ldx, int B, int H, int W, int Cin, int c, int C2, const void* w1, const float* b1, const void* wa,
                    const float* ba, const void* wb, const float* bb, const void* w4, const float* b4, void* y, int ldy, bsy_stream stream);
 int bsy_c3k2_fused_supported(int Cin, int c, int C2);
+int bsy_c3k2_preact(const void* y01, int ldx, int B, int H, int W, int c, int C2, const void* wa, const float* ba, const void* wb,
+                    const float* bb, const void* w4, const float* b4, void* y, int ldy, bsy_stream stream);
 
 int bsy_dwconv(const void* x, int ldx, int B, int H, int W, int C, int kh, int kw, int stride, const float* w, int wld,
                const float* b, void* y, int ldy, int act, bsy_stream stream);
```
